# lgalke/aae-recommender

Measured on AMD Instinct MI355X. Metric: train docs/sec at |items|=100k h=200, higher is better.
Workload: dtype f32; 1 GPU; C3 PubMed-scale synthetic Bags: |items|=100000, hidden=200, code=50, fp32, batch=100 docs/GPU/step, full partial_fit (ae+disc+gen, 4 Adam) inside the AdversarialAutoEncoder.fit epoch loop (permutation batches of a corpus resident in HBM); n_items=100000, n_hidden=200, n_code=50, batch_per_gpu=100, global_batch=100, cond_inc=0, rng=device, parallelism=dp1

## Files before the change

### aae-recommender_amd/aaerec/_hip.py

```python
import ctypes as C
import itertools
import weakref
import os

import numpy as np
import torch

_HERE = os.path.dirname(os.path.abspath(__file__))
LIB_PATH = os.environ.get("AAE_HIP_LIB") or os.path.join(_HERE, "libaaerec_hip.so")

ABI_VERSION = 4
ACTIVATIONS = {"ReLU": 0, "SELU": 1, "Tanh": 2, "Sigmoid": 3, "ELU": 4, "LeakyReLU": 5,
               "Softplus": 6, "Hardtanh": 7, "ReLU6": 8, "CELU": 9, "Softsign": 10, "Hardsigmoid": 11, "LogSigmoid": 12,
               "Softshrink": 13, "Hardshrink": 14, "Identity": 15, "GELU": 16, "SiLU": 17, "Mish": 18, "Hardswish": 19}
FINALS = {"linear": 0, "softmax": 1, "sigmoid": 2}
OPTIMIZERS = {"adam": 0, "sgd": 1}
PRIORS = {"gauss": 0, "categorical": 1, "bernoulli": 2}
RNG_INJECT, RNG_DEVICE = 0, 1
RANK_K_MAX = 1024
COOC_TILE = 16384
SPGEMM_HASH_PRODUCTS = 4096
SPGEMM_STAGE = 512
SPTRANS_LDS = 4096
LOWRANK_DIMS_MAX = 4096
METRIC_MAX = 32
METRIC_ROW_MAX = 4096
RANK_ABSENT = 2 ** 31 - 1
METRIC_NDCG_K_MAX = 1 << 20
METRIC_KINDS = {"mrr": 0, "map": 1, "p": 2, "ndcg": 3, "r-prec": 4, "clicks": 5}
GRAD_FUSED, GRAD_EXPORT = 0, 1


class _NullCtx:
    def __enter__(self):
        return None

    def __exit__(self, *a):
        return False


_NULL_CTX = _NullCtx()

T_ENC_W1T, T_ENC_B1, T_ENC_W2, T_ENC_W3, T_DEC_V1, T_DEC_V2, T_DEC_V3, T_DISC_D1, T_DISC_D2, T_DISC_D3 = range(10)
T_ADAM_ENC, T_ADAM_GEN, T_ADAM_DEC, T_ADAM_DISC, T_GRAD = 16, 32, 48, 64, 80
T_ACT_Z, T_ACT_LOSSES, T_ACT_A1, T_ACT_DZC, T_ACT_DH2, T_ACT_DA2 = 96, 97, 98, 99, 100, 101
T_ACT_GA1 = 102
CAT_SUM, CAT_MEAN = 0, 1
CAT_SPARSE_ADAM, CAT_ADAM = 0, 1
O_ENC, O_DEC, O_GEN, O_DISC = 0, 1, 2, 3
MODEL_AAE, MODEL_AE, MODEL_VAE = 0, 1, 3
DTYPE_F32, DTYPE_BF16 = 0, 1


class AaeConfig(C.Structure):
    _fields_ = [("abi_version", C.c_int32), ("n_items", C.c_int32), ("n_hidden", C.c_int32),
                ("n_code", C.c_int32), ("cond_inc", C.c_int32), ("max_batch", C.c_int32),
                ("max_nnz", C.c_int32), ("activation", C.c_int32), ("enc_final", C.c_int32),
                ("optimizer", C.c_int32), ("normalize_inputs", C.c_int32), ("rng_mode", C.c_int32),
                ("prior", C.c_int32), ("grad_mode", C.c_int32), ("dropout1", C.c_float),
                ("dropout2", C.c_float), ("gen_lr", C.c_float), ("reg_lr", C.c_float),
                ("prior_scale", C.c_float), ("has_prior_scale", C.c_int32), ("seed", C.c_uint64),
                ("unfused_decoder", C.c_int32), ("dp_world", C.c_int32), ("model_kind", C.c_int32),
                ("dtype", C.c_int32), ("blocked_output", C.c_int32), ("dense_noise", C.c_int32),
                ("reserved", C.c_int32 * 2)]


class AaeBatch(C.Structure):
    _fields_ = [("indptr_dev", C.c_void_p), ("indices_dev", C.c_void_p), ("values_dev", C.c_void_p),
                ("rows_dev", C.c_void_p), ("row_start", C.c_int32), ("n_rows", C.c_int32),
                ("nnz_bound", C.c_int32), ("max_row_nnz", C.c_int32), ("generation", C.c_int64)]


class AaeRngInject(C.Structure):
    _fields_ = [("masks_dev", C.c_void_p * 12), ("z_real_dev", C.c_void_p)]


_COLL_AG = C.CFUNCTYPE(C.c_int, C.c_void_p, C.c_void_p, C.c_void_p, C.c_int64, C.c_void_p)
_COLL_AR = C.CFUNCTYPE(C.c_int, C.c_void_p, C.c_void_p, C.c_int64, C.c_void_p)


class AaeCollectives(C.Structure):
    _fields_ = [("ctx", C.c_void_p), ("all_gather", _COLL_AG), ("reduce_scatter", _COLL_AG), ("all_reduce", _COLL_AR),
                ("world", C.c_int32), ("rank", C.c_int32)]


class AaeTensor(C.Structure):
    _fields_ = [("byte_offset", C.c_size_t), ("rows", C.c_int64), ("cols", C.c_int64), ("ld", C.c_int64)]


class AaeCooc(C.Structure):
    _fields_ = [("indptr_dev", C.c_void_p), ("indices_dev", C.c_void_p), ("values_dev", C.c_void_p), ("n_rows", C.c_int32)]


class AaePopular(C.Structure):
    _fields_ = [("counts_dev", C.c_void_p), ("order_dev", C.c_void_p), ("pos_dev", C.c_void_p), ("n_items", C.c_int32)]


class AaeMetricSpec(C.Structure):
    _fields_ = [("kind", C.c_int32), ("k", C.c_int32)]


class AaeRankRows(C.Structure):
    _fields_ = [("indptr_dev", C.c_void_p), ("ranks_dev", C.c_void_p), ("n_rows", C.c_int32)]


class AaeLowRank(C.Structure):
    _fields_ = [("vt_dev", C.c_void_p), ("ld", C.c_int64), ("n_features", C.c_int32), ("dims", C.c_int32)]


_PROTOS = {
    "aae_abi_version": (C.c_int, []),
    "aae_set_option": (C.c_int, [C.c_char_p, C.c_char_p]),
    "aae_last_error": (C.c_char_p, []),
    "aae_arena_bytes": (C.c_int, [C.POINTER(AaeConfig), C.POINTER(C.c_size_t)]),
    "aae_create": (C.c_int, [C.POINTER(AaeConfig), C.c_void_p, C.c_size_t, C.c_void_p, C.POINTER(C.c_void_p)]),
    "aae_destroy": (C.c_int, [C.c_void_p]),
    "aae_tensor_info": (C.c_int, [C.c_void_p, C.c_int, C.POINTER(AaeTensor)]),
    "aae_set_lr": (C.c_int, [C.c_void_p, C.c_double, C.c_double]),
    "aae_params_changed": (C.c_int, [C.c_void_p]),
    "aae_set_rng_rows": (C.c_int, [C.c_void_p, C.c_int64, C.c_int64]),
    "aae_sync": (C.c_int, [C.c_void_p, C.c_void_p]),
    "aae_load_linear": (C.c_int, [C.c_void_p, C.c_int, C.c_int, C.c_void_p, C.c_void_p]),
    "aae_store_linear": (C.c_int, [C.c_void_p, C.c_int, C.c_int, C.c_void_p, C.c_void_p]),
    "aae_load_adam": (C.c_int, [C.c_void_p, C.c_int, C.c_int, C.c_void_p, C.c_void_p, C.c_void_p, C.c_void_p, C.c_int64]),
    "aae_store_adam": (C.c_int, [C.c_void_p, C.c_int, C.c_int, C.c_void_p, C.c_void_p, C.c_void_p, C.c_void_p, C.POINTER(C.c_int64)]),
    "aae_step": (C.c_int, [C.c_void_p, C.POINTER(AaeBatch), C.c_void_p, C.POINTER(AaeRngInject), C.c_void_p]),
    "aae_ae_encode": (C.c_int, [C.c_void_p, C.POINTER(AaeBatch), C.POINTER(AaeRngInject), C.c_void_p, C.c_void_p]),
    "aae_ae_decode_backward": (C.c_int, [C.c_void_p, C.c_void_p, C.c_int64, C.POINTER(AaeRngInject), C.c_void_p, C.c_void_p]),
    "aae_vae_step": (C.c_int, [C.c_void_p, C.POINTER(AaeBatch), C.c_void_p, C.c_void_p, C.c_void_p]),
# ... 39 lines not shown
    "aae_w1_import": (C.c_int, [C.c_void_p, C.c_void_p, C.c_void_p, C.c_int32, C.c_int32, C.c_int64, C.c_int, C.c_void_p]),
    "aae_set_grad_scale": (C.c_int, [C.c_void_p, C.c_float]),
    "aae_ae_forward": (C.c_int, [C.c_void_p, C.POINTER(AaeBatch), C.c_void_p, C.POINTER(AaeRngInject), C.c_void_p]),
    "aae_output_layer_step": (C.c_int, [C.c_void_p, C.POINTER(AaeBatch), C.c_void_p]),
    "aae_ae_backward": (C.c_int, [C.c_void_p, C.c_void_p, C.c_int64, C.c_void_p]),
    "aae_set_doc_l1": (C.c_int, [C.c_void_p, C.c_void_p]),
    "aae_set_first_layer_external": (C.c_int, [C.c_void_p, C.c_int]),
    "aae_first_layer_forward": (C.c_int, [C.c_void_p, C.POINTER(AaeBatch), C.c_void_p, C.c_void_p]),
    "aae_first_layer_update": (C.c_int, [C.c_void_p, C.c_void_p, C.c_int64, C.c_int32, C.c_int64, C.c_int, C.c_void_p]),
    "aae_apply_gathered": (C.c_int, [C.c_void_p, C.c_int, C.c_int, C.c_void_p, C.c_int64, C.c_int32, C.c_int64, C.c_void_p]),
    "aae_cat_encode": (C.c_int, [C.c_void_p, C.c_int32, C.c_int32, C.c_void_p, C.c_int32, C.c_int32, C.c_int32, C.c_void_p,
                                 C.c_int64, C.c_void_p]),
    "aae_cat_update": (C.c_int, [C.c_void_p, C.c_void_p, C.c_void_p, C.c_void_p, C.c_int32, C.c_int32, C.c_void_p, C.c_int32,
                                 C.c_int32, C.c_int32, C.c_void_p, C.c_int64, C.c_int32, C.c_double, C.c_int64, C.c_void_p]),
    "aae_csr_embed": (C.c_int, [C.c_void_p, C.c_void_p, C.c_void_p, C.c_int32, C.c_void_p, C.c_int32, C.c_int32, C.c_int64,
                                C.c_void_p, C.c_int64, C.c_void_p]),
    "aae_cooc_scores": (C.c_int, [C.POINTER(AaeCooc), C.c_int32, C.POINTER(AaeBatch), C.c_void_p, C.c_int64, C.c_void_p]),
    "aae_cooc_topk": (C.c_int, [C.POINTER(AaeCooc), C.c_int32, C.POINTER(AaeBatch), C.c_int32, C.c_int32, C.c_void_p, C.c_int64,
                                C.c_void_p, C.c_void_p, C.c_void_p]),
    "aae_cooc_ranks": (C.c_int, [C.POINTER(AaeCooc), C.c_int32, C.POINTER(AaeBatch), C.POINTER(AaeBatch), C.c_int32, C.c_void_p,
                                 C.c_int64, C.c_void_p, C.c_void_p]),
    "aae_cooc_scores_i32": (C.c_int, [C.POINTER(AaeCooc), C.c_int32, C.POINTER(AaeBatch), C.c_void_p, C.c_int64, C.c_void_p]),
    "aae_cooc_topk_i32": (C.c_int, [C.POINTER(AaeCooc), C.c_int32, C.POINTER(AaeBatch), C.c_int32, C.c_int32, C.c_void_p, C.c_int64,
                                    C.c_void_p, C.c_void_p, C.c_void_p]),
    "aae_cooc_ranks_i32": (C.c_int, [C.POINTER(AaeCooc), C.c_int32, C.POINTER(AaeBatch), C.POINTER(AaeBatch), C.c_int32, C.c_void_p,
                                     C.c_int64, C.c_void_p, C.c_void_p]),
    "aae_spgemm_i32_bound": (C.c_int, [C.POINTER(AaeCooc), C.POINTER(AaeCooc), C.c_int32, C.c_void_p, C.c_void_p]),
    "aae_spgemm_i32_count": (C.c_int, [C.POINTER(AaeCooc), C.POINTER(AaeCooc), C.c_int32, C.c_void_p, C.c_void_p, C.c_void_p]),
    "aae_spgemm_i32_fill": (C.c_int, [C.POINTER(AaeCooc), C.POINTER(AaeCooc), C.c_int32, C.c_void_p, C.c_void_p, C.c_void_p, C.c_void_p,
                                      C.c_void_p]),
    "aae_csr_transpose_count": (C.c_int, [C.c_void_p, C.c_void_p, C.c_int32, C.c_int32, C.c_void_p, C.c_void_p]),
    "aae_csr_transpose_fill": (C.c_int, [C.c_void_p, C.c_void_p, C.c_void_p, C.c_int32, C.c_int32, C.c_void_p, C.c_void_p, C.c_void_p,
                                         C.c_void_p, C.c_void_p, C.c_int64, C.c_int64, C.c_void_p]),
    "aae_mi_i32_marginals": (C.c_int, [C.POINTER(AaeCooc), C.POINTER(AaeCooc), C.c_int32, C.c_int32, C.c_void_p, C.c_void_p, C.c_void_p,
                                       C.c_void_p]),
    "aae_mi_i32_rows": (C.c_int, [C.POINTER(AaeCooc), C.POINTER(AaeCooc), C.c_int32, C.c_void_p, C.c_void_p, C.c_void_p, C.c_void_p,
                                  C.c_void_p]),
    "aae_mi_i32_finish": (C.c_int, [C.c_int32, C.c_void_p, C.c_void_p, C.c_void_p, C.c_void_p]),
    "aae_pop_counts": (C.c_int, [C.POINTER(AaeCooc), C.c_int32, C.c_void_p, C.c_void_p]),
    "aae_pop_topk": (C.c_int, [C.POINTER(AaePopular), C.POINTER(AaeBatch), C.c_int32, C.c_int32, C.c_void_p, C.c_void_p, C.c_void_p]),
    "aae_pop_ranks": (C.c_int, [C.POINTER(AaePopular), C.POINTER(AaeBatch), C.POINTER(AaeBatch), C.c_int32, C.c_void_p, C.c_void_p]),
    "aae_rand_scores": (C.c_int, [C.c_uint64, C.c_int64, C.c_int64, C.c_int32, C.c_int32, C.c_int32, C.c_void_p, C.c_int64, C.c_void_p]),
    "aae_rand_topk": (C.c_int, [C.c_uint64, C.c_int64, C.c_int64, C.c_int32, C.c_int32, C.POINTER(AaeBatch), C.c_int32, C.c_int32, C.c_void_p,
                                C.c_void_p, C.c_void_p]),
    "aae_rand_ranks": (C.c_int, [C.c_uint64, C.c_int64, C.c_int64, C.c_int32, C.c_int32, C.POINTER(AaeBatch), C.POINTER(AaeBatch), C.c_int32,
                                 C.c_void_p, C.c_void_p]),
    "aae_metric_rows": (C.c_int, [C.POINTER(AaeRankRows), C.POINTER(AaeMetricSpec), C.c_int32, C.c_void_p, C.c_int32, C.c_void_p,
                                  C.c_int64, C.c_void_p]),
    "aae_metric_finish": (C.c_int, [C.c_void_p, C.c_int64, C.c_int32, C.c_int32, C.c_void_p, C.c_void_p]),
    "aae_ranks_from_lists": (C.c_int, [C.c_void_p, C.c_int64, C.c_int32, C.POINTER(AaeBatch), C.c_void_p, C.c_void_p]),
    "aae_spmm_f32": (C.c_int, [C.POINTER(AaeBatch), C.c_void_p, C.c_int64, C.c_int32, C.c_int32, C.c_void_p, C.c_int64, C.c_void_p]),
    "aae_lowrank_scores": (C.c_int, [C.POINTER(AaeLowRank), C.c_int32, C.POINTER(AaeBatch), C.c_void_p, C.c_int64, C.c_void_p, C.c_int64,
                                     C.c_void_p]),
    "aae_lowrank_topk": (C.c_int, [C.POINTER(AaeLowRank), C.c_int32, C.POINTER(AaeBatch), C.POINTER(AaeBatch), C.c_int32, C.c_int32,
                                   C.c_void_p, C.c_int64, C.c_void_p, C.c_int64, C.c_void_p, C.c_void_p, C.c_void_p]),
    "aae_lowrank_ranks": (C.c_int, [C.POINTER(AaeLowRank), C.c_int32, C.POINTER(AaeBatch), C.POINTER(AaeBatch), C.POINTER(AaeBatch),
                                    C.c_int32, C.c_void_p, C.c_int64, C.c_void_p, C.c_int64, C.c_void_p, C.c_void_p]),
    "aae_dense_to_csr": (C.c_int, [C.c_void_p, C.c_int32, C.c_int64, C.c_int32, C.c_int32, C.c_void_p, C.c_void_p, C.c_void_p,
                                   C.c_int64, C.c_void_p, C.POINTER(C.c_int32 * 4), C.c_void_p]),
    "aae_profile_enable": (C.c_int, [C.c_void_p, C.c_int]),
    "aae_profile_read": (C.c_int, [C.c_void_p, C.c_int, C.POINTER(C.c_double), C.POINTER(C.c_int64)]),
    "aae_join": (C.c_int, [C.c_void_p, C.c_void_p]),
    "aae_join_output_layer": (C.c_int, [C.c_void_p, C.c_void_p]),
    "aae_rccl_unique_id": (C.c_int, [C.c_char_p]),
    "aae_rccl_init": (C.c_int, [C.c_char_p, C.c_int32, C.c_int32, C.POINTER(AaeCollectives)]),
    "aae_rccl_destroy": (C.c_int, [C.POINTER(AaeCollectives)]),
    "aae_dp_step": (C.c_int, [C.c_void_p, C.c_void_p, C.POINTER(AaeCollectives), C.POINTER(AaeBatch), C.POINTER(AaeBatch),
                              C.POINTER(AaeBatch), C.c_void_p, C.POINTER(AaeRngInject), C.c_void_p]),
    "aae_dp_reserve": (C.c_int, [C.c_void_p, C.c_int32, C.c_int32]),
    "aae_shard_step": (C.c_int, [C.c_void_p, C.POINTER(AaeCollectives), C.POINTER(AaeBatch), C.POINTER(AaeBatch), C.c_void_p,
                                 C.POINTER(AaeRngInject), C.c_float, C.c_void_p]),
    "aae_memcpy_sync": (C.c_int, [C.c_void_p, C.c_void_p, C.c_size_t, C.c_void_p]),
    "aae_echo_collectives": (C.c_int, [C.c_int32, C.POINTER(AaeCollectives)]),
    "aae_ipc_create": (C.c_int, [C.c_int64, C.c_char_p, C.POINTER(C.c_void_p)]),
    "aae_ipc_init": (C.c_int, [C.c_void_p, C.c_char_p, C.c_int32, C.c_int32, C.c_int64, C.POINTER(AaeCollectives)]),
    "aae_ipc_destroy": (C.c_int, [C.POINTER(AaeCollectives), C.c_void_p]),
    "aae_set_input_noise": (C.c_int, [C.c_void_p, C.c_void_p, C.c_int64]),
    "aae_set_input_noise_gen": (C.c_int, [C.c_void_p, C.c_float]),
    "aae_dae_thin": (C.c_int, [C.c_void_p, C.c_void_p, C.c_void_p, C.c_void_p, C.c_int64, C.c_float, C.c_void_p, C.c_void_p]),
    "aae_prefetch_batch": (C.c_int, [C.c_void_p, C.POINTER(AaeBatch)]),
    "aae_set_split": (C.c_int, [C.c_void_p, C.c_int32]),
}
K_ENC_GATHER, K_DEC_BCE_FWD, K_DEC_DA2, K_DEC_DV3_ADAM, K_ENC_W1_ADAM, K_DEC_FUSED, K_CHAIN, K_DEC_CRIT, K_DEC_OPT, K_RANK, K_COLLECTIVE = range(11)

_lib = None


class AaeHipError(RuntimeError):
    pass


def _destroy_handle(lib, handle, arena, pid):
    if os.getpid() == pid:
        try:
            lib.aae_destroy(handle)
        except Exception:
            pass
    del arena


def load_library():
    global _lib
    if _lib is not None:
        return _lib
    if not os.path.exists(LIB_PATH):
        raise ImportError(
            f"{LIB_PATH} is missing: build it with `python -c 'import __graft_entry__ as g; g.build()'` "
            "(hipcc --offload-arch=gfx950).  There is no CPU fallback for the AAE step.")
    lib = C.CDLL(LIB_PATH)
    for name, (res, args) in _PROTOS.items():
        fn = getattr(lib, name)
        fn.restype, fn.argtypes = res, args
    if lib.aae_abi_version() != ABI_VERSION:
        raise ImportError("libaaerec_hip.so ABI version mismatch")
    _lib = lib
    return lib


def set_option(name, value):
    _check(load_library().aae_set_option(str(name).encode(), None if value is None else str(value).encode()))


def _check(rc):
    if rc != 0:
        raise AaeHipError(f"libaaerec_hip error {rc}: {load_library().aae_last_error().decode()}")


def _ptr(t):
    return None if t is None else C.c_void_p(t.data_ptr())


def _arg(a):
    if a is None or torch.is_tensor(a):
        return _ptr(a)
    return C.byref(a) if isinstance(a, C.Structure) else a


_UPLOAD_STREAMS = {}


def upload(x, device, dtype=None):
    t = x if torch.is_tensor(x) else torch.as_tensor(np.asarray(x))
    dev = torch.device(device)
    if t.is_cuda or dev.type != "cuda":
        return t.to(dev, dtype) if dtype is not None else t.to(dev)
    if dtype is not None:
        t = t.to(dtype)
    side = _UPLOAD_STREAMS.get(dev)
    if side is None:
        side = _UPLOAD_STREAMS[dev] = torch.cuda.Stream(dev)
    with torch.cuda.stream(side):
        out = t.to(dev)
    out.record_stream(torch.cuda.current_stream(dev))
    return out


class HostRows:
    PIN_LIMIT = 32 << 30

    def __init__(self, n_rows, n_cols, device):
        self.device = torch.device(device)
        self.pinned = n_rows * n_cols * 4 <= self.PIN_LIMIT
        if self.pinned:
            try:
                self.host = torch.empty(n_rows, n_cols, dtype=torch.float32, pin_memory=True)
            except RuntimeError:
# ... 1304 lines not shown
```

### aae-recommender_amd/csrc/aae_abi.hip

```cpp
#include <hip/hip_runtime.h>
#include <hip/hip_ext.h>
#include <math.h>
#include <stdio.h>
#include <stdlib.h>
#include <string.h>

#include <algorithm>
#include <string>
#include <vector>

#include "../../include/aaerec_hip.h"
#include "gemm_f32.h"
#include "kernels.h"
#include "dec_fused.h"
#include "dec_fused_bf16.h"
#include "dec_crit_x3.h"
#include "rank_x3.h"
#include "rank_long.h"
#include "rank_full.h"
#include "cooc.h"
#include "spgemm.h"
#include "sptrans.h"
#include "mutinfo.h"
#include "popular.h"
#include "randrank.h"
#include "rank_metrics.h"
#include "lowrank.h"
#include "chain.h"
#include "chain4.h"
#include "chain16x3.h"
#include "cond_embed.h"
#include "w1_update.h"
#include "dae_corrupt.h"

using namespace aae;

#include "kernel_pick.h"

#include <map>
static std::map<std::string, std::string> g_options;
const char* option_value(const char* name) {
    auto it = g_options.find(name);
    if (it != g_options.end()) return it->second.c_str();
    return getenv((std::string("AAE_") + name).c_str());
}

#include "abi_model.h"
#include "abi_layers.h"
#include "abi_chains.h"
#include "abi_rank.h"

extern "C" {

int aae_abi_version(void) { return AAE_ABI_VERSION; }

int aae_set_option(const char* name, const char* value) {
    if (!name || !*name) return fail(AAE_EINVAL, "option name is empty");
    static const char* known[] = {"NO_CHAIN", "CHAIN16", "SPLIT_ANY", "BLOCKED_ANY", "EARLY_ANY", "NO_LATE_JOIN", "NO_ITEM_COUNT", "NO_ITEM_LISTS", "W1_SERIAL",
                                  "NO_RANK_FUSED", "CHAIN_KSLICES", "X16_ROWS", "DW_KSPLIT_ROWS", "DEC_TS", "CHAIN_TS", "DW_TS", "DEC_SKIP", "CHAIN_SKIP", "RANK_SKIP",
                                  "RANK_COLLECT_CAP"};
    bool ok = false;
    for (const char* k : known) ok = ok || strcmp(k, name) == 0;
    if (!ok) return fail(AAE_EINVAL, "unknown option (aae_options, csrc/abi_model.h, lists them)");
    if (value && strcmp(name, "RANK_COLLECT_CAP") == 0) {
        char* end = nullptr;
        const long v = strtol(value, &end, 10);
        if (end == value || *end || v < 1 || v > kLongCap) return fail(AAE_EINVAL, "RANK_COLLECT_CAP must be a whole number in [1, 4096]");
    }
    if (value) g_options[name] = value; else g_options.erase(name);
    return AAE_OK;
}
const char* aae_last_error(void) { return g_err.c_str(); }

int aae_arena_bytes(const aae_config* cfg, size_t* bytes_out) {
    TRY(validate(cfg));
    if (!bytes_out) return fail(AAE_EINVAL, "bytes_out is NULL");
    aae_model tmp; memset((void*)&tmp, 0, sizeof(tmp)); tmp.cfg = *cfg;
    read_options(tmp.opt);
    *bytes_out = layout(&tmp, nullptr, true);
    return AAE_OK;
}

int aae_create(const aae_config* cfg, void* arena_dev, size_t arena_bytes, void* stream, aae_handle* out) {
    TRY(validate(cfg));
    if (!arena_dev || !out) return fail(AAE_EINVAL, "arena/out is NULL");
    if (reinterpret_cast<uintptr_t>(arena_dev) & 255) return fail(AAE_EINVAL, "arena must be 256-byte aligned");
    aae_model* m = new aae_model();
    memset((void*)m, 0, sizeof(*m));
    m->cfg = *cfg;
    read_options(m->opt);
    size_t need = layout(m, static_cast<char*>(arena_dev), false);
    if (need > arena_bytes) { delete m; return fail(AAE_ENOMEM, "arena smaller than aae_arena_bytes()"); }
    m->base = static_cast<char*>(arena_dev); m->bytes = need;
    m->alpha_mode = cfg->activation == AAE_ACT_SELU;
    m->vae = cfg->model_kind == 3; m->vae_cut = false;
    m->bf16 = cfg->dtype == 1;
    m->blocked_ok = cfg->blocked_output == 1;
    m->blocked_any = m->opt.blocked_any;
    m->split_any = m->opt.split_any;
    m->x3_gemm = !m->bf16;
    m->noise_next = nullptr; m->noise_ld = 0; m->dense_step = false; m->noise_gen_next = false; m->noise_gen_scale = 0.f;
    m->ae_only = cfg->model_kind == 1 || m->vae;
    m->lazy = true;
    auto limit = [](bool& ok, size_t bytes) { return [&ok, bytes](auto kernel) { ok = ok && raise_lds_limit(kernel, bytes); }; };
    const int maxlds = 160 * 1024;
    {
        int dev = 0, cus = 0;
        if (hipGetDevice(&dev) != hipSuccess ||
            hipDeviceGetAttribute(&cus, hipDeviceAttributeMultiprocessorCount, dev) != hipSuccess || cus < 1) {
            delete m; return fail(AAE_EHIP, "no HIP device");
        }
        m->n_cu = std::min(cus, 304);
        const int nb = (m->h + 1 + 15) / 16;
        m->fused_nb = nb <= 4 ? 4 : nb <= 7 ? 7 : nb <= 13 ? 13 : 0;
        m->fused_ok = m->fused_nb != 0 && fused_width_ok(m->h, m->ldh);
        m->use_chain = (m->h + 1 <= 208) && (m->c + 1 <= 208) && (m->cp + 1 <= (m->vae ? kVaeDecInMax : 2 * 208)) &&
                       !m->opt.no_chain;
        const size_t chain_lds = kCSlots * kCR * kCL * sizeof(float);
        if (m->use_chain) each_chain(false, limit(m->use_chain, chain_lds));
        m->act_nm = cfg->activation > AAE_ACT_LEAKYRELU;
        if (m->use_chain && m->act_nm) each_chain(true, limit(m->use_chain, chain_lds));
        m->use_chain4 = m->use_chain && !m->act_nm && !m->opt.chain16;
        if (m->use_chain4) each_chain4(limit(m->use_chain4, chain_lds));
        if (m->use_chain && m->cp + 1 > 208 && !m->use_chain4 && !m->vae) m->use_chain = false;
        m->x16_rows = m->opt.x16_rows;
        m->dw_ksplit_rows = 256;
        if (m->opt.dw_ksplit_rows >= 0) m->dw_ksplit_rows = m->opt.dw_ksplit_rows;
        if (!m->opt.no_item_count) {
            void* hp = nullptr; void* dp = nullptr;
            if (hipHostMalloc(&hp, 64, hipHostMallocMapped) == hipSuccess && hipHostGetDevicePointer(&dp, hp, 0) == hipSuccess) {
                m->cnt_host = static_cast<int*>(hp); m->cnt_host_dev = static_cast<int*>(dp); *m->cnt_host = 0;
            } else { if (hp) (void)hipHostFree(hp); (void)hipGetLastError(); }
        }
        m->x16_ok = m->use_chain4 && m->FXi[P_W2] != nullptr;
        if (m->x16_ok) each_chain16x3(limit(m->x16_ok, kX16Lds));
        m->force_unfused = cfg->unfused_decoder == 1;
        if (m->fused_ok) {
            each_dec_fused(kDecFused, limit(m->fused_ok, maxlds));
            if (m->bf16) each_dec_fused_bf16(kDecFused, limit(m->fused_ok, maxlds));
            if (!raise_lds_limit(tile_bucket_kernel, maxlds - 2048)) m->fused_ok = false;
            m->bucket_wide_ok = raise_lds_limit(tile_bucket_wide_kernel, maxlds - 16384);
            {
                hipFuncAttributes fa;
                static bool told = false;
                if (m->bucket_wide_ok && !told && hipFuncGetAttributes(&fa, reinterpret_cast<const void*>(tile_bucket_wide_kernel)) == hipSuccess && fa.numRegs < 121) {
                    told = true;
                    fprintf(stderr, "aaerec: tile_bucket_wide_kernel allocates %d vector registers, not the 128 it claims to keep its CU to itself (buckets.h)\n", fa.numRegs);
                }
                (void)hipGetLastError();
            }
        }
    }
    m->late_enabled = !m->opt.no_late_join;
    m->early_enabled = true;
    m->early_any = m->opt.early_any;
    m->rank_ok = m->fused_ok && m->use_chain4 && !m->vae && !m->opt.no_rank_fused;
    m->vae_rank_ok = m->vae && m->fused_ok && m->use_chain4 && !m->opt.no_rank_fused;
    if (m->vae_rank_ok) each_chain4_vae(limit(m->vae_rank_ok, kCSlots * kCR * kCL * sizeof(float)));
    bool& rank_ok = m->vae ? m->vae_rank_ok : m->rank_ok;
    if (rank_ok) each_rank([&](const RankPick& r) { rank_ok = rank_ok && raise_lds_limit(r.kernel, r.lds); });
    m->w1_big_lds = raise_lds_limit(w1_item_update_kernel, sizeof(int) * w1_items_lds_words(16384));
    (void)hipGetLastError();
    m->grad_scale = 1.f;
    m->rng_row0 = 0; m->rng_global = 0;
    m->Gt = m->G.p;
    m->split_ok = false; m->opt_pending = false; m->side = nullptr; m->ev_crit = m->ev_opt = nullptr;
    m->split_wgs = std::max(1, (m->n_cu * 5) / 8);
    m->pf_armed = m->pf_built = m->pf_pending = false; m->pf_step = -1; m->hstep = 0; m->flushed_hstep = -1; m->ev_head = m->ev_pf = nullptr;
    bool side_ok = false;
    if (cfg->grad_mode == AAE_GRAD_FUSED) {
        int lo = 0, hi = 0;
        const unsigned evflags = hipEventDisableTiming | hipEventDisableSystemFence;
        side_ok = hipDeviceGetStreamPriorityRange(&lo, &hi) == hipSuccess &&
                  hipStreamCreateWithPriority(&m->side, hipStreamNonBlocking, lo) == hipSuccess &&
                  hipEventCreateWithFlags(&m->ev_crit, evflags) == hipSuccess &&
                  hipEventCreateWithFlags(&m->ev_opt, evflags) == hipSuccess &&
                  hipEventCreateWithFlags(&m->ev_head, evflags) == hipSuccess &&
                  hipEventCreateWithFlags(&m->ev_pf, evflags) == hipSuccess &&
                  hipEventCreateWithFlags(&m->ev_bk, evflags) == hipSuccess &&
                  hipEventCreateWithFlags(&m->ev_end, evflags) == hipSuccess;
        if (!side_ok) {
            if (m->side) (void)hipStreamDestroy(m->side);
            m->side = nullptr;
        }
        (void)hipGetLastError();
    }
    if (side_ok && m->fused_ok && m->bf16 && m->split_wgs > 0 &&
        (size_t)((m->N + kBU - 1) / kBU) * kBU * bf_stride(4) <= (size_t)m->R * m->ldn) {
        m->split_ok = true;
        for (int mode : {kDecCrit, kDecOpt}) each_dec_fused_bf16(mode, limit(m->split_ok, maxlds));
        (void)hipGetLastError();
    }
    if (side_ok && m->fused_ok && m->split_wgs > 0 && 
        (size_t)((m->N + kTI - 1) / kTI) * kTI * (size_t)std::min(m->R, 16 * kMB) * sizeof(float) < (size_t)0x7FFFFFF0u) {
        bool ok = true;
        for (int mode : {kDecCrit, kDecOpt, kDecOptAcc}) each_dec_fused(mode, limit(ok, maxlds));
        each_dec_opt_blocks(limit(ok, maxlds));
        if (!m->bf16) m->split_ok = ok;
        m->x3_ok = ok;
        each_dec_crit_x3(false, limit(m->x3_ok, maxlds));
        each_dec_opt_blocks_x3(limit(m->x3_ok, maxlds));
        each_dec_opt_x3(false, limit(m->x3_ok, maxlds));
        (void)hipGetLastError();
        if (m->bf16) {
            m->bf16_x3 = m->x3_ok && ok;
            if (!m->bf16_x3) m->x3_ok = false;
            else m->split_ok = true;
            m->bf16_one = m->bf16_x3;
            each_dec_crit_x3(true, limit(m->bf16_one, maxlds));
            each_dec_opt_x3(true, limit(m->bf16_one, maxlds));
            (void)hipGetLastError();
        }
        if (m->x3_ok) {
            const int ntiles = (m->N + 31) / 32;
            const double t_tile = (2.2 + 0.0096 * m->h) * (m->bf16_one ? 0.98 : 1.0);
            int w = (int)(ntiles * t_tile / (m->bf16_one ? 127.0 : 57.0) / 8.0 + 0.5) * 8;
            w = std::max(w, std::min(ntiles, m->bf16_one ? 40 : 64));
            const int cap = m->late_enabled ? m->n_cu * 7 / 16 : m->n_cu * 9 / 16;
            m->split_wgs = std::max(1, std::min(w, cap));
        }
    }
    hipStream_t s = S(stream);
    hipError_t e = hipMemsetAsync(arena_dev, 0, need, s);
    if (e != hipSuccess) { delete m; return fail(AAE_EHIP, std::string("hipMemsetAsync: ") + hipGetErrorString(e)); }
    struct { Ten* t; int col; } ones[] = {{&m->eh1, m->h}, {&m->eh2, m->h}, {&m->zc, m->cp}, {&m->dh1, m->h},
                                           {&m->dh2, m->h}, {&m->zin, m->c}, {&m->xh1, m->h}, {&m->xh2, m->h}};
    for (auto& o : ones)
        hipLaunchKernelGGL(fill_col_kernel, dim3(((int)o.t->rows + 255) / 256), dim3(256), 0, s, o.t->p, (int)o.t->ld,
                           (int)o.t->rows, o.col, 1.0f);
    OptScalars hs[4]; memset(hs, 0, sizeof(hs));
    for (int i = 0; i < 4; ++i) {
        hs[i].t = 0; hs[i].is_sgd = cfg->optimizer == AAE_OPT_SGD;
        hs[i].lr = (i == O_ENC || i == O_DEC) ? (double)cfg->gen_lr : (double)cfg->reg_lr;
        hs[i].neg_step_size = 0.f; hs[i].bc2_sqrt = 1.f; hs[i].inv_bc2_sqrt = 1.f;
    }
    e = hipMemcpyAsync(m->sc, hs, sizeof(hs), hipMemcpyHostToDevice, s);
    if (e == hipSuccess) e = hipStreamSynchronize(s);
    if (e != hipSuccess) { delete m; return fail(AAE_EHIP, std::string("init: ") + hipGetErrorString(e)); }
    *out = m;
    return AAE_OK;
}

#ifdef W1_TS
int aae_debug_w1_ts(unsigned long long* out, int n) {
    return (int)hipMemcpyFromSymbol(out, HIP_SYMBOL(aae::w1_ts), sizeof(unsigned long long) * (size_t)n);
}
#endif
int aae_destroy(aae_handle h) {
    if (!h) return AAE_OK;
    if (h->side) {
        (void)hipStreamSynchronize(h->side);
        (void)hipStreamDestroy(h->side);
    }
    if (h->dp_scratch) (void)hipFree(h->dp_scratch);
    if (h->cnt_host) (void)hipHostFree(h->cnt_host);
    for (hipEvent_t e : {h->ev_crit, h->ev_opt, h->ev_head, h->ev_pf, h->ev_bk, h->ev_end}) if (e) (void)hipEventDestroy(e);
    if (h->prof_ev) {
        for (int k = 0; k < AAE_K_N; ++k)
            for (auto& pr : h->prof_ev[k]) { (void)hipEventDestroy(pr.first); (void)hipEventDestroy(pr.second); }
        delete[] h->prof_ev;
    }
    delete h;
    return AAE_OK;
}


int aae_profile_enable(aae_handle h, int on) {
    if (!h) return fail(AAE_EINVAL, "handle is NULL");
    if (on && !h->prof_ev) h->prof_ev = new std::vector<std::pair<hipEvent_t, hipEvent_t>>[AAE_K_N];
    h->prof_on = on != 0;
    h->prof_mask = on == 1 ? ~0u : ((unsigned)on >> 1);
    return AAE_OK;
}

int aae_profile_read(aae_handle h, int kernel_id, double* total_ms, int64_t* launches) {
    if (!h || !total_ms || !launches) return fail(AAE_EINVAL, "NULL argument");
    if (kernel_id < 0 || kernel_id >= AAE_K_N) return fail(AAE_EINVAL, "bad kernel id");
    *total_ms = 0.0; *launches = 0;
    if (!h->prof_ev) return AAE_OK;
    auto& v = h->prof_ev[kernel_id];
    for (size_t i = 0; i < h->prof_used[kernel_id]; ++i) {
        HIPCHK(hipEventSynchronize(v[i].second));
        float ms = 0.f;
        HIPCHK(hipEventElapsedTime(&ms, v[i].first, v[i].second));
        *total_ms += ms; *launches += 1;
    }
    h->prof_used[kernel_id] = 0;
    return AAE_OK;
}

int aae_prefetch_batch(aae_handle h, const aae_batch* next) {
    if (!h || !next) return fail(AAE_EINVAL, "NULL argument");
    if (!next->indptr_dev || !next->indices_dev || !next->values_dev) return fail(AAE_EINVAL, "batch pointers are NULL");
    if (next->n_rows < 1 || next->n_rows > h->R) return fail(AAE_EINVAL, "batch n_rows outside [1, max_batch]");
    if (next->nnz_bound > h->cfg.max_nnz) return fail(AAE_EINVAL, "batch nnz_bound > max_nnz");
    if (next->generation == 0) { h->pf_armed = false; return AAE_OK; }
    h->pf_batch = *next;
    h->pf_armed = true;
    return AAE_OK;
}

// ... 3 lines not shown
    if (noise_dev && noise_ld < h->N) return fail(AAE_EINVAL, "noise_ld < n_items");
    h->noise_next = noise_dev; h->noise_ld = noise_ld;
    h->noise_gen_next = false;
    return AAE_OK;
}

int aae_join_output_layer(aae_handle h, void* stream) {
    if (!h) return fail(AAE_EINVAL, "handle is NULL");
    if (h->opt_pending) {
        HIPCHK(hipStreamWaitEvent(S(stream), h->ev_opt, 0));
        h->opt_pending = false;
        if (!h->pf_after_opt) h->pf_pending = false;
    }
    return AAE_OK;
}

int aae_join(aae_handle h, void* stream) {
    if (!h) return fail(AAE_EINVAL, "handle is NULL");
    return join_deferred(h, S(stream));
}

int aae_set_split(aae_handle h, int32_t workgroups) {
    if (!h) return fail(AAE_EINVAL, "handle is NULL");
    if (workgroups < 0) return fail(AAE_EINVAL, "workgroups must be >= 0");
    if (h->opt_pending) return fail(AAE_ESTATE, "aae_set_split with a deferred launch pending: call aae_join / aae_sync first");
    h->split_wgs = workgroups;
    return AAE_OK;
}

int aae_set_grad_scale(aae_handle h, float scale) {
    if (!h) return fail(AAE_EINVAL, "handle is NULL");
    h->grad_scale = scale; return AAE_OK;
}

int aae_set_rng_rows(aae_handle h, int64_t row_offset, int64_t global_rows) {
    if (!h) return fail(AAE_EINVAL, "handle is NULL");
    if (row_offset < 0 || global_rows < 0 || row_offset > (1 << 30) || global_rows > (1 << 30))
        return fail(AAE_EINVAL, "aae_set_rng_rows: bad offset / global_rows");
    h->rng_row0 = (int)row_offset; h->rng_global = (int)global_rows;
    return AAE_OK;
}

int aae_params_changed(aae_handle h) {
    if (!h) return fail(AAE_EINVAL, "handle is NULL");
    for (int i = 0; i < NP; ++i) h->pt_ok[i] = false;
    return AAE_OK;
}

int aae_set_lr(aae_handle h, double gen_lr, double reg_lr) {
    if (!h) return fail(AAE_EINVAL, "handle is NULL");
    TRY(join_host(h));
    OptScalars hs[4];
    HIPCHK(hipMemcpy(hs, h->sc, sizeof(hs), hipMemcpyDeviceToHost));
    hs[O_ENC].lr = gen_lr; hs[O_DEC].lr = gen_lr; hs[O_GEN].lr = reg_lr; hs[O_DISC].lr = reg_lr;
    HIPCHK(hipMemcpy(h->sc, hs, sizeof(hs), hipMemcpyHostToDevice));
    h->spec_tab_ok = false;
    return AAE_OK;
}

int aae_tensor_info(aae_handle h, int id, aae_tensor* out) {
    if (!h || !out) return fail(AAE_EINVAL, "handle/out is NULL");
    const Ten* t = nullptr;
    Ten tmp;
    auto adam = [&](int base, int lo, int hi, int set) -> const Ten* {
        int k = id - base, pid = lo + k / 2;
        if (k < 0 || pid > hi) return nullptr;
        return (k & 1) ? &h->V[set][pid] : &h->M[set][pid];
    };
    if (id >= 0 && id < AAE_T_N_PARAMS) t = &h->P[id];
    else if (id >= AAE_T_ADAM_ENC && id < AAE_T_ADAM_ENC + 8) t = adam(AAE_T_ADAM_ENC, P_W1T, P_W3, 0);
    else if (id >= AAE_T_ADAM_GEN && id < AAE_T_ADAM_GEN + 8) t = adam(AAE_T_ADAM_GEN, P_W1T, P_W3, 1);
    else if (id >= AAE_T_ADAM_DEC && id < AAE_T_ADAM_DEC + 6) t = adam(AAE_T_ADAM_DEC, P_V1, P_V3, 0);
    else if (id >= AAE_T_ADAM_DISC && id < AAE_T_ADAM_DISC + 6) t = adam(AAE_T_ADAM_DISC, P_D1, P_D3, 0);
    else if (id >= AAE_T_GRAD && id < AAE_T_GRAD + NP) { t = &h->Gr[id - AAE_T_GRAD]; if (!t->rows) t = nullptr; }
    else if (id == AAE_T_ACT_Z) t = &h->zsave;
    else if (id == AAE_T_ACT_A1) t = &h->a1;
    else if (id == AAE_T_ACT_DH2) t = &h->dh2;
    else if (id == AAE_T_ACT_DA2) t = &h->da2;
    else if (id == AAE_T_ACT_GA1) t = (h->ext_first && h->ga1x.p) ? &h->ga1x : h->use_chain ? &h->gb3 : &h->gb1;
    else if (id == AAE_T_ACT_DZC) { tmp = h->gzc; tmp.cols = h->cp; t = &tmp; }
    else if (id == AAE_T_ACT_LOSSES) {
        tmp.rows = 1; tmp.cols = 4; tmp.ld = 4; tmp.off = (size_t)((char*)h->losses - h->base); t = &tmp;
    }
    if (!t) return fail(AAE_EINVAL, "unknown tensor id");
    out->byte_offset = t->off; out->rows = t->rows; out->cols = t->cols; out->ld = t->ld;
    return AAE_OK;
}

int aae_sync(aae_handle h, void* stream) {
    if (!h) return fail(AAE_EINVAL, "handle is NULL");
    TRY(join_deferred(h, S(stream)));
    return lazy_flush(h, S(stream));
}


}

#include "abi_condition.h"
#include "abi_state_dict.h"
#include "abi_dae.h"
#include "abi_step_open.h"
#include "abi_output_layer.h"
#include "abi_step_phases.h"
#include "abi_predict.h"
#include "abi_cooc.h"
#include "abi_spgemm.h"
#include "abi_sptrans.h"
#include "abi_mutinfo.h"
#include "abi_popular.h"
#include "abi_random.h"
#include "abi_metrics.h"
#include "abi_lowrank.h"
#include "abi_data_parallel.h"

#include "dp_step.h"
#include "ipc_collectives.h"
```

### aae-recommender_amd/csrc/abi_chains.h

```cpp
#pragma once

namespace {

ChainOp cop(int kind, int src, int dst, int N) {
    ChainOp o; memset(&o, 0, sizeof(o));
    o.kind = kind; o.src = src; o.dst = dst; o.N = N; o.one_col = -1; o.scale = 1.f; o.yslot = 0; o.fake_slot = -1;
    return o;
}
ChainOp cop_load(const float* g, int ld, int dst, int N, int row0 = 0) {
    ChainOp o = cop(COP_LOAD, 0, dst, N); o.W = g; o.ldw = ld; o.out_row0 = row0; return o;
}
ChainOp cop_linear(int kind, int src, int dst, const Ten& W, int K, int N, int epi) {
    ChainOp o = cop(kind, src, dst, N); o.W = W.p; o.ldw = (int)W.ld; o.K = K; o.epi = epi;
    if (kind == COP_LINEAR_DX) { o.Wkn = W.p; o.ldkn = (int)W.ld; }
    return o;
}
void cop_out(ChainOp& o, float* out, int ld, int row0 = 0) { o.out = out; o.ldo = ld; o.out_row0 = row0; }

W4Copies w4_of(const aae_model* m, int pid) {
    return W4Copies{m->PT[pid].p, m->D4[pid].p, (int)m->P[pid].rows, (int)m->P[pid].cols, m->FXi[pid], m->DXi[pid], m->FXBi[pid], kCWide};
}
float* ga1_ptr(const aae_model* m) {
    return (m->ext_first && m->ga1x.p) ? m->ga1x.p + (size_t)(m->R - m->rows) * m->ldh : m->gb3.p;
}
// ... 173 lines not shown
        if (u.src >= 0) o.src = phys[u.src];
        if (u.y >= 0) o.yslot = phys[u.y];
        if (u.fake >= 0) o.fake_slot = phys[u.fake];
        o.dst = phys[u.dst];
        if (o.kind == COP_FINAL_FWD) o.src = o.dst;
    }
    return true;
}

static bool x16_program_ok(const ChainProgram& P) {
    for (int i = 0; i < P.nops; ++i) {
        const ChainOp& o = P.ops[i];
        switch (o.kind) {
            case COP_LINEAR: case COP_LINEAR_DX:
                if (!o.WX || o.N > kCWide || o.K > kX16Kp) return false;
                break;
            case COP_LOAD: if (o.dst_col0 + o.N > kX16Kp) return false; break;
            case COP_DROPACT: case COP_SLABSUM: case COP_STORE: case COP_FINAL_FWD: case COP_FINAL_BWD: case COP_PRIOR: case COP_DISC_HEAD:
                if (o.N > kCWide) return false;
                break;
            default: return false;
        }
        if (o.one_col >= kX16Kp) return false;
    }
    return true;
}

int print_chain_timeline(const ChainProgram& P, const unsigned long long* ts_dev, bool x16, bool four, hipStream_t s) {
    static const char* names[] = {"LOAD", "LINEAR", "LINEAR_DX", "FINAL_FWD", "FINAL_BWD", "ADV", "DROPACT", "SLABSUM", "ACTBWD", "STORE", "REPARAM", "REPARAM_BWD", "DISC_HEAD", "PRIOR"};
    unsigned long long h[128];
    HIPCHK(hipStreamSynchronize(s));
    HIPCHK(hipMemcpy(h, ts_dev, sizeof(h), hipMemcpyDeviceToHost));
    if (x16) {
        fprintf(stderr, "[chain16x3 rows=%d nops=%d total=%.2fus; per op: whole (products | epilogue | barrier)]", P.rows, P.nops, (h[3 * P.nops] - h[0]) * 0.01);
        for (int i = 0; i < P.nops; ++i) {
            const bool lin = P.ops[i].kind == COP_LINEAR || P.ops[i].kind == COP_LINEAR_DX;
            fprintf(stderr, " %s(K%d,N%d)=%.2f", names[P.ops[i].kind], P.ops[i].K, P.ops[i].N, (h[3 * i + 3] - h[3 * i]) * 0.01);
            if (lin) fprintf(stderr, "(%.2f|%.2f|%.2f)", (h[3 * i + 1] - h[3 * i]) * 0.01, (h[3 * i + 2] - h[3 * i + 1]) * 0.01, (h[3 * i + 3] - h[3 * i + 2]) * 0.01);
        }
        fprintf(stderr, "\n");
        return AAE_OK;
    }
    fprintf(stderr, "[chain rows=%d nops=%d total=%.2fus]", P.rows, P.nops, (h[P.nops] - h[0]) * 0.01);
    for (int i = 0; i < P.nops; ++i)
        fprintf(stderr, " %s(K%d,N%d%s%s)=%.2f", names[P.ops[i].kind], P.ops[i].K, P.ops[i].N,
                P.ops[i].out ? ",st" : "", P.ops[i].out2 ? ",st2" : "", (h[i + 1] - h[i]) * 0.01);
    fprintf(stderr, "\n");
    if (P.nops <= 2) return AAE_OK;
    fprintf(stderr, "   [op 2, wave 0 of workgroup 0] loads+mfma+partials=%.2f wait-barrier=%.2f epi-ctx=%.2f epilogue=%.2f barrier=%.2f (us)\n",
            (h[21] - h[20]) * 0.01, (h[22] - h[21]) * 0.01, (h[23] - h[22]) * 0.01, (h[24] - h[23]) * 0.01, (h[25] - h[24]) * 0.01);
    if (!four) return AAE_OK;
    fprintf(stderr, "   [op 2: matrix phase %.2f us = %.0f shader clocks -> %.2f GHz]\n", (h[64 + 50] - h[64 + 48]) * 0.01,
            (double)(h[64 + 51] - h[64 + 49]), (double)(h[64 + 51] - h[64 + 49]) / ((h[64 + 50] - h[64 + 48]) * 10.0));
    for (int k = 0; k < 3; ++k) {
        fprintf(stderr, "   [op 2, every wave, us after the op's start: %s]", k == 0 ? "loads issued" : k == 1 ? "first chunk multiplied" : "partial sums stored");
        for (int w = 0; w < 16; ++w) fprintf(stderr, " %.2f", ((double)h[64 + 16 * k + w] - (double)h[64 + 48]) * 0.01);
        fprintf(stderr, "\n");
    }
    return AAE_OK;
}

int launch_chain(aae_model* m, ChainBuilder& cb, hipStream_t s) {
    if (cb.P.nops > kCMaxOps) return fail(AAE_ESTATE, "chain program too long");
    const bool want_ts = m->opt.chain_ts && !cb.vae4;
    static unsigned long long* ts_dev = nullptr;
    if (want_ts) {
        if (!ts_dev && hipMalloc(&ts_dev, 128 * sizeof(unsigned long long)) != hipSuccess) return fail(AAE_EHIP, "ts alloc");
        cb.P.ts = ts_dev;
    }
    const bool ts_kernel = want_ts && !m->bf16;
    ProfScope ps(m, AAE_K_CHAIN, s);
    bool four = m->use_chain4;
    for (int i = 0; i < cb.P.nops && four; ++i)
        if ((cb.P.ops[i].kind == COP_LINEAR || cb.P.ops[i].kind == COP_LINEAR_DX) && !cb.P.ops[i].Wkn && !cb.P.ops[i].W4) four = false;
    for (int i = 0; i < cb.P.nops && four; ++i)
        if (cb.P.ops[i].kind == COP_ADV || (cb.P.ops[i].kind == COP_REPARAM && !cb.vae4) || cb.P.ops[i].kind == COP_REPARAM_BWD) four = false;
    if (cb.vae4 && !four) return fail(AAE_ESTATE, "a VAE rank program needs the 4-row chain kernel");
    for (int i = 0; i < cb.P.nops; ++i)
        if ((cb.P.ops[i].row_lo > 0 || cb.P.ops[i].y_glb) && !four)
            return fail(AAE_ESTATE, "a program prefix for the upper rows / an epilogue's y from global memory needs the 4-row chain kernel");
    if (four && m->x16_ok && cb.P.rows >= (cb.x16_rows > 0 ? cb.x16_rows : m->x16_rows) && !cb.P.bk.enabled && !cb.P.il.enabled && x16_program_ok(cb.P)) {
        ChainProgram X = cb.P;
        if (x16_remap_slots(X)) {
            X.x16_row_lo = 1 << 30;
            for (int i = 0; i < X.nops; ++i) if (X.ops[i].row_lo > 0) X.x16_row_lo = X.ops[i].row_lo;
            for (int cls = 0; cls < 2; ++cls) {
                int nxt = -1;
                for (int i = X.nops - 1; i >= 0; --i) {
                    X.ops[i].x16_next_lin[cls] = nxt;
                    const bool runs = cls == 1 || X.ops[i].row_lo == 0;
                    if (runs && (X.ops[i].kind == COP_LINEAR || X.ops[i].kind == COP_LINEAR_DX)) nxt = i;
                }
                X.x16_first_lin[cls] = nxt;
            }
            const ChainKernel kernel = pick_chain16x3(m->bf16, ts_kernel);
            if (!kernel) return fail(AAE_ESTATE, "no chain16x3 kernel is compiled for this mode");
            hipLaunchKernelGGL(kernel, dim3((X.rows + kX16R - 1) / kX16R), dim3(kX16T), kX16Lds, s, X);
            LAUNCHCHK("chain16x3_kernel");
            return ts_kernel ? print_chain_timeline(X, ts_dev, true, four, s) : AAE_OK;
        }
    }
    const ChainKernel kernel = four ? pick_chain4(m->bf16, ts_kernel, m->bf16 && !cb.P.kslices, cb.vae4) : pick_chain(m->bf16, m->act_nm);
    if (!kernel) return fail(AAE_ESTATE, "no chain kernel is compiled for this mode");
    int grid = (cb.P.rows + (four ? kR4 : kCR) - 1) / (four ? kR4 : kCR) + (cb.P.bk.enabled ? 1 : 0);
    if (cb.P.il.enabled && !four) cb.P.il.enabled = 0;
    if (cb.P.il.enabled) { grid += cb.P.il.nblocks; m->il_set ^= 1; m->item_lists_valid = true; }
    hipLaunchKernelGGL(kernel, dim3(grid), dim3(four ? kC4T : kCT), kCSlots * kCR * kCL * sizeof(float), s, cb.P);
    LAUNCHCHK("chain_kernel");
    return want_ts ? print_chain_timeline(cb.P, ts_dev, false, four, s) : AAE_OK;
}

int launch_w1_hot(aae_model* m, hipStream_t s);
static ItemLists item_lists_of(const aae_model* m, int set) {
    ItemLists L;
    L.rec = m->il_rec[set]; L.ovf = m->il_ovf[set]; L.hot_count = m->il_hot_count + set; L.cap = m->il_cap; L.hot_cap = m->il_hot_cap;
    return L;
}
struct DwBuilder {
    aae_model* mh = nullptr;
    DwGroup g; int tiles;
    int ksplit_rows = 0;
    int dw_ts = -1;
    DwBuilder() { memset(&g, 0, sizeof(g)); tiles = 0; }
    void add(aae_model* m, const float* G, int ldg, const float* X, int ldx, int rows, int pid, int which) {
        DwJob& J = g.jobs[g.njobs++];
        ksplit_rows = m->dw_ksplit_rows; dw_ts = m->opt.dw_ts;
        const Ten& W = m->P[pid];
        const int set = (which == O_GEN) ? 1 : 0;
        J.G = G; J.ldg = ldg; J.X = X; J.ldx = ldx; J.rows = rows; J.M = (int)W.rows; J.N = (int)W.cols;
        J.p = W.p; J.m = m->M[set][pid].p; J.v = m->V[set][pid].p; J.ld = (int)W.ld; J.sc = m->sc + which;
        J.grad = m->cfg.grad_mode == AAE_GRAD_EXPORT ? m->Gr[pid].p : nullptr;
        J.w4 = w4_of(m, pid);
        J.tile0 = tiles; J.tiles_n = (J.N + 31) / 32;
        tiles += ((J.M + 31) / 32) * J.tiles_n;
    }
    int add_first_layer(aae_model* m, const float* ga1, int which, hipStream_t s) {
        const int set = (which == O_GEN) ? 1 : 0;
        W1Job& w = g.w1;
        w.enabled = 1; w.ga1 = ga1; w.ld = m->ldh; w.h = m->h; w.rows = m->rows;
        w.bp = m->P[P_B1].p; w.bm = m->M[set][P_B1].p; w.bv1 = m->V[set][P_B1].p;
        w.bgrad = m->cfg.grad_mode == AAE_GRAD_EXPORT ? m->Gr[P_B1].p : nullptr; w.sc = m->sc + which;
        w.ncol = (m->h + 63) / 64;
        constexpr bool no_merge = false;
        w.nitem = 0;
        m->w1_items_merged = false;
        w.wave_form = 0;
        if (!no_merge && !m->dense_step && (!m->ext_first || m->own_first) && sizeof(int) * w1_items_lds_words(m->rows) <= kDwSmemBytes) {
            TRY(ensure_buckets(m, s));
            w.items = w1_items_args(m, ga1, 0, 0, which);
            w.nitem = std::max(1, std::min(std::min(m->cfg.max_nnz, std::max(256, m->rows * 32)), m->N));
            m->w1_items_merged = true;
            constexpr bool no_wave = false;
            constexpr bool no_hybrid = false, hyb_any = false;
            if (!no_hybrid && m->rows <= 16 * kMB && sizeof(int) * w1_hybrid_lds_words(m->rows) <= kDwSmemBytes &&
                (int64_t)m->cfg.max_nnz <= 512ll * w.nitem && ((int64_t)m->N >= 40ll * m->rows || hyb_any)) {
                w.wave_form = 2;
                w.nitem = (w.nitem + 3) / 4;
                if (m->item_lists_valid && !w.items.gout) {
                    w.lists_on = 1; w.lists = item_lists_of(m, m->il_set);
                    w.nhot = std::min(m->il_hot_cap, 64);
                }
            } else
            if (!no_wave && m->rows > 16 * kMB && m->hot_list && (int64_t)m->N >= 40ll * m->rows) {
                w.wave_form = 1;
                w.nitem = (w.nitem + 3) / 4;
                const int set = m->hot_flip; m->hot_flip ^= 1;
                w.hot = m->hot_list + (size_t)set * m->hot_cap; w.hot_count = m->hot_count + set; w.hot_zero = m->hot_count + (set ^ 1);
                m->w1_hot_pending = true; m->w1_hot_set = set; m->w1_hot_which = which; m->w1_hot_ga1 = ga1;
                mh = m;
            }
            w.cnt_out = nullptr;
            constexpr bool hyb_count = true;
            if ((w.wave_form != 2 || hyb_count) && m->cnt_host) {
                w.cnt_out = m->cnt_host_dev;
                const int seen = *reinterpret_cast<volatile int*>(m->cnt_host);
                if (seen > 0) {
                    const int per = w.wave_form ? 4 : 1;
                    int want = ((seen + seen / 4 + per - 1) / per + 63) & ~63;
                    if (w.wave_form == 2) want = std::max(want, (int)((std::min<int64_t>(m->cfg.max_nnz, m->N) + 2047) / 2048));
                    w.nitem = std::min(w.nitem, std::max(256, want));
                }
            }
            if (w.lists_on) w.nitem += w.nhot;
        }
        return AAE_OK;
    }
    void add_loss(aae_model* m, int n, int slot) { g.loss.enabled = 1; g.loss.terms = m->adv_terms; g.loss.n = n; g.loss.out = m->losses + slot; }
    int launch(hipStream_t s, hipEvent_t done = nullptr, bool* marked = nullptr) {
        int blocks = tiles;
// ... 120 lines not shown
        const int gy = std::max(1, std::min(16, m->chunks / 16 + 1));
        hipLaunchKernelGGL(zero_int_kernel, dim3(std::min(64, ntiles / 256 + 1)), dim3(256), 0, s, m->tcount, ntiles + 1);
        hipLaunchKernelGGL(tile_hist_kernel, dim3(B, gy), dim3(256), 0, s, m->bv, m->tcount);
        hipLaunchKernelGGL(tile_scan_kernel, dim3(1), dim3(1024), 0, s, m->tcount, m->tstart, ntiles);
        hipLaunchKernelGGL(tile_fill_kernel, dim3(B, gy), dim3(256), 0, s, m->bv, m->tstart, m->tcount, m->teb, m->ten, m->tev);
    }
    LAUNCHCHK("tile buckets");
    m->buckets_valid = true;
    return AAE_OK;
}
int build_tile_buckets_aside(aae_model* m) {
    TRY(build_tile_buckets(m, m->side));
    HIPCHK(hipEventRecord(m->ev_bk, m->side));
    m->bk_pending = true;
    return AAE_OK;
}
int ensure_buckets(aae_model* m, hipStream_t s) {
    if (m->bk_pending) {
        HIPCHK(hipStreamWaitEvent(s, m->ev_bk, 0));
        m->bk_pending = false;
    }
    if (!m->buckets_valid) TRY(build_tile_buckets(m, s));
    return AAE_OK;
}

W1Items w1_items_args(aae_model* m, const float* ga1, int rpb, size_t bstride, int which) {
    const int set = (which == O_GEN) ? 1 : 0;
    W1Items a;
    a.ulist = m->ulist; a.ucount = m->ucount;
    a.tstart = m->tstart; a.eb = m->teb; a.en = m->ten; a.ev = m->tev;
    a.ga1 = ga1; a.ld = m->ldh; a.rpb = rpb; a.bstride = bstride;
    a.rscale = m->rscale; a.rows = m->rows; a.h = m->h;
    a.W = m->P[P_W1T].p; a.M = m->M[set][P_W1T].p; a.V = m->V[set][P_W1T].p; a.ldw = m->ldw1;
    a.gout = m->cfg.grad_mode == AAE_GRAD_EXPORT ? m->Gr[P_W1T].p : nullptr;
    a.sc = m->sc + which; a.tsync = m->tsync; a.step_ctr = m->step_ctr;
    a.mark_synced = (which == O_GEN || m->ae_only) ? 1 : 0;
    return a;
}
int launch_w1_items(aae_model* m, const float* ga1, int rpb, size_t bstride, int which, hipStream_t s) {
    TRY(ensure_buckets(m, s));
    const W1Items a = w1_items_args(m, ga1, rpb, bstride, which);
    const size_t lds = sizeof(int) * w1_items_lds_words(m->rows);
    if (lds > 64 * 1024 && !m->w1_big_lds) return fail(AAE_ESTATE, "first-layer update: batch too large for the LDS row lists");
    ProfScope ps(m, AAE_K_ENC_W1_ADAM, s);
    const int items = std::max(1, std::min(std::min(m->cfg.max_nnz, std::max(256, m->rows * 32)), m->N));
    hipLaunchKernelGGL(w1_item_update_kernel, dim3(items), dim3(256), lds, s, a);
    LAUNCHCHK("w1_item_update");
    return AAE_OK;
}

static void piggyback_buckets(aae_model* m, ChainBuilder& cb) {
    const int ntiles = (m->N + kTI - 1) / kTI;
    const size_t need = sizeof(int) * ((size_t)ntiles + 1 + kBucketMaxDocs + 1 + 1024);
    if (m->x16_ok && m->rows >= m->x16_rows) return;
    if (m->buckets_valid || !fused_decoder_applies(m) || ntiles > kBucketMaxTiles || m->rows > kBucketMaxDocs ||
        need > (size_t)kCSlots * kCR * kCL * sizeof(float))
        return;
    flip_bucket_set(m);
    BucketJob& b = cb.P.bk;
    b.bv = m->bv; b.ntiles = ntiles; b.tstart = m->tstart; b.eb = m->teb; b.en = m->ten; b.ev = m->tev; b.enabled = 1;
    m->buckets_valid = true;
}

static void piggyback_item_lists(aae_model* m, ChainBuilder& cb) {
    if (m->opt.no_item_lists || !m->il_cap || m->item_lists_valid || !m->buckets_valid || m->bk_pending) return;
    if (m->cfg.grad_mode != AAE_GRAD_FUSED || m->dense_step || m->ext_first) return;
    if (m->x16_ok && m->rows >= m->x16_rows) return;
    const int bound = std::max(1, std::min(std::min(m->cfg.max_nnz, std::max(256, m->rows * 32)), m->N));
    if (!(m->rows <= 16 * kMB && sizeof(int) * w1_items_lds_words(m->rows) <= kDwSmemBytes &&
          sizeof(int) * w1_hybrid_lds_words(m->rows) <= kDwSmemBytes && (int64_t)m->cfg.max_nnz <= 512ll * bound &&
          (int64_t)m->N >= 40ll * m->rows))
        return;
    static_assert(sizeof(int) * (kC4T / 64 * 2 * kW1HybRows + kW1BuildDeferWords + 2 * 4 + 2 * kW1OvfRows + 4) <= kCSlots * kCR * kCL * sizeof(float),
                  "the builder's LDS fits a chain workgroup's");
    const int set = m->il_set ^ 1;
    ItemListJob& j = cb.P.il;
    j.ulist = m->ulist; j.ucount = m->ucount; j.tstart = m->tstart; j.eb = m->teb; j.en = m->ten; j.ev = m->tev;
    j.rscale = m->rscale; j.rows = m->rows;
    j.out = item_lists_of(m, set); j.hot_zero = m->il_hot_count + (set ^ 1);
    j.nblocks = std::max(1, std::min(64, (bound + 2 * (kC4T / 64) - 1) / (2 * (kC4T / 64))));
    j.enabled = 1;
}

int chain_ae_forward(aae_model* m, bool with_dec, const float* cond_dev, float* z_out, hipStream_t s) {
    const int B = m->rows, h = m->h, c = m->c, cp = m->cp;
    const aae_rng_inject& I = m->inj;
    ChainBuilder cb(m, B);
    piggyback_buckets(m, cb);
    chain_encoder_tail(m, cb, true, I.masks_dev[1], 1, B, m->eh2.p, s, I.masks_dev[0], 0);
    ChainOp& f = m->cfg.enc_final == AAE_FINAL_LINEAR ? cb.P.ops[cb.P.nops - 1] : cb.add(cop(COP_FINAL_FWD, 2, 2, c));
    f.aux = m->cfg.enc_final;
    cop_out(f, m->zc.p, m->ldc); f.out2 = m->zsave.p; f.ldo2 = m->ldz;
    if (z_out) { ChainOp& st = cb.add(cop(COP_STORE, 2, 2, c)); cop_out(st, z_out, c); }
    if (with_dec) {
        if (wide_dec_in(m)) {
            const int nA = kCWide - c, ci = m->cfg.cond_inc;
            ChainOp& ca = cb.add(cop_load(cond_dev, ci, 2, nA)); ca.dst_col0 = c;
            ChainOp& cl = cb.add(cop_load(cond_dev + nA, ci, 5, ci - nA)); cl.one_col = cp - kCWide;
        } else if (m->cfg.cond_inc > 0) {
            ChainOp& cl = cb.add(cop_load(cond_dev, m->cfg.cond_inc, 2, m->cfg.cond_inc)); cl.dst_col0 = c; cl.one_col = cp;
        } else {
            f.one_col = cp;
        }
        ChainOp& v1 = add_dec_in_fwd(cb, m, 2, 5, 3, s);
        v1.d = make_drop(m, 0, true, I.masks_dev[2], nullptr, B, h, 2); v1.one_col = h; cop_out(v1, m->dh1.p, m->ldh);
        ChainOp& v2 = cb.add(cop_fwd(m, P_V2, 3, 4, h + 1, h, CEPI_DROPACT, s));
        v2.d = make_drop(m, 1, true, I.masks_dev[3], nullptr, B, h, 3); v2.one_col = h; cop_out(v2, m->dh2.p, m->ldh);
    }
    m->dec_hidden_done = with_dec;
    return launch_chain(m, cb, s);
}

int chain_dec_hidden(aae_model* m, bool train, int rows, hipStream_t s) {
    const int h = m->h, cp = m->cp;
    const aae_rng_inject& I = m->inj;
    ChainBuilder cb(m, rows);
    if (wide_dec_in(m)) {
        cb.add(cop_load(m->zc.p, m->ldc, 0, kCWide));
        ChainOp& lb = cb.add(cop_load(m->zc.p + kCWide, m->ldc, 3, cp - kCWide)); lb.one_col = cp - kCWide;
    } else {
        ChainOp& l = cb.add(cop_load(m->zc.p, m->ldc, 0, cp)); l.one_col = cp;
    }
    ChainOp& v1 = add_dec_in_fwd(cb, m, 0, 3, 1, s);
    v1.d = make_drop(m, 0, train, I.masks_dev[2], nullptr, rows, h, 2); v1.one_col = h; cop_out(v1, m->dh1.p, m->ldh);
    ChainOp& v2 = cb.add(cop_fwd(m, P_V2, 1, 2, h + 1, h, CEPI_DROPACT, s));
    v2.d = make_drop(m, 1, train, I.masks_dev[3], nullptr, rows, h, 3); v2.one_col = h; cop_out(v2, m->dh2.p, m->ldh);
    return launch_chain(m, cb, s);
}

int chain_ae_backward(aae_model* m, bool dec_part, bool enc_part, const float* part_slabs, size_t slab_stride,
                      const float* gz_ext, int ld_gz, float* dzc_out, int which, hipStream_t s, int nslab = 16, bool item_lists = false) {
    const int B = m->rows, h = m->h, c = m->c, cp = m->cp;
    const aae_rng_inject& I = m->inj;
    ChainBuilder cb(m, B);
    if (dec_part) {
        if (part_slabs) {
            ChainOp& ss = cb.add(cop(COP_SLABSUM, 0, 2, h)); ss.W = part_slabs; ss.ldw = m->ldh; ss.aux = nslab; ss.stride = slab_stride;
            ss.epi = CEPI_ACTBWD; ss.aux_ptr = m->dh2.p; ss.aux_ld = m->ldh;
            ss.d = make_drop(m, 1, true, I.masks_dev[3], nullptr, B, h, 3); cop_out(ss, m->gb0.p, m->ldh);
        } else {
            cb.add(cop_load(m->gb0.p, m->ldh, 2, h));
        }
        if (y_needs_load(m)) cb.add(cop_load(m->dh1.p, m->ldh, 3, h));
        ChainOp& x2 = cb.add(cop_dx(m, P_V2, 2, 4, h, h, CEPI_ACTBWD, s)); set_y(cb, m, x2, m->dh1.p, m->ldh, 3);
        x2.d = make_drop(m, 0, true, I.masks_dev[2], nullptr, B, h, 2); cop_out(x2, m->gb1.p, m->ldh);
        add_dec_in_dx(cb, m, 4, 5, 3, dzc_out, s);
    }
    if (enc_part) {
        if (!dec_part || gz_ext) cb.add(cop_load(gz_ext ? gz_ext : m->gzc.p, gz_ext ? ld_gz : m->ldc, 5, c));
        int sg = 7;
        ChainOp* prod = (dec_part && !gz_ext && cb.P.nops) ? &cb.P.ops[cb.P.nops - 1] : nullptr;
        if (m->cfg.enc_final == AAE_FINAL_LINEAR && prod && cp == c && !prod->out2) {
            prod->out2 = m->ga3.p; prod->ldo2 = m->ldz; sg = 5;
        } else {
            if (m->cfg.enc_final != AAE_FINAL_LINEAR) cb.add(cop_load(m->zsave.p, m->ldz, 6, c));
            ChainOp& fb = cb.add(cop(COP_FINAL_BWD, 5, 7, c)); fb.yslot = 6; fb.aux = m->cfg.enc_final;
            cop_out(fb, m->ga3.p, m->ldz);
        }
        if (y_needs_load(m)) cb.add(cop_load(m->eh2.p, m->ldh, 8, h));
        ChainOp& x3 = cb.add(cop_dx(m, P_W3, sg, 9, c, h, CEPI_ACTBWD, s)); set_y(cb, m, x3, m->eh2.p, m->ldh, 8);
        x3.d = make_drop(m, 1, true, I.masks_dev[which == O_GEN ? 9 : 1], nullptr, B, h, which == O_GEN ? 9 : 1);
        cop_out(x3, m->gb2.p, m->ldh);
        if (y_needs_load(m)) cb.add(cop_load(m->eh1.p, m->ldh, 0, h));
        ChainOp& x2 = cb.add(cop_dx(m, P_W2, 9, 1, h, h, CEPI_ACTBWD, s)); set_y(cb, m, x2, m->eh1.p, m->ldh, 0);
        x2.d = make_drop(m, 0, true, I.masks_dev[which == O_GEN ? 8 : 0], nullptr, B, h, which == O_GEN ? 8 : 0);
        cop_out(x2, ga1_ptr(m), m->ldh);
    }
    if (item_lists) piggyback_item_lists(m, cb);
    return launch_chain(m, cb, s);
}

int encoder_first_layer_update(aae_model* m, const float* ga1, int which, hipStream_t s, bool merged = false) {
    const int B = m->rows, h = m->h;
    const int set = (which == O_GEN) ? 1 : 0;
    const bool exportg = m->cfg.grad_mode == AAE_GRAD_EXPORT;
    if (m->dense_step) {
        if (!merged) {
            hipLaunchKernelGGL(colsum_adam_kernel, dim3((h + 63) / 64), dim3(1024), 0, s, ga1, B, h, m->ldh, m->P[P_B1].p,
                               m->M[set][P_B1].p, m->V[set][P_B1].p, (float*)nullptr, m->sc + which);
            LAUNCHCHK("colsum_adam");
        }
        TRY(linear_dw(m, m->Xn.p, m->ldn, B, ga1, m->ldh, P_W1T, which, s));
        hipLaunchKernelGGL(fill_tsync_kernel, dim3(grid1d((size_t)m->N)), dim3(256), 0, s, m->tsync, m->N, m->step_ctr);
        LAUNCHCHK("fill_tsync");
        return AAE_OK;
    }
    if (!merged) {
        hipLaunchKernelGGL(colsum_adam_kernel, dim3((h + 63) / 64), dim3(1024), 0, s, ga1, B, h, m->ldh, m->P[P_B1].p,
                           m->M[set][P_B1].p, m->V[set][P_B1].p, exportg ? m->Gr[P_B1].p : (float*)nullptr, m->sc + which);
        LAUNCHCHK("colsum_adam");
    }
    if (merged && m->w1_items_merged) { m->w1_items_merged = false; return AAE_OK; }
    return launch_w1_items(m, ga1, 0, 0, which, s);
}

int launch_gather(aae_model* m, const float* bias, float* act_out, const DropSpec& d, bool head, bool open_step, const char* what,
                  hipStream_t s) {
    ProfScope ps(m, AAE_K_ENC_GATHER, s);
    const size_t shm = (size_t)16 * r4(m->h) * sizeof(float);
    constexpr int g4_rows = 512;
    const bool four = m->rows >= g4_rows;
    const AdvanceJob adv{m->sc, m->step_ctr, m->lazy ? m->tab : nullptr, m->losses, open_step ? 1 : 0,
                         head ? m->stamp2 : nullptr, head ? m->ucount2 : nullptr};
    hipExtLaunchKernelGGL(four ? enc_gather_kernel_t<4> : enc_gather_kernel_t<16>, dim3(m->rows), dim3(four ? 256 : 1024),
                          (uint32_t)(four ? shm / 4 : shm), s, nullptr, head ? m->ev_head : nullptr, 0, m->bv,
                          (const float*)m->P[P_W1T].p, m->ldw1, bias, m->h, (int)m->cfg.normalize_inputs,
                          m->a1.p, act_out, m->ldh, (int)m->cfg.activation, d, (uint64_t)m->cfg.seed,
                          (const long long*)m->step_ctr, m->rscale, m->doc_l1, adv, (long long)(open_step ? m->hstep : -1));
    LAUNCHCHK(what);
    return AAE_OK;
}

int gather_first_layer(aae_model* m, bool train, const uint8_t* mk1, uint32_t sid1, hipStream_t s, bool head = false,
                       bool open_step = false) {
    const DropSpec d1 = make_drop(m, 0, train, mk1, nullptr, m->rows, m->h, sid1);
    TRY(launch_gather(m, m->P[P_B1].p, m->eh1.p, d1, head, open_step, "enc_gather", s));
    m->pf_bumped = head;
    return AAE_OK;
}

static bool same_batch(const aae_batch& a, const aae_batch& b) {
    return a.indptr_dev == b.indptr_dev && a.indices_dev == b.indices_dev && a.values_dev == b.values_dev &&
           a.rows_dev == b.rows_dev && a.row_start == b.row_start && a.n_rows == b.n_rows &&
           a.generation != 0 && a.generation == b.generation;
}

int launch_prefetch(aae_model* m, bool wait_head = true, bool early = false) {
    const aae_batch& b = m->pf_batch;
    m->pf_armed = false;
    m->pf_this_step = true;
    m->pf_after_opt = !wait_head;
    if (!m->side || !m->mark2 || !m->lazy) return AAE_OK;
    BatchView bv; bv.indptr = b.indptr_dev; bv.indices = b.indices_dev; bv.values = b.values_dev;
    bv.rows = b.rows_dev; bv.row_start = b.row_start; bv.n_rows = b.n_rows;
    const int mr = b.max_row_nnz > 0 ? b.max_row_nnz : 1024;
    const int chunks = std::max(1, std::min(64, (mr + 15) / 16));
    const int gy = std::max(1, std::min(16, chunks / 16 + 1));
    hipStream_t q = m->side;
    if (early) HIPCHK(hipStreamWaitEvent(q, m->ev_end, 0));
    else if (wait_head) HIPCHK(hipStreamWaitEvent(q, m->ev_head, 0));
    if (early || !(wait_head && m->pf_bumped)) hipLaunchKernelGGL(bump_stamp_kernel, dim3(1), dim3(1), 0, q, m->stamp2, m->ucount2);
    m->pf_bumped = false;
    hipLaunchKernelGGL(uniq_items_kernel, dim3(b.n_rows, gy), dim3(256), 0, q, bv, m->mark2, m->stamp2, m->ulist2, m->ucount2);
    if (m->cfg.optimizer == AAE_OPT_ADAM) {
        const int grid = std::min(m->cfg.max_nnz, std::max(256, b.n_rows * 32));
        hipLaunchKernelGGL(w1_catchup_kernel, dim3(grid), dim3(256), 0, q, m->ulist2, m->ucount2, m->N, m->tsync,
                           m->P[P_W1T].p, m->M[0][P_W1T].p, m->V[0][P_W1T].p, m->M[1][P_W1T].p, m->V[1][P_W1T].p,
                           m->ldw1, m->h, m->tab, m->step_ctr, 0, m->mark, m->stamp, early ? m->hstep : -1ll);
    }
    LAUNCHCHK("prefetch (unique items + catch-up of the next batch)");
    TRY(side_done(m, m->ev_pf));
    m->pf_pending = true;
    m->pf_built = true; m->pf_step = m->hstep + 1; m->pf_built_batch = b;
    return AAE_OK;
}

int chain_vae_forward(aae_model* m, const float* cond_dev, const float* eps_dev, int rows, hipStream_t s) {
    const int h = m->h, c = m->c, cp = m->cp;
    ChainBuilder cb(m, rows);
    ChainOp& l = cb.add(cop_load(m->eh1.p, m->ldh, 0, h)); l.one_col = h;
    ChainOp& ml = cb.add(cop_fwd(m, P_W3, 0, 1, h + 1, 2 * c, CEPI_NONE, s));
    cop_out(ml, m->mulv.p, (int)m->mulv.ld);
    ChainOp& rp = cb.add(cop(COP_REPARAM, 1, 2, c));
    rp.W = eps_dev; rp.ldw = c; rp.aux = 12; rp.aux_ptr = m->veps.p; rp.aux_ld = (int)m->veps.ld;
    if (wide_dec_in(m)) {
        ChainOp& ca = cb.add(cop_load(cond_dev, m->cfg.cond_inc, 2, kCWide - c)); ca.dst_col0 = c;
        ChainOp& st = cb.add(cop(COP_STORE, 2, 2, kCWide)); cop_out(st, m->zc.p, m->ldc);
    } else {
        if (m->cfg.cond_inc > 0) {
            ChainOp& cl = cb.add(cop_load(cond_dev, m->cfg.cond_inc, 2, m->cfg.cond_inc)); cl.dst_col0 = c; cl.one_col = cp;
        } else {
            rp.one_col = cp;
        }
        ChainOp& st = cb.add(cop(COP_STORE, 2, 2, cp)); cop_out(st, m->zc.p, m->ldc);
    }
    ChainOp& v1 = add_vae_dec_in_fwd(cb, m, cond_dev, m->cfg.cond_inc, c, true, 2, 4, 3, nullptr);
    v1.one_col = h; cop_out(v1, m->dh2.p, m->ldh);
    return launch_chain(m, cb, s);
}

int chain_vae_encode(aae_model* m, const float* eps_dev, float* z_out, int rows, hipStream_t s) {
    const int h = m->h, c = m->c;
    ChainBuilder cb(m, rows);
    ChainOp& l = cb.add(cop_load(m->eh1.p, m->ldh, 0, h)); l.one_col = h;
    ChainOp& ml = cb.add(cop_fwd(m, P_W3, 0, 1, h + 1, 2 * c, CEPI_NONE, s));
    cop_out(ml, m->mulv.p, (int)m->mulv.ld);
    ChainOp& rp = cb.add(cop(COP_REPARAM, 1, 2, c));
    rp.W = eps_dev; rp.ldw = c; rp.aux = 12; rp.aux_ptr = m->veps.p; rp.aux_ld = (int)m->veps.ld;
    ChainOp& st = cb.add(cop(COP_STORE, 2, 2, c)); cop_out(st, m->zc.p, m->ldc);
    if (z_out) { st.out2 = z_out; st.ldo2 = c; }
    return launch_chain(m, cb, s);
}
int chain_vae_dec_hidden(aae_model* m, int rows, hipStream_t s) {
    const int h = m->h, cp = m->cp;
    ChainBuilder cb(m, rows);
    ChainOp& l = cb.add(cop_load(m->zc.p, m->ldc, 2, std::min(cp, kCWide)));
    if (!wide_dec_in(m)) l.one_col = cp;
    ChainOp& v1 = add_vae_dec_in_fwd(cb, m, m->zc.p, m->ldc, 0, false, 2, 4, 3, nullptr);
    v1.one_col = h; cop_out(v1, m->dh2.p, m->ldh);
    return launch_chain(m, cb, s);
}
int chain_vae_backward_dec(aae_model* m, const float* part_slabs, size_t slab_stride, float* dzc_out, hipStream_t s) {
    const int B = m->rows, h = m->h, cp = m->cp;
    ChainBuilder cb(m, B);
    if (part_slabs) {
        ChainOp& ss = cb.add(cop(COP_SLABSUM, 0, 0, h)); ss.W = part_slabs; ss.ldw = m->ldh; ss.aux = 16; ss.stride = slab_stride;
        cb.add(cop_load(m->dh2.p, m->ldh, 1, h));
        ChainOp& ab = cb.add(cop(COP_ACTBWD, 0, 2, h)); ab.yslot = 1; cop_out(ab, m->gb0.p, m->ldh);
    } else {
        cb.add(cop_load(m->gb0.p, m->ldh, 2, h));
    }
    add_vae_dec_in_dx(cb, m, 2, 3, 8, true, dzc_out);
    return launch_chain(m, cb, s);
}
int chain_vae_backward_enc(aae_model* m, const float* dz_dev, int ld_dz, hipStream_t s) {
    const int B = m->rows, h = m->h, c = m->c;
    ChainBuilder cb(m, B);
    cb.P.loss_slot = 1;
    cb.add(cop_load(dz_dev, ld_dz, 3, c));
    cb.add(cop_load(m->mulv.p, (int)m->mulv.ld, 4, 2 * c));
    ChainOp& rb = cb.add(cop(COP_REPARAM_BWD, 3, 5, 2 * c)); rb.yslot = 4; rb.scale = m->grad_scale;
    rb.aux_ptr = m->veps.p; rb.aux_ld = (int)m->veps.ld; cop_out(rb, m->gmulv.p, (int)m->gmulv.ld);
    cb.add(cop_load(m->eh1.p, m->ldh, 6, h));
    ChainOp& x1 = cb.add(cop_linear(COP_LINEAR_DX, 5, 7, m->P[P_W3], 2 * c, h, CEPI_ACTBWD)); x1.yslot = 6;
    cop_out(x1, m->gb3.p, m->ldh);
    return launch_chain(m, cb, s);
}

int chain_vae_backward(aae_model* m, const float* part_slabs, size_t slab_stride, hipStream_t s) {
    const int B = m->rows, h = m->h, c = m->c, cp = m->cp;
    ChainBuilder cb(m, B);
    cb.P.loss_slot = 1;
    if (part_slabs) {
        ChainOp& ss = cb.add(cop(COP_SLABSUM, 0, 0, h)); ss.W = part_slabs; ss.ldw = m->ldh; ss.aux = 16; ss.stride = slab_stride;
        cb.add(cop_load(m->dh2.p, m->ldh, 1, h));
        ChainOp& ab = cb.add(cop(COP_ACTBWD, 0, 2, h)); ab.yslot = 1; cop_out(ab, m->gb0.p, m->ldh);
    } else {
        cb.add(cop_load(m->gb0.p, m->ldh, 2, h));
    }
    add_vae_dec_in_dx(cb, m, 2, 3, 8, cp > c, nullptr);
    cb.add(cop_load(m->mulv.p, (int)m->mulv.ld, 4, 2 * c));
    ChainOp& rb = cb.add(cop(COP_REPARAM_BWD, 3, 5, 2 * c)); rb.yslot = 4; rb.scale = m->grad_scale;
    rb.aux_ptr = m->veps.p; rb.aux_ld = (int)m->veps.ld; cop_out(rb, m->gmulv.p, (int)m->gmulv.ld);
    cb.add(cop_load(m->eh1.p, m->ldh, 6, h));
    ChainOp& x1 = cb.add(cop_linear(COP_LINEAR_DX, 5, 7, m->P[P_W3], 2 * c, h, CEPI_ACTBWD)); x1.yslot = 6;
    cop_out(x1, m->gb3.p, m->ldh);
    return launch_chain(m, cb, s);
}

int chain_disc_step(aae_model* m, hipStream_t s) {
    const int B = m->rows, h = m->h, c = m->c;
    const aae_rng_inject& I = m->inj;
    if (!m->ext_first) TRY(gather_first_layer(m, false, nullptr, 0, s));
    constexpr bool merge_ok = true;
    bool merged = merge_ok && m->use_chain4 && B % kR4 == 0 && !m->vae;
    for (int pid : {P_W2, P_W3, P_D1, P_D2}) merged = merged && m->PT[pid].p != nullptr;
    if (!merged) {
        ChainBuilder cb(m, B);
        chain_encoder_tail(m, cb, false, nullptr, 0, B, nullptr, s);
        ChainOp& f = m->cfg.enc_final == AAE_FINAL_LINEAR ? cb.P.ops[cb.P.nops - 1] : cb.add(cop(COP_FINAL_FWD, 2, 2, c));
        f.aux = m->cfg.enc_final; cop_out(f, m->zin.p, m->ldz, B);
        TRY(launch_chain(m, cb, s));
    }
    {
        ChainBuilder cb(m, 2 * B);
        cb.beside_deferred(m);
        cb.P.loss_slot = 1; cb.P.loss_terms = m->adv_terms;
        if (merged) {
            chain_encoder_tail(m, cb, false, nullptr, 0, B, nullptr, s);
            if (m->cfg.enc_final != AAE_FINAL_LINEAR) { ChainOp& f = cb.add(cop(COP_FINAL_FWD, 2, 2, c)); f.aux = m->cfg.enc_final; }
            for (int i = 0; i < cb.P.nops; ++i) {
                ChainOp& o = cb.P.ops[i];
                o.row_lo = B;
                if (o.kind == COP_LOAD || o.out) o.out_row0 = -B;
            }
        }
        ChainOp& l = cb.add(cop(COP_PRIOR, 0, 0, c)); l.one_col = c;
        l.W = m->zin.p; l.ldw = m->ldz; l.row_split = B; l.aux = m->cfg.prior;
        l.scale = m->cfg.has_prior_scale ? m->cfg.prior_scale : 1.0f;
        l.grow0 = m->rng_row0;
        l.aux_ptr = m->cfg.rng_mode == AAE_RNG_DEVICE ? nullptr : const_cast<float*>(I.z_real_dev); l.aux_ld = c;
        cop_out(l, m->zin.p, m->ldz);
        if (merged) l.fake_slot = 2;
        ChainOp& d1 = cb.add(cop_fwd(m, P_D1, 0, 1, c + 1, h, CEPI_DROPACT, s));
        d1.d = make_drop(m, 0, true, I.masks_dev[4], I.masks_dev[6], B, h, 4); d1.one_col = h; cop_out(d1, m->xh1.p, m->ldh);
        ChainOp& d2 = cb.add(cop_fwd(m, P_D2, 1, 2, h + 1, h, CEPI_DROPACT, s));
        d2.d = make_drop(m, 1, true, I.masks_dev[5], I.masks_dev[7], B, h, 5); d2.one_col = h; cop_out(d2, m->xh2.p, m->ldh);
        ChainOp& x3 = cb.add(cop_linear(COP_DISC_HEAD, 2, 5, m->P[P_D3], h + 1, h, CEPI_ACTBWD)); x3.yslot = 2; x3.d = d2.d;
        x3.aux = 0; x3.row_split = B; x3.scale = m->grad_scale; x3.aux_ptr = m->ga3.p; x3.aux_ld = 4;
        cop_out(x3, m->gb0.p, m->ldh);
        ChainOp& x2 = cb.add(cop_dx(m, P_D2, 5, 6, h, h, CEPI_ACTBWD, s)); x2.yslot = 1; x2.d = d1.d;
        cop_out(x2, m->gb1.p, m->ldh);
        TRY(launch_chain(m, cb, s));
    }
    DwBuilder dw;
    dw.add(m, m->ga3.p, 4, m->xh2.p, m->ldh, 2 * B, P_D3, O_DISC);
    dw.add(m, m->gb0.p, m->ldh, m->xh1.p, m->ldh, 2 * B, P_D2, O_DISC);
    dw.add(m, m->gb1.p, m->ldh, m->zin.p, m->ldz, 2 * B, P_D1, O_DISC);
    dw.add_loss(m, 2 * B, 1);
    return dw.launch(s);
}

int chain_gen_step(aae_model* m, hipStream_t s) {
    const int B = m->rows, h = m->h, c = m->c;
    const aae_rng_inject& I = m->inj;
    ChainBuilder cb(m, B);
    cb.beside_deferred(m);
    cb.P.loss_slot = 2; cb.P.loss_terms = m->adv_terms;
    cb.add(cop_load(m->a1.p, m->ldh, 0, h));
    ChainOp& e1 = cb.add(cop(COP_DROPACT, 0, 1, h));
    e1.d = make_drop(m, 0, true, I.masks_dev[8], nullptr, B, h, 8); e1.one_col = h; cop_out(e1, m->eh1.p, m->ldh);
    ChainOp& e2 = cb.add(cop_fwd(m, P_W2, 1, 2, h + 1, h, CEPI_DROPACT, s));
    e2.d = make_drop(m, 1, true, I.masks_dev[9], nullptr, B, h, 9); e2.one_col = h; cop_out(e2, m->eh2.p, m->ldh);
    ChainOp& l3 = cb.add(cop_fwd(m, P_W3, 2, 3, h + 1, c, CEPI_NONE, s));
    ChainOp& f = m->cfg.enc_final == AAE_FINAL_LINEAR ? l3 : cb.add(cop(COP_FINAL_FWD, 3, 3, c));
    f.aux = m->cfg.enc_final; f.one_col = c;
    ChainOp& d1 = cb.add(cop_fwd(m, P_D1, 3, 4, c + 1, h, CEPI_DROPACT, s));
    d1.d = make_drop(m, 0, true, I.masks_dev[10], nullptr, B, h, 10); d1.one_col = h;
    ChainOp& d2 = cb.add(cop_fwd(m, P_D2, 4, 5, h + 1, h, CEPI_DROPACT, s));
    d2.d = make_drop(m, 1, true, I.masks_dev[11], nullptr, B, h, 11); d2.one_col = h;
    ChainOp& x3 = cb.add(cop_linear(COP_DISC_HEAD, 5, 8, m->P[P_D3], h + 1, h, CEPI_ACTBWD)); x3.yslot = 5; x3.d = d2.d;
    x3.aux = 1; x3.row_split = B; x3.scale = m->grad_scale;
    ChainOp& x2 = cb.add(cop_dx(m, P_D2, 8, 9, h, h, CEPI_ACTBWD, s)); x2.yslot = 4; x2.d = d1.d;
    ChainOp& dz = cb.add(cop_dx(m, P_D1, 9, 0, h, c, CEPI_NONE, s));
    int sg = 6;
    if (m->cfg.enc_final == AAE_FINAL_LINEAR) {
        cop_out(dz, m->ga3.p, m->ldz); sg = 0;
    } else {
        ChainOp& fb = cb.add(cop(COP_FINAL_BWD, 0, 6, c)); fb.yslot = 3; fb.aux = m->cfg.enc_final;
        cop_out(fb, m->ga3.p, m->ldz);
    }
    ChainOp& w3 = cb.add(cop_dx(m, P_W3, sg, 7, c, h, CEPI_ACTBWD, s)); w3.yslot = 2; w3.d = e2.d;
    cop_out(w3, m->gb2.p, m->ldh);
    ChainOp& w2 = cb.add(cop_dx(m, P_W2, 7, 8, h, h, CEPI_ACTBWD, s)); w2.yslot = 1; w2.d = e1.d;
    cop_out(w2, ga1_ptr(m), m->ldh);
    TRY(launch_chain(m, cb, s));
    DwBuilder dw;
    dw.add(m, m->ga3.p, m->ldz, m->eh2.p, m->ldh, B, P_W3, O_GEN);
    dw.add(m, m->gb2.p, m->ldh, m->eh1.p, m->ldh, B, P_W2, O_GEN);
    TRY(dw.add_first_layer(m, ga1_ptr(m), O_GEN, s));
    dw.add_loss(m, B, 2);
    const bool mark_end = m->early_enabled && m->pf_this_step && m->w1_items_merged && !m->ext_first && m->side && m->ev_end &&
                          (m->rows > 16 * kMB || m->early_any);
    bool marked = false;
    TRY(dw.launch(s, mark_end ? m->ev_end : nullptr, &marked));
    m->end_marked = marked;
    if (m->ext_first && !m->own_first) return AAE_OK;
    return encoder_first_layer_update(m, m->gb3.p, O_GEN, s, true);
}

}
```

### aae-recommender_amd/csrc/abi_layers.h

```cpp
#pragma once

namespace {

static inline int gmode(const aae_model* m) { return m->bf16 ? kGemmBf16 : m->x3_gemm ? kGemmX3 : kGemmF32; }
template <class Epi>
int linear_fwd(const float* X, int ldx, int rows, const Ten& Wa, const Epi& epi, hipStream_t s, int bf = 0) {
    GemmShape g{X, Wa.p, rows, (int)Wa.rows, (int)Wa.cols, ldx, (int)Wa.ld, r4((int)Wa.cols) + 16};
    g.k_per_split = ((int)Wa.cols + 63) / 64 * 64;
    if (Wa.rows > 4096) (void)launch_gemm_mode<0, 1, true>(bf, g, epi, 1, s);
    else (void)launch_gemm_mode<0, 1, false>(bf, g, epi, 1, s);
    LAUNCHCHK("linear_fwd");
    return AAE_OK;
}
template <class Epi>
int linear_dx(const float* Gd, int ldg, int rows, const Ten& Wa, int n_in, const Epi& epi, hipStream_t s, int bf = 0) {
    GemmShape g{Gd, Wa.p, rows, n_in, (int)Wa.rows, ldg, (int)Wa.ld, 0};
    g.k_per_split = ((int)Wa.rows + 63) / 64 * 64;
    (void)launch_gemm_mode<0, 0, false>(bf, g, epi, 1, s);
    LAUNCHCHK("linear_dx");
    return AAE_OK;
}
int linear_dw(aae_model* m, const float* Gd, int ldg, int rows, const float* X, int ldx, int pid, int which,
              hipStream_t s) {
    const Ten& W = m->P[pid];
    GemmShape g{Gd, X, (int)W.rows, (int)W.cols, rows, ldg, ldx, 0};
    g.k_per_split = (rows + 63) / 64 * 64;
    const bool big = W.rows > 4096;
    const int bf = pid == P_V3 ? gmode(m) : kGemmF32;
    if (m->cfg.grad_mode == AAE_GRAD_EXPORT) {
        EpiStore e; e.out = m->Gr[pid].p; e.ld = (int)W.ld;
        if (big) (void)launch_gemm_mode<1, 0, true>(bf, g, e, 1, s); else (void)launch_gemm_mode<1, 0, false>(bf, g, e, 1, s);
    } else {
        const int set = (which == O_GEN) ? 1 : 0;
        EpiAdam e; e.p = W.p; e.m = m->M[set][pid].p; e.v = m->V[set][pid].p; e.ld = (int)W.ld; e.sc = m->sc + which;
        m->pt_ok[pid] = false;
        if (big) (void)launch_gemm_mode<1, 0, true>(bf, g, e, 1, s); else (void)launch_gemm_mode<1, 0, false>(bf, g, e, 1, s);
    }
    LAUNCHCHK("linear_dw");
    return AAE_OK;
}

int set_batch(aae_model* m, const aae_batch* b) {
    if (!b || !b->indptr_dev || !b->indices_dev || !b->values_dev) return fail(AAE_EINVAL, "batch pointers are NULL");
    if (b->n_rows < 1 || b->n_rows > m->R) return fail(AAE_EINVAL, "batch n_rows outside [1, max_batch]");
    if (b->nnz_bound > m->cfg.max_nnz) return fail(AAE_EINVAL, "batch nnz_bound > max_nnz");
    m->bv.indptr = b->indptr_dev; m->bv.indices = b->indices_dev; m->bv.values = b->values_dev;
    m->bv.rows = b->rows_dev; m->bv.row_start = b->row_start; m->bv.n_rows = b->n_rows;
    m->rows = b->n_rows; m->have_batch = true; m->buckets_valid = false; m->item_lists_valid = false; m->w1_merged = false;
    {
        int mr = b->max_row_nnz > 0 ? b->max_row_nnz : 1024;
        m->chunks = std::max(1, std::min(64, (mr + 15) / 16));
    }
    return AAE_OK;
}

int lazy_prepare(aae_model* m, int upto_off, bool bump, hipStream_t s) {
    if (bump) hipLaunchKernelGGL(bump_stamp_kernel, dim3(1), dim3(1), 0, s, m->stamp, m->ucount);
    int gy = std::max(1, std::min(16, m->chunks / 16 + 1));
    hipLaunchKernelGGL(uniq_items_kernel, dim3(m->rows, gy), dim3(256), 0, s, m->bv, m->mark, m->stamp, m->ulist,
                       m->ucount);
    LAUNCHCHK("uniq_items");
    if (m->cfg.optimizer == AAE_OPT_ADAM) {
        int grid = std::min(m->cfg.max_nnz, std::max(256, m->rows * 32));
        hipLaunchKernelGGL(w1_catchup_kernel, dim3(grid), dim3(256), 0, s, m->ulist, m->ucount, m->N, m->tsync,
                           m->P[P_W1T].p, m->M[0][P_W1T].p, m->V[0][P_W1T].p, m->M[1][P_W1T].p, m->V[1][P_W1T].p,
                           m->ldw1, m->h, m->tab, m->step_ctr, upto_off);
        LAUNCHCHK("w1_catchup");
    }
    return AAE_OK;
}

int lazy_flush(aae_model* m, hipStream_t s) {
    if (!m->lazy || m->cfg.optimizer != AAE_OPT_ADAM) return AAE_OK;
    hipLaunchKernelGGL(w1_catchup_kernel, dim3(std::min(m->N, 8192)), dim3(256), 0, s, (const int*)nullptr,
                       (const int*)nullptr, m->N, m->tsync, m->P[P_W1T].p, m->M[0][P_W1T].p, m->V[0][P_W1T].p,
                       m->M[1][P_W1T].p, m->V[1][P_W1T].p, m->ldw1, m->h, m->tab, m->step_ctr, 0);
    LAUNCHCHK("w1_catchup all");
    return AAE_OK;
}

int encoder_forward(aae_model* m, bool train, const uint8_t* mk1, const uint8_t* mk2, uint32_t sid1, uint32_t sid2,
                    bool reuse_a1, float* z_dst, int ldz_dst, hipStream_t s) {
    const int B = m->rows, h = m->h;
    DropSpec d1 = make_drop(m, 0, train, mk1, nullptr, B, h, sid1);
    DropSpec d2 = make_drop(m, 1, train, mk2, nullptr, B, h, sid2);
    if (!reuse_a1) {
        ProfScope ps(m, AAE_K_ENC_GATHER, s);
        size_t shm = (size_t)16 * r4(h) * sizeof(float);
        hipLaunchKernelGGL(enc_gather_kernel, dim3(B), dim3(1024), shm, s, m->bv, m->P[P_W1T].p, m->ldw1,
                           m->P[P_B1].p, h, m->cfg.normalize_inputs, m->a1.p, m->eh1.p, m->ldh, m->cfg.activation,
                           d1, m->cfg.seed, m->step_ctr, m->rscale, m->doc_l1, AdvanceJob{nullptr, nullptr, nullptr, nullptr, 0},
                           (long long)-1);
        LAUNCHCHK("enc_gather");
    } else {
        hipLaunchKernelGGL(drop_act_kernel, dim3(grid1d((size_t)B * h)), dim3(256), 0, s, m->a1.p, m->eh1.p, B, h,
                           m->ldh, m->cfg.activation, d1, m->cfg.seed, m->step_ctr);
        LAUNCHCHK("drop_act");
    }
    EpiDropAct e2; e2.out = m->eh2.p; e2.ld = m->ldh; e2.act = m->cfg.activation; e2.d = d2; e2.seed = m->cfg.seed;
    e2.step_ctr = m->step_ctr;
    TRY(linear_fwd(m->eh1.p, m->ldh, B, m->P[P_W2], e2, s, gmode(m)));
    EpiStore e3; e3.out = z_dst; e3.ld = ldz_dst;
    TRY(linear_fwd(m->eh2.p, m->ldh, B, m->P[P_W3], e3, s, gmode(m)));
    if (m->cfg.enc_final != AAE_FINAL_LINEAR) {
        hipLaunchKernelGGL(final_act_fwd_kernel, dim3((B + 3) / 4), dim3(256), 0, s, z_dst, B, m->c, ldz_dst,
                           m->cfg.enc_final, (float*)nullptr, 0);
        LAUNCHCHK("final_act_fwd");
    }
    return AAE_OK;
}

int launch_w1_items(aae_model* m, const float* ga1, int rpb, size_t bstride, int which, hipStream_t s);
W1Items w1_items_args(aae_model* m, const float* ga1, int rpb, size_t bstride, int which);
int ensure_buckets(aae_model* m, hipStream_t s);

int encoder_backward(aae_model* m, const float* gz, int ldgz, const float* z, int ldzz, const uint8_t* mk1,
                     const uint8_t* mk2, uint32_t sid1, uint32_t sid2, int which, hipStream_t s) {
    const int B = m->rows, h = m->h, cc = m->c;
    DropSpec d1 = make_drop(m, 0, true, mk1, nullptr, B, h, sid1);
    DropSpec d2 = make_drop(m, 1, true, mk2, nullptr, B, h, sid2);
    const float* ga3 = gz; int ldga3 = ldgz;
    if (m->cfg.enc_final != AAE_FINAL_LINEAR) {
        hipLaunchKernelGGL(final_act_bwd_kernel, dim3((B + 3) / 4), dim3(256), 0, s, z, ldzz, gz, ldgz, m->ga3.p,
                           m->ldz, B, cc, m->cfg.enc_final);
        LAUNCHCHK("final_act_bwd");
        ga3 = m->ga3.p; ldga3 = m->ldz;
    }
    EpiActBwd b2; b2.out = m->gb0.p; b2.ld = m->ldh; b2.y = m->eh2.p; b2.ldy = m->ldh; b2.act = m->cfg.activation;
    b2.d = d2; b2.seed = m->cfg.seed; b2.step_ctr = m->step_ctr;
    TRY(linear_dx(ga3, ldga3, B, m->P[P_W3], h, b2, s, gmode(m)));
    TRY(linear_dw(m, ga3, ldga3, B, m->eh2.p, m->ldh, P_W3, which, s));
    EpiActBwd b1; b1.out = m->gb1.p; b1.ld = m->ldh; b1.y = m->eh1.p; b1.ldy = m->ldh; b1.act = m->cfg.activation;
    b1.d = d1; b1.seed = m->cfg.seed; b1.step_ctr = m->step_ctr;
    TRY(linear_dx(m->gb0.p, m->ldh, B, m->P[P_W2], h, b1, s, gmode(m)));
    TRY(linear_dw(m, m->gb0.p, m->ldh, B, m->eh1.p, m->ldh, P_W2, which, s));
    const int set = (which == O_GEN) ? 1 : 0;
    const bool exportg = m->cfg.grad_mode == AAE_GRAD_EXPORT;
    hipLaunchKernelGGL(colsum_adam_kernel, dim3((h + 63) / 64), dim3(1024), 0, s, m->gb1.p, B, h, m->ldh,
                       m->P[P_B1].p, m->M[set][P_B1].p, m->V[set][P_B1].p, exportg ? m->Gr[P_B1].p : (float*)nullptr,
                       m->sc + which);
    LAUNCHCHK("colsum_adam");
    return launch_w1_items(m, m->gb1.p, 0, 0, which, s);
}

int disc_forward(aae_model* m, int rows, const uint8_t* m1a, const uint8_t* m1b, const uint8_t* m2a,
                 const uint8_t* m2b, int split, uint32_t sid1, uint32_t sid2, hipStream_t s) {
    const int h = m->h;
    DropSpec d1 = make_drop(m, 0, true, m1a, m1b, split, h, sid1);
    DropSpec d2 = make_drop(m, 1, true, m2a, m2b, split, h, sid2);
    EpiDropAct e1; e1.out = m->xh1.p; e1.ld = m->ldh; e1.act = m->cfg.activation; e1.d = d1; e1.seed = m->cfg.seed;
    e1.step_ctr = m->step_ctr;
    TRY(linear_fwd(m->zin.p, m->ldz, rows, m->P[P_D1], e1, s, gmode(m)));
    EpiDropAct e2 = e1; e2.out = m->xh2.p; e2.d = d2;
    TRY(linear_fwd(m->xh1.p, m->ldh, rows, m->P[P_D2], e2, s, gmode(m)));
    EpiSigmoid e3; e3.out = m->dout.p; e3.ld = 4;
    TRY(linear_fwd(m->xh2.p, m->ldh, rows, m->P[P_D3], e3, s));
// ... 37 lines not shown
```

### aae-recommender_amd/csrc/abi_model.h

```cpp
#pragma once

static thread_local std::string g_err;
static int fail(int code, const std::string& msg) { g_err = msg; return code; }

#define HIPCHK(expr)                                                                        \
    do {                                                                                    \
        hipError_t e_ = (expr);                                                             \
        if (e_ != hipSuccess)                                                               \
            return fail(AAE_EHIP, std::string(#expr) + ": " + hipGetErrorString(e_));       \
    } while (0)
#define LAUNCHCHK(what)                                                                     \
    do {                                                                                    \
        hipError_t e_ = hipGetLastError();                                                  \
        if (e_ != hipSuccess) return fail(AAE_EHIP, std::string(what) + ": " + hipGetErrorString(e_)); \
    } while (0)
#define TRY(expr) do { int rc_ = (expr); if (rc_ != AAE_OK) return rc_; } while (0)

namespace {

inline int r4(int x) { return (x + 3) & ~3; }

struct Ten {
    float* p = nullptr; size_t off = 0; int64_t rows = 0, cols = 0, ld = 0;
    size_t floats() const { return (size_t)rows * ld; }
};

enum { P_W1T = 0, P_B1, P_W2, P_W3, P_V1, P_V2, P_V3, P_D1, P_D2, P_D3, NP };
enum { O_ENC = 0, O_DEC = 1, O_GEN = 2, O_DISC = 3 };

}

struct aae_options {
    bool no_chain;
    bool chain16;
    bool split_any;
    bool blocked_any;
    bool early_any;
    bool no_late_join;
    bool no_item_lists;
    bool no_item_count;
    bool w1_serial;
    bool no_rank_fused;
    bool chain_kslices;
    int x16_rows;
    int rank_collect_cap;
    int dw_ksplit_rows;
    char dec_ts[8];
    bool chain_ts;
    int dw_ts;
    int dec_skip, chain_skip, rank_skip;
};
const char* option_value(const char* name);
inline void read_options(aae_options& o) {
    auto on = [](const char* n) { return option_value(n) != nullptr; };
    auto num = [](const char* n, int dflt) { const char* e = option_value(n); return e ? atoi(e) : dflt; };
    o.no_chain = on("NO_CHAIN"); o.chain16 = on("CHAIN16"); o.split_any = on("SPLIT_ANY"); o.blocked_any = on("BLOCKED_ANY");
    o.early_any = on("EARLY_ANY"); o.no_late_join = on("NO_LATE_JOIN"); o.no_item_count = on("NO_ITEM_COUNT");
    o.no_item_lists = on("NO_ITEM_LISTS");
    o.w1_serial = on("W1_SERIAL"); o.no_rank_fused = on("NO_RANK_FUSED"); o.chain_kslices = on("CHAIN_KSLICES");
    o.x16_rows = num("X16_ROWS", 1024); o.dw_ksplit_rows = num("DW_KSPLIT_ROWS", -1);
    o.rank_collect_cap = std::max(0, std::min(num("RANK_COLLECT_CAP", 0), 4096));
    const char* ts = option_value("DEC_TS");
    snprintf(o.dec_ts, sizeof(o.dec_ts), "%s", ts ? ts : "");
    o.chain_ts = on("CHAIN_TS"); o.dw_ts = num("DW_TS", -1);
    o.dec_skip = num("DEC_SKIP", 0); o.chain_skip = num("CHAIN_SKIP", 0); o.rank_skip = num("RANK_SKIP", 0);
}

struct aae_model {
    aae_config cfg;
    aae_options opt;
    char* base; size_t bytes;
    int N, h, c, cp, R, R2;
    int ldh, ldw1, ldc, ldz, ldn;
    bool alpha_mode;
    float grad_scale;
    int rng_row0, rng_global;
    Ten P[NP], M[2][NP], V[2][NP], Gr[NP];
    unsigned short* FXi[NP]; unsigned short* DXi[NP]; unsigned short* FXBi[NP];
    bool x16_ok; int x16_rows;
    Ten PT[NP]; Ten D4[NP]; bool pt_ok[NP];
    Ten a1, eh1, eh2, zc, dh1, dh2, G, slabs, gb0, gb1, gb2, gb3, gzc, ga3, zin, xh1, xh2, dout, zsave, da2;
    Ten ga1x;
    const float* doc_l1;
    bool ext_first;
    bool own_first;
    bool ae_only;
    bool vae;
    bool bf16;
    bool vae_cut;
    Ten mulv, gmulv, veps;
    bool use_chain;
    bool use_chain4;
    bool act_nm;
    bool dec_hidden_done;
    bool enc_bwd_done;
    int max_slabs;
    float* bce_partials; int bce_partials_cap;
    float* fix_partials;
    float* rscale;
    bool w1_merged;
    bool w1_items_merged;
    bool buckets_valid;
    unsigned* il_rec[2]; unsigned* il_ovf[2]; int* il_hot_count; int il_cap, il_hot_cap, il_set;
    bool item_lists_valid;
    bool lazy;
    int n_cu; bool fused_ok; int fused_nb; bool force_unfused;
    int* tcount; int* tstart; int* teb; int* ten; float* tev;
    int* tstart2; int* teb2; int* ten2; float* tev2;
    int* tsync; int* mark; int* ulist; int* ucount; int* stamp; LazyTab* tab;
    int* hot_list = nullptr; int* hot_count = nullptr; int hot_cap = 0, hot_flip = 0;
    bool w1_hot_pending = false; int w1_hot_set = 0, w1_hot_which = 0; const float* w1_hot_ga1 = nullptr;
    int* pslot; int* ptag;
    int chunks;
    float* losses;
    float* adv_terms;
    OptScalars* sc;
    long long* step_ctr;
    BatchView bv; bool have_batch; int rows; int phase;
    aae_rng_inject inj;
    bool prof_on; unsigned prof_mask;
    std::vector<std::pair<hipEvent_t, hipEvent_t>>* prof_ev;
    size_t prof_used[AAE_K_N];
    bool split_ok; int split_wgs; bool opt_pending;
    hipStream_t side; hipEvent_t ev_crit, ev_opt;
    bool bf16_one = false;
    bool bf16_x3 = false;
    float* Gt;
    Ten Xn; const float* noise_next; int64_t noise_ld; bool dense_step;
    bool noise_gen_next; float noise_gen_scale;
    float* noise_l1;
    bool bucket_wide_ok = false;
    bool split_any = false;
    float* dp_scratch = nullptr; size_t dp_scratch_floats = 0;
    bool x3_gemm = false;
    bool x3_ok = false;
    bool w1_big_lds = false;
    bool blocked_any = false;
    Ten dh2f;
    bool blocked_ok; Ten Gacc;
    int* mark2; int* ulist2; int* ucount2; int* stamp2;
    int* cnt_host; int* cnt_host_dev;
    int dw_ksplit_rows;
    aae_batch pf_batch, pf_built_batch; bool pf_armed; bool pf_built; long long pf_step; long long hstep;
    bool pf_pending; hipEvent_t ev_head, ev_pf;
    bool pf_bumped = false;
    bool pf_after_opt = false;
    hipEvent_t ev_bk = nullptr; bool bk_pending = false;
    bool last_out_split = false;
    Ten dh2s; OptScalars* sc_snap = nullptr;
    bool late_enabled = false, late_ok = false;
    hipEvent_t ev_end = nullptr; bool end_marked = false, spec_tab_ok = false, pf_this_step = false, early_enabled = false, early_any = false;
    long long flushed_hstep = -1;
    int64_t long_stats[5] = {0, 0, 0, 0, 0};
    bool rank_ok = false;
    bool vae_rank_ok = false;
    bool side_ordered = false;
};

namespace {

struct Arena {
    char* base; size_t off = 0; bool dry;
    float* take(size_t nfloats, size_t* off_out) {
        off = (off + 255) & ~(size_t)255;
        size_t o = off; off += nfloats * sizeof(float);
        if (off_out) *off_out = o;
        return dry ? nullptr : reinterpret_cast<float*>(base + o);
    }
    Ten mat(int64_t rows, int64_t cols, int64_t ld, int64_t pad_rows = 0) {
        Ten t; t.rows = rows; t.cols = cols; t.ld = ld;
        t.p = take((size_t)(rows + pad_rows) * ld, &t.off);
        return t;
    }
};

constexpr int kRowBlock = 104, kMaxRowBlocks = 16;

inline bool fused_width_ok(int h, int ldh) {
    return (h + 1 + 15) / 16 <= 13 && ldh <= 256 && (ldh % 4) == 0 && ldh <= kSD - 2;
}

constexpr int kVaeInParts = 5, kVaeDecInMax = kVaeInParts * kCWide;
static_assert(kVaeDecInMax == 1040, "validate()'s message, include/aaerec_hip.h, README.md and aaerec/vae.py name this bound");
int validate(const aae_config* c) {
    if (!c) return fail(AAE_EINVAL, "cfg is NULL");
    if (c->abi_version != AAE_ABI_VERSION) return fail(AAE_EINVAL, "abi_version mismatch");
    if (c->n_items < 1 || c->n_hidden < 1 || c->n_code < 1 || c->cond_inc < 0)
        return fail(AAE_EINVAL, "n_items/n_hidden/n_code must be positive");
    if (c->n_hidden > 4096) return fail(AAE_EINVAL, "n_hidden > 4096 not supported");
    if (c->max_batch < 1 || c->max_nnz < 1) return fail(AAE_EINVAL, "max_batch/max_nnz must be positive");
    if (c->max_batch > 16384) return fail(AAE_EINVAL, "max_batch > 16384 not supported");
    if (c->activation < 0 || c->activation >= AAE_ACT_COUNT) return fail(AAE_EINVAL, "unknown activation");
    if (c->enc_final < 0 || c->enc_final > AAE_FINAL_SIGMOID) return fail(AAE_EINVAL, "unknown enc_final");
    if (c->optimizer != AAE_OPT_ADAM && c->optimizer != AAE_OPT_SGD) return fail(AAE_EINVAL, "unknown optimizer");
    if (c->rng_mode != AAE_RNG_INJECT && c->rng_mode != AAE_RNG_DEVICE) return fail(AAE_EINVAL, "unknown rng_mode");
    if (c->grad_mode != AAE_GRAD_FUSED && c->grad_mode != AAE_GRAD_EXPORT) return fail(AAE_EINVAL, "unknown grad_mode");
    if (!(c->dropout1 >= 0.f && c->dropout1 < 1.f && c->dropout2 >= 0.f && c->dropout2 < 1.f))
        return fail(AAE_EINVAL, "dropout must be in [0,1)");
    if (c->reserved[0] || c->reserved[1]) return fail(AAE_EINVAL, "reserved fields must be zero");
    if (c->dense_noise != 0 && c->dense_noise != 1) return fail(AAE_EINVAL, "dense_noise must be 0 or 1 (dense noisy encoder input)");
    if (c->dense_noise == 1 && (c->model_kind != 1 || c->grad_mode != AAE_GRAD_FUSED || c->dtype != 0))
        return fail(AAE_EINVAL, "dense_noise = 1 (dense noisy encoder input) needs the plain autoencoder (model_kind = 1), fp32, fused optimiser");
    if (c->blocked_output != 0 && c->blocked_output != 1) return fail(AAE_EINVAL, "blocked_output must be 0 or 1 (row-blocked fused output layer)");
    if (c->dtype != 0 && c->dtype != 1) return fail(AAE_EINVAL, "dtype must be 0 (fp32) or 1 (bf16 matrix-core inputs)");
    if (c->dtype == 1 && c->model_kind == 3) return fail(AAE_EINVAL, "bf16 arithmetic is not available in VAE mode");
    if (c->model_kind < 0 || c->model_kind > 3 || c->model_kind == 2)
        return fail(AAE_EINVAL, "model_kind must be 0 (AAE), 1 (plain autoencoder) or 3 (VAE)");
    if (c->model_kind == 3 && (c->n_hidden + 1 > 208 || c->n_code + c->cond_inc + 1 > kVaeDecInMax || 2 * c->n_code > 208))
        return fail(AAE_EINVAL, "VAE mode needs n_hidden <= 207, n_code + cond_inc + 1 <= 1040 (the decoder input in up to five parts of 208 columns), 2 * n_code <= 208");
    if (c->dp_world < 0 || c->dp_world > 64) return fail(AAE_EINVAL, "dp_world (data-parallel world size) out of range");
    if (c->unfused_decoder != 0 && c->unfused_decoder != 1) return fail(AAE_EINVAL, "unfused_decoder must be 0 or 1");
    return AAE_OK;
}


size_t layout(aae_model* m, char* base, bool dry) {
    const aae_config& c = m->cfg;
    m->N = c.n_items; m->h = c.n_hidden; m->c = c.n_code; m->cp = c.n_code + c.cond_inc;
    m->R = c.max_batch; m->R2 = 2 * c.max_batch;
    m->ldh = r4(m->h + 1); m->ldw1 = r4(m->h); m->ldc = r4(m->cp + 1); m->ldz = r4(m->c + 1); m->ldn = r4(m->N);
    Arena a{base, 0, dry};
    const int N = m->N, h = m->h, cc = m->c, cp = m->cp;
    m->P[P_W1T] = a.mat(N, h, m->ldw1);
    m->P[P_B1] = a.mat(1, h, m->ldw1);
    m->P[P_W2] = a.mat(h, h + 1, m->ldh, 16);
    m->P[P_W3] = a.mat(c.model_kind == 3 ? 2 * cc : cc, h + 1, m->ldh, 16);
    m->P[P_V1] = a.mat(h, cp + 1, m->ldc, 16);
    m->P[P_V2] = a.mat(h, h + 1, m->ldh, 16);
// ... 238 lines not shown
```

### aae-recommender_amd/csrc/abi_step_open.h

```cpp
#pragma once

namespace {

void remember_inject(aae_model* m, const aae_rng_inject* inj, bool reset) {
    if (inj) m->inj = *inj;
    else if (reset) memset(&m->inj, 0, sizeof(m->inj));
}

int launch_advance(aae_model* m, hipStream_t s, bool ahead = false) {
    hipLaunchKernelGGL(advance_step_kernel, dim3(1), dim3(64), 0, s, m->sc, m->step_ctr, m->lazy ? m->tab : nullptr,
                       ahead ? (int*)nullptr : m->stamp, ahead ? (int*)nullptr : m->ucount, m->losses);
    LAUNCHCHK("advance_step");
    return AAE_OK;
}

int open_step_plain(aae_model* m, const aae_batch* batch, const aae_rng_inject* inj, hipStream_t s) {
    TRY(set_batch(m, batch));
    remember_inject(m, inj, true);
    TRY(join_deferred(m, s));
    m->hstep++; m->pf_armed = false;
    TRY(launch_advance(m, s));
    m->enc_bwd_done = false;
    return AAE_OK;
}
// ... 2 lines not shown
    const bool ahead = m->pf_built && m->pf_step == m->hstep && same_batch(m->pf_built_batch, *batch) && m->lazy;
    m->pf_built = false;
    if (ahead) { std::swap(m->mark, m->mark2); std::swap(m->ulist, m->ulist2); std::swap(m->ucount, m->ucount2); std::swap(m->stamp, m->stamp2); }
    return ahead;
}

int stage_cond(aae_model* m, const float* cond_dev, hipStream_t s) {
    if (m->cfg.cond_inc <= 0) return AAE_OK;
    hipLaunchKernelGGL(copy2d_kernel, dim3(grid1d((size_t)m->rows * m->cfg.cond_inc)), dim3(256), 0, s, cond_dev,
                       m->cfg.cond_inc, m->zc.p + m->c, m->ldc, m->rows, m->cfg.cond_inc, 1.0f);
    LAUNCHCHK("copy cond");
    return AAE_OK;
}

}

extern "C" {

static int ae_encode_impl(aae_handle m, const aae_batch* batch, const aae_rng_inject* inj, float* z_out, bool with_dec,
                          const float* cond_dev, void* stream) {
    if (!m) return fail(AAE_EINVAL, "handle is NULL");
    TRY(set_batch(m, batch));
    remember_inject(m, inj, true);
    hipStream_t s = S(stream);
    TRY(join_step_open(m, s));
    m->hstep++;
    const bool ahead = take_lists_built_ahead(m, batch);
    const bool end_marked = m->end_marked, spec_ok = m->spec_tab_ok;
    m->end_marked = false; m->pf_this_step = false; m->spec_tab_ok = m->lazy;
    const bool noise_gen = m->noise_gen_next; const float noise_gen_scale = m->noise_gen_scale; m->noise_gen_next = false;
    const bool fold_advance = ahead && m->use_chain && !m->ext_first && m->noise_next == nullptr && !noise_gen;
    if (!fold_advance) TRY(launch_advance(m, s, ahead));
    m->dense_step = m->noise_next != nullptr || noise_gen;
    const float* noise = m->noise_next; m->noise_next = nullptr;
    if (m->dense_step) {
        if (!m->use_chain) return fail(AAE_ESTATE, "the dense noisy input needs the layer-chain kernels");
        if (m->lazy && m->cfg.optimizer == AAE_OPT_ADAM) {
            hipLaunchKernelGGL(w1_catchup_kernel, dim3(std::min(m->N, 8192)), dim3(256), 0, s, (const int*)nullptr,
                               (const int*)nullptr, m->N, m->tsync, m->P[P_W1T].p, m->M[0][P_W1T].p, m->V[0][P_W1T].p,
                               m->M[1][P_W1T].p, m->V[1][P_W1T].p, m->ldw1, m->h, m->tab, m->step_ctr, -1);
            LAUNCHCHK("w1_catchup all");
        }
        hipLaunchKernelGGL(uniq_items_kernel, dim3(m->rows, std::max(1, std::min(16, m->chunks / 16 + 1))), dim3(256), 0, s, m->bv,
                           m->mark, m->stamp, m->ulist, m->ucount);
        if (noise_gen) TRY(launch_dense_noise_gen(m, noise_gen_scale, s));
        else {
        hipLaunchKernelGGL(dense_input_kernel, dim3(m->rows), dim3(1024), 0, s, m->bv, noise, m->noise_ld, m->N,
                           (int)m->cfg.normalize_inputs, m->Xn.p, m->ldn);
        LAUNCHCHK("dense_input");
        }
        const int B = m->rows, h = m->h, N = m->N;
        int splits;
        const int kps = split_k_items(m, B, &splits);
        GemmShape g{m->Xn.p, m->P[P_W1T].p, B, h, N, m->ldn, m->ldw1, kps};
        EpiSlab e; e.out = m->slabs.p; e.ld = m->ldh; e.slab_stride = (size_t)m->R * m->ldh;
        (void)launch_gemm_mode<0, 0, true>(gmode(m), g, e, splits, s);
        LAUNCHCHK("dense first layer");
        DropSpec d1 = make_drop(m, 0, true, m->inj.masks_dev[0], nullptr, B, h, 0);
        hipLaunchKernelGGL(slab_reduce_fwd_kernel, dim3(grid1d((size_t)B * h)), dim3(256), 0, s, m->slabs.p, splits,
                           e.slab_stride, B, h, m->ldh, m->P[P_B1].p, m->a1.p, m->eh1.p, (int)m->cfg.activation, d1,
                           (uint64_t)m->cfg.seed, m->step_ctr);
        LAUNCHCHK("slab_reduce_fwd");
        m->dec_hidden_done = false; m->enc_bwd_done = false;
        TRY(chain_ae_forward(m, with_dec, cond_dev, z_out, s));
        m->phase = 1;
        m->pf_armed = false;
        return AAE_OK;
    }
    if (m->ext_first) {
        if (!m->use_chain || m->vae) return fail(AAE_ESTATE, "an external first layer needs the layer-chain kernels (and no VAE mode)");
        m->dec_hidden_done = false; m->enc_bwd_done = false; m->pf_armed = false;
        TRY(chain_ae_forward(m, with_dec, cond_dev, z_out, s));
        m->phase = 1;
        return AAE_OK;
    }
    if (m->lazy && !ahead) TRY(lazy_prepare(m, -1, false, s));
    m->dec_hidden_done = false; m->enc_bwd_done = false;
    if (m->side && m->ev_bk && m->last_out_split && m->rows > 16 * kMB && !m->buckets_valid && fused_decoder_applies(m))
        TRY(build_tile_buckets_aside(m));
    const bool pf = m->pf_armed && m->side && m->mark2 && m->lazy && m->use_chain;
    if (m->pf_armed && !pf) m->pf_armed = false;
    if (m->use_chain) {
        const bool early = pf && ahead && end_marked && spec_ok && m->early_enabled && (m->rows > 16 * kMB || m->early_any);
        if (early) TRY(launch_prefetch(m, true, true));
        TRY(gather_first_layer(m, true, m->inj.masks_dev[0], 0, s, pf && !early, fold_advance));
        if (pf && !early) TRY(launch_prefetch(m));
        TRY(chain_ae_forward(m, with_dec, cond_dev, z_out, s));
        m->phase = 1;
        return AAE_OK;
    }
    TRY(encoder_forward(m, true, m->inj.masks_dev[0], m->inj.masks_dev[1], 0, 1, false, m->zc.p, m->ldc, s));
    hipLaunchKernelGGL(copy2d_kernel, dim3(grid1d((size_t)m->rows * m->c)), dim3(256), 0, s, m->zc.p, m->ldc,
                       m->zsave.p, m->ldz, m->rows, m->c, 1.0f);
    if (z_out)
        hipLaunchKernelGGL(copy2d_kernel, dim3(grid1d((size_t)m->rows * m->c)), dim3(256), 0, s, m->zc.p, m->ldc,
                           z_out, m->c, m->rows, m->c, 1.0f);
    LAUNCHCHK("ae_encode copies");
    m->phase = 1;
    return AAE_OK;
}

int aae_ae_encode(aae_handle m, const aae_batch* batch, const aae_rng_inject* inj, float* z_out, void* stream) {
    return ae_encode_impl(m, batch, inj, z_out, false, nullptr, stream);
}


}
```

### aae-recommender_amd/csrc/abi_step_phases.h

```cpp
#pragma once

extern "C" {

int aae_decoder_step(aae_handle m, const aae_batch* batch, const float* zin_dev, int64_t zin_ld,
                     const aae_rng_inject* inj, float* dzin_out, void* stream) {
    if (!m) return fail(AAE_EINVAL, "handle is NULL");
    if (!zin_dev) return fail(AAE_EINVAL, "zin_dev is NULL");
    if (zin_ld < m->cp) return fail(AAE_EINVAL, "zin_ld < n_code + cond_inc");
    hipStream_t s = S(stream);
    TRY(open_step_plain(m, batch, inj, s));
    m->dec_hidden_done = false;
    m->phase = 1;
    TRY(decode_backward(m, zin_dev, zin_ld, nullptr, dzin_out, DecodeMode{}, s));
    m->phase = 0;
    return AAE_OK;
}

int aae_vae_step(aae_handle m, const aae_batch* batch, const float* cond_dev, const float* eps_dev, void* stream) {
    if (!m) return fail(AAE_EINVAL, "handle is NULL");
    if (!m->vae) return fail(AAE_ESTATE, "model was not created in VAE mode (cfg.model_kind = 3)");
    if (!m->use_chain) return fail(AAE_ESTATE, "VAE mode needs the layer-chain kernels");
    if (m->cfg.cond_inc > 0 && !cond_dev) return fail(AAE_EINVAL, "cond_inc > 0 needs cond_dev");
    if (m->cfg.rng_mode == AAE_RNG_INJECT && !eps_dev) return fail(AAE_EINVAL, "rng_mode inject needs eps_dev");
    hipStream_t s = S(stream);
// ... 206 lines not shown
    const float pscale = m->cfg.has_prior_scale ? m->cfg.prior_scale : 1.0f;
    if (m->cfg.rng_mode != AAE_RNG_DEVICE && !I.z_real_dev) return fail(AAE_EINVAL, "rng_mode=inject needs z_real_dev");
    if (!m->use_chain) {
        if (m->cfg.rng_mode == AAE_RNG_DEVICE) {
            hipLaunchKernelGGL(prior_kernel, dim3(grid1d((size_t)B * cc)), dim3(256), 0, s, m->zin.p, m->ldz, B, cc,
                               m->cfg.prior, pscale, m->cfg.seed, m->step_ctr, m->rng_row0);
        } else {
            hipLaunchKernelGGL(copy2d_kernel, dim3(grid1d((size_t)B * cc)), dim3(256), 0, s, I.z_real_dev, cc, m->zin.p,
                               m->ldz, B, cc, pscale);
        }
        LAUNCHCHK("prior");
    }
    if (m->use_chain) {
        TRY(chain_disc_step(m, s));
        m->phase = 4;
        return AAE_OK;
    }
    TRY(encoder_forward(m, false, nullptr, nullptr, 0, 0, false, m->zin.p + (size_t)B * m->ldz, m->ldz, s));
    TRY(disc_forward(m, 2 * B, I.masks_dev[4], I.masks_dev[6], I.masks_dev[5], I.masks_dev[7], B, 4, 5, s));
    hipLaunchKernelGGL(adv_loss_kernel, dim3(1), dim3(256), 0, s, m->dout.p, 4, B, 0, m->grad_scale, m->ga3.p, 4,
                       m->losses, 1);
    LAUNCHCHK("adv_loss disc");
    {
        DropSpec d1 = make_drop(m, 0, true, I.masks_dev[4], I.masks_dev[6], B, h, 4);
        DropSpec d2 = make_drop(m, 1, true, I.masks_dev[5], I.masks_dev[7], B, h, 5);
        EpiActBwd b2; b2.out = m->gb0.p; b2.ld = m->ldh; b2.y = m->xh2.p; b2.ldy = m->ldh; b2.act = m->cfg.activation;
        b2.d = d2; b2.seed = m->cfg.seed; b2.step_ctr = m->step_ctr;
        TRY(linear_dx(m->ga3.p, 4, 2 * B, m->P[P_D3], h, b2, s));
        TRY(linear_dw(m, m->ga3.p, 4, 2 * B, m->xh2.p, m->ldh, P_D3, O_DISC, s));
        EpiActBwd b1 = b2; b1.out = m->gb1.p; b1.y = m->xh1.p; b1.d = d1;
        TRY(linear_dx(m->gb0.p, m->ldh, 2 * B, m->P[P_D2], h, b1, s, gmode(m)));
        TRY(linear_dw(m, m->gb0.p, m->ldh, 2 * B, m->xh1.p, m->ldh, P_D2, O_DISC, s));
        TRY(linear_dw(m, m->gb1.p, m->ldh, 2 * B, m->zin.p, m->ldz, P_D1, O_DISC, s));
    }
    m->phase = 4;
    return AAE_OK;
}

int aae_gen_step(aae_handle m, const aae_rng_inject* inj, void* stream) {
    if (!m) return fail(AAE_EINVAL, "handle is NULL");
    if (m->phase != 4) return fail(AAE_ESTATE, "aae_gen_step before aae_disc_step");
    remember_inject(m, inj, false);
    hipStream_t s = S(stream);
    const int B = m->rows, h = m->h, cc = m->c;
    const aae_rng_inject& I = m->inj;
    if (m->use_chain) {
        TRY(chain_gen_step(m, s));
        m->phase = 0;
        return AAE_OK;
    }
    TRY(encoder_forward(m, true, I.masks_dev[8], I.masks_dev[9], 8, 9, true, m->zin.p, m->ldz, s));
    hipLaunchKernelGGL(copy2d_kernel, dim3(grid1d((size_t)B * cc)), dim3(256), 0, s, m->zin.p, m->ldz, m->zsave.p,
                       m->ldz, B, cc, 1.0f);
    TRY(disc_forward(m, B, I.masks_dev[10], nullptr, I.masks_dev[11], nullptr, B, 10, 11, s));
    hipLaunchKernelGGL(adv_loss_kernel, dim3(1), dim3(256), 0, s, m->dout.p, 4, B, 1, m->grad_scale, m->ga3.p, 4,
                       m->losses, 2);
    LAUNCHCHK("adv_loss gen");
    {
        DropSpec d1 = make_drop(m, 0, true, I.masks_dev[10], nullptr, B, h, 10);
        DropSpec d2 = make_drop(m, 1, true, I.masks_dev[11], nullptr, B, h, 11);
        EpiActBwd b2; b2.out = m->gb0.p; b2.ld = m->ldh; b2.y = m->xh2.p; b2.ldy = m->ldh; b2.act = m->cfg.activation;
        b2.d = d2; b2.seed = m->cfg.seed; b2.step_ctr = m->step_ctr;
        TRY(linear_dx(m->ga3.p, 4, B, m->P[P_D3], h, b2, s));
        EpiActBwd b1 = b2; b1.out = m->gb1.p; b1.y = m->xh1.p; b1.d = d1;
        TRY(linear_dx(m->gb0.p, m->ldh, B, m->P[P_D2], h, b1, s, gmode(m)));
        EpiStore ez; ez.out = m->gzc.p; ez.ld = m->ldc;
        TRY(linear_dx(m->gb1.p, m->ldh, B, m->P[P_D1], cc, ez, s, gmode(m)));
    }
    TRY(encoder_backward(m, m->gzc.p, m->ldc, m->zsave.p, m->ldz, I.masks_dev[8], I.masks_dev[9], 8, 9, O_GEN, s));
    m->phase = 0;
    return AAE_OK;
}

int aae_disc_gen(aae_handle m, const aae_rng_inject* inj, void* stream) {
    TRY(aae_disc_step(m, inj, stream));
    return aae_gen_step(m, nullptr, stream);
}

int aae_step(aae_handle m, const aae_batch* batch, const float* cond_dev, const aae_rng_inject* inj, void* stream) {
    if (!m) return fail(AAE_EINVAL, "handle is NULL");
    if (m->ext_first) return fail(AAE_ESTATE, "aae_step: the first layer is external (aae_set_first_layer_external): drive the phases");
    if (m->cfg.cond_inc > 0 && !cond_dev) return fail(AAE_EINVAL, "cond_inc > 0 needs cond_dev");
    hipStream_t s = S(stream);
    TRY(ae_encode_impl(m, batch, inj, nullptr, true, cond_dev, stream));
    TRY(stage_cond(m, cond_dev, s));
    DecodeMode mode; mode.enc_too = true;
    TRY(decode_backward(m, nullptr, 0, nullptr, nullptr, mode, s));
    TRY(aae_ae_encoder_backward(m, nullptr, 0, stream));
    if (!m->ae_only) TRY(aae_disc_gen(m, nullptr, stream));
    return AAE_OK;
}

int aae_read_losses(aae_handle m, float out[3], void* stream) {
    if (!m || !out) return fail(AAE_EINVAL, "handle/out is NULL");
    float tmp[4];
    HIPCHK(hipMemcpyAsync(tmp, m->losses, sizeof(tmp), hipMemcpyDeviceToHost, S(stream)));
    HIPCHK(hipStreamSynchronize(S(stream)));
    out[0] = tmp[0]; out[1] = tmp[1]; out[2] = tmp[2];
    return AAE_OK;
}


}
```

### aae-recommender_amd/csrc/chain.h

```cpp
#pragma once
#include "device_common.h"
#include "gemm_f32.h"
#include "kernels.h"
#include "buckets.h"
#include "w1_update.h"
#include "w1_lists.h"

namespace aae {

constexpr int kCR = 16;
constexpr int kCL = 212;
constexpr int kCSlots = 10;
constexpr int kCWide = 208;
constexpr int kCT = 1024;
constexpr int kCW = kCT / 64;
constexpr int kCQ = (13 + kCW - 1) / kCW;
constexpr int kTPR = kCT / 16;
constexpr int kRS = kCT == 1024 ? 6 : 5;
constexpr int kJ = 64 / kTPR;
constexpr int kCMaxOps = 16;

enum { COP_LOAD = 0,
       COP_LINEAR,
       COP_LINEAR_DX,
       COP_FINAL_FWD,
       COP_FINAL_BWD,
       COP_ADV,
       COP_DROPACT,
       COP_SLABSUM,
       COP_ACTBWD,
       COP_STORE,
       COP_REPARAM,
       COP_REPARAM_BWD,
       COP_DISC_HEAD,
       COP_PRIOR };

enum { CEPI_NONE = 0, CEPI_DROPACT = 1, CEPI_ACTBWD = 2, CEPI_SIGMOID = 3 };

struct ChainOp {
    int kind, src, dst, K, N;
    const float* W; int ldw;
    const float* Wkn; int ldkn;
    const float* W4; int ns4;
    const unsigned short* WX; int xpl;
    int x16_next_lin[2];
    int epi, yslot;
    DropSpec d;
    float* out; int ldo; int out_row0;
    float* out2; int ldo2;
    int one_col;
    int aux;
    size_t stride;
    float scale;
    int row_split;
    int dst_col0;
    float* aux_ptr; int aux_ld;
    int grow0;
    int row_lo;
    int fake_slot;
    const float* y_glb; int y_ld;
    int acc_in;
};

struct ChainProgram {
    int nops, rows, act;
    uint64_t seed; const long long* step_ctr;
    float* loss_out; int loss_slot;
    float* loss_terms;
    int dbg;
    unsigned long long* ts;
    BucketJob bk;
    int x16_first_lin[2], x16_row_lo;
    ChainOp ops[kCMaxOps];
    int kslices;
    ItemListJob il;
};

__device__ __forceinline__ void chain_barrier() { asm volatile("s_waitcnt lgkmcnt(0)\n\ts_barrier" ::: "memory"); }

template <class T> __device__ __forceinline__ T chain_pin(T v) { asm volatile("" : "+s"(v)); return v; }

struct EpiCtx {
    int epi, act, den, drng, split, width, goa, gob;
    uint32_t thr;
    uint64_t dkey;
    float mk, ak, ad;
    const uint8_t* ma; const uint8_t* mb;
    const float* y;
};

__device__ __forceinline__ EpiCtx chain_epi_ctx(int epi, const ChainOp& op, const ChainProgram& P, uint64_t key,
                                                const float* slots) {
    EpiCtx c;
    c.epi = epi; c.act = P.act;
    c.den = op.d.enabled; c.drng = op.d.device_rng;
    c.split = op.d.split_row; c.width = op.d.width;
    c.goa = op.d.goff_a; c.gob = op.d.goff_b;
    c.thr = op.d.keep_threshold;
    uint64_t sid = op.d.stream_id;
    c.mk = op.d.mul_keep; c.ak = op.d.add_keep; c.ad = op.d.add_drop;
    c.ma = op.d.mask_a; c.mb = op.d.mask_b;
    int ys = op.yslot;
    asm volatile("" : "+s"(c.epi), "+s"(c.act), "+s"(c.den), "+s"(c.drng), "+s"(c.split), "+s"(c.width), "+s"(c.goa), "+s"(c.gob), "+s"(c.thr));
    asm volatile("" : "+s"(sid), "+s"(c.mk), "+s"(c.ak), "+s"(c.ad), "+s"(c.ma), "+s"(c.mb), "+s"(ys));
    c.dkey = key ^ (sid * 0xA0761D6478BD642Full);
    c.y = slots + ys * kCR * kCL;
    return c;
}

__device__ __forceinline__ int chain_keep(const EpiCtx& c, int row, int col) {
    if (c.drng) return hash_cell(c.dkey, (uint32_t)(row + (row < c.split ? c.goa : c.gob)), (uint32_t)col) >= c.thr;
    typedef const __attribute__((address_space(1))) uint8_t* gmask_t;
    gmask_t m = (gmask_t)(row < c.split ? c.ma : c.mb);
    if (!m) return 1;
    const int r = row < c.split ? row : row - c.split;
    return m[(size_t)r * c.width + col] != 0;
}

template <bool NM = false>
__device__ __forceinline__ float chain_epi(const EpiCtx& c, int grow, int lrow, int col, float v) {
    if (c.epi == CEPI_DROPACT) {
        if (c.den) v = chain_keep(c, grow, col) ? v * c.mk + c.ak : c.ad;
        return act_fwd<NM>(c.act, v);
    }
    if (c.epi == CEPI_ACTBWD) {
        v *= act_grad_from_y<NM>(c.act, c.y[lrow * kCL + col]);
        if (c.den) v *= chain_keep(c, grow, col) ? c.mk : 0.f;
        return v;
    }
    if (c.epi == CEPI_SIGMOID) return sigmoidf_(v);
    return v;
}

__device__ __forceinline__ void chain_load_block(const float* __restrict__ g, int ld, int row0, int nrows, int N,
                                                 float* dst, int dst_col0, float scale) {
    const int tid = threadIdx.x, lrow = tid >> kRS;
    const bool vec = (ld & 3) == 0 && (dst_col0 & 3) == 0 && ((reinterpret_cast<uintptr_t>(g) & 15) == 0);
    const int rowc = min(lrow, max(nrows, 1) - 1);
    const int nf4 = (N + 3) >> 2;
    if (vec) {
        float4 v[2];
#pragma unroll
        for (int j = 0; j < kJ; ++j) {
            const int c4 = min((tid & (kTPR - 1)) + kTPR * j, nf4 - 1);
            v[j] = *reinterpret_cast<const float4*>(g + (size_t)(row0 + rowc) * ld + c4 * 4);
        }
#pragma unroll
        for (int j = 0; j < kJ; ++j) {
            const int c4 = (tid & (kTPR - 1)) + kTPR * j;
            if (c4 * 4 + dst_col0 < kCL) {
                const bool ok = lrow < nrows;
                float4 o;
                o.x = (ok && c4 * 4 + 0 < N) ? v[j].x * scale : 0.f;
                o.y = (ok && c4 * 4 + 1 < N) ? v[j].y * scale : 0.f;
                o.z = (ok && c4 * 4 + 2 < N) ? v[j].z * scale : 0.f;
                o.w = (ok && c4 * 4 + 3 < N) ? v[j].w * scale : 0.f;
                *reinterpret_cast<float4*>(dst + lrow * kCL + dst_col0 + c4 * 4) = o;
            }
// ... 659 lines not shown
```

### aae-recommender_amd/csrc/chain4.h

```cpp
#pragma once
#include "chain.h"

namespace aae {

constexpr int kR4 = 4;
#ifndef C4_WAVES
#define C4_WAVES 16
#endif
constexpr int kC4W = C4_WAVES;
constexpr int kC4WS = kC4W == 16 ? 4 : 3;
constexpr int kC4T = 64 * kC4W;
constexpr int kC4E = 1024 / kC4T;
constexpr int kC4ER = kC4T / 256;
constexpr int kC4Part = 4096;

__device__ __forceinline__ float chain4_rb(float x) {
    return __builtin_bit_cast(float, gemm_pack_bf16(x, 0.f) << 16);
}

struct Lin4 { int N, K, ldkn, ns4; const float* W4; const float* Wkn; };

template <int MK, bool BF, bool TS = false>
__device__ __forceinline__ void chain4_linear(const Lin4& op, const float* src, float* part, int wave, int lane,
                                              int cgs, int kper, unsigned long long* wts_ = nullptr) {
// ... 61 lines not shown
    }
    f32x4 acc0 = (f32x4){0.f, 0.f, 0.f, 0.f}, acc1 = acc0;
    const float* a = src + (lane & 3) * kCL;
    if (wts && lane == 0) wts[wave] = wall_clock64();
    const int klim = min(min(K, k0 + kper), kCL);
#ifdef C4_NO_A
    auto ldx = [&](int j) { return make_float4(1.f + j, 2.f, 3.f, 4.f + lane); };
#else
    auto ldx = [&](int j) { return *reinterpret_cast<const float4*>(a + min(k0 + 4 * j, kCL - 4)); };
#endif
    float4 xn = ldx(0);
#pragma unroll
    for (int j = 0; j < MK / 4; ++j) {
        if (wts && j == 1 && lane == 0) { asm volatile("s_nop 0" :: "v"(acc0[0])); wts[16 + wave] = wall_clock64(); }
        const int kk = k0 + 4 * j;
        float4 x = xn;
        if (j + 1 < MK / 4) xn = ldx(j + 1);
        if (kk >= klim) continue;
        if (kk + 4 > klim) {
            x.y = kk + 1 < klim ? x.y : 0.f;
            x.z = kk + 2 < klim ? x.z : 0.f;
            x.w = 0.f;
        }
        float w0 = w[4 * j], w1 = w[4 * j + 1], w2 = w[4 * j + 2], w3 = w[4 * j + 3];
        if (BF) {
            x.x = chain4_rb(x.x); x.y = chain4_rb(x.y); x.z = chain4_rb(x.z); x.w = chain4_rb(x.w);
            w0 = chain4_rb(w0); w1 = chain4_rb(w1); w2 = chain4_rb(w2); w3 = chain4_rb(w3);
        }
#ifdef C4_NO_MFMA
        acc0[0] += x.x * w0; acc1[0] += x.y * w1; acc0[1] += x.z * w2; acc1[1] += x.w * w3;
#else
        acc0 = __builtin_amdgcn_mfma_f32_4x4x1f32(x.x, w0, acc0, 0, 0, 0);
        acc1 = __builtin_amdgcn_mfma_f32_4x4x1f32(x.y, w1, acc1, 0, 0, 0);
        acc0 = __builtin_amdgcn_mfma_f32_4x4x1f32(x.z, w2, acc0, 0, 0, 0);
        acc1 = __builtin_amdgcn_mfma_f32_4x4x1f32(x.w, w3, acc1, 0, 0, 0);
#endif
    }
    acc0 += acc1;
    float* pp = part + (size_t)ks * (4 * 64 * cgp) + 64 * cg + lane;
#pragma unroll
#ifndef C4_NO_PART
    for (int r = 0; r < 4; ++r) pp[r * 64 * cgp] = acc0[r];
#else
    if (acc0[0] == 12345.f) pp[0] = acc0[1];
#endif
    if (wts && lane == 0) wts[32 + wave] = wall_clock64();
}

template <int NJ>
__device__ __forceinline__ f32x4 chain4_cols(const float* W4, int ns4, int N, int K, const float* src, int wave, int lane) {
    const int kq = lane >> 4, col = min(16 * wave + (lane & 15), N - 1);
    const unsigned st = (unsigned)ns4 * 16u;
    const __amdgpu_buffer_rsrc_t rw = __builtin_amdgcn_make_buffer_rsrc(const_cast<float*>(W4), 0, (unsigned)(((K + 3) >> 2) + kW4Pad) * st, 0x00020000);
    const unsigned vo = (unsigned)col * 16u + (unsigned)kq * st;
    unsigned so = 0;
    float4 wq[NJ];
#pragma unroll
    for (int j = 0; j < NJ; ++j) { wq[j] = __builtin_bit_cast(float4, __builtin_amdgcn_raw_buffer_load_b128(rw, vo, so, 0)); so += 4u * st; }
    __builtin_amdgcn_sched_barrier(0);
    const float4* a4 = reinterpret_cast<const float4*>(src + (lane & 3) * kCL + 4 * kq);
    f32x4 c0 = (f32x4){0.f, 0.f, 0.f, 0.f}, c1 = c0;
#pragma unroll
    for (int j = 0; j < NJ; ++j) {
        const float4 x = a4[4 * j];
        c0 = __builtin_amdgcn_mfma_f32_4x4x1f32(chain4_rb(x.x), chain4_rb(wq[j].x), c0, 0, 0, 0);
        c1 = __builtin_amdgcn_mfma_f32_4x4x1f32(chain4_rb(x.y), chain4_rb(wq[j].y), c1, 0, 0, 0);
        c0 = __builtin_amdgcn_mfma_f32_4x4x1f32(chain4_rb(x.z), chain4_rb(wq[j].z), c0, 0, 0, 0);
        c1 = __builtin_amdgcn_mfma_f32_4x4x1f32(chain4_rb(x.w), chain4_rb(wq[j].w), c1, 0, 0, 0);
    }
    c0 += c1;
#pragma unroll
    for (int r = 0; r < 4; ++r) {
        const auto a = __builtin_amdgcn_permlane16_swap(__float_as_uint(c0[r]), __float_as_uint(c0[r]), false, false);
        const float y = __uint_as_float(a[0]) + __uint_as_float(a[1]);
        const auto b = __builtin_amdgcn_permlane32_swap(__float_as_uint(y), __float_as_uint(y), false, false);
        c0[r] = __uint_as_float(b[0]) + __uint_as_float(b[1]);
    }
    return c0;
}

template <bool BF, bool TS = false, bool COLS = false, bool VAE = false>
__global__ __launch_bounds__(kC4T) void chain4_kernel(ChainProgram P) {
    extern __shared__ __attribute__((aligned(16))) float slots[];
    const int il_blocks = P.il.enabled ? P.il.nblocks : 0;
    if ((int)blockIdx.x >= (int)gridDim.x - il_blocks) {
        w1_lists_build_body<kC4T>(P.il, reinterpret_cast<unsigned*>(slots), (int)blockIdx.x - ((int)gridDim.x - il_blocks), il_blocks);
        return;
    }
    if (P.bk.enabled && (int)blockIdx.x == (int)gridDim.x - 1 - il_blocks) {
        tile_bucket_body<kBucketMaxDocs, kC4T>(P.bk.bv, P.bk.ntiles, P.bk.tstart, P.bk.eb, P.bk.en, P.bk.ev, reinterpret_cast<int*>(slots));
        return;
    }
    float* part = slots + kCSlots * kR4 * kCL;
    const int tid = threadIdx.x, lane = tid & 63;
    const int wave = __builtin_amdgcn_readfirstlane(tid >> 6);
    const int erow0 = tid >> 8, ecol = tid & 255;
    const int r0 = blockIdx.x * kR4;
    const int nrows = min(kR4, P.rows - r0);
    const uint64_t key = rng_key(P.seed, (uint64_t)*P.step_ctr, 0);

    unsigned long long* tsp = (TS && blockIdx.x == 0) ? P.ts : nullptr;
    int nops = P.nops, kslices = COLS ? P.kslices : 1;
    asm volatile("" : "+s"(tsp), "+s"(nops));
    if constexpr (COLS) asm volatile("" : "+s"(kslices));
    for (int oi = 0; oi < nops; ++oi) {
        const ChainOp& op = P.ops[oi];
        if (TS && tsp && tid == 0) tsp[oi] = wall_clock64();
        int kind = op.kind, src_i = op.src, dst_i = op.dst, row_lo = op.row_lo, one_col = op.one_col, opN = op.N, opK = op.K;
        int ldo = op.ldo, ldo2 = op.ldo2, out_row0 = op.out_row0;
        float* outp = op.out; float* out2p = op.out2;
        Lin4 lin; lin.N = opN; lin.K = opK; lin.ldkn = op.ldkn; lin.ns4 = op.ns4; lin.W4 = op.W4; lin.Wkn = op.Wkn;
        int epi_k = op.epi, yslot_k = op.yslot, acc_in = op.acc_in;
        asm volatile("" : "+s"(kind), "+s"(src_i), "+s"(dst_i), "+s"(row_lo), "+s"(one_col), "+s"(opN), "+s"(opK), "+s"(ldo), "+s"(ldo2),
                          "+s"(out_row0), "+s"(outp), "+s"(out2p), "+s"(epi_k), "+s"(yslot_k), "+s"(acc_in));
        const float* ygp = op.y_glb; int yld = op.y_ld;
        asm volatile("" : "+s"(lin.ldkn), "+s"(lin.ns4), "+s"(lin.W4), "+s"(lin.Wkn), "+s"(ygp), "+s"(yld));
        lin.N = opN; lin.K = opK;
        if (r0 < row_lo) continue;
        float* dst = slots + dst_i * kR4 * kCL;
        const float* src = slots + src_i * kR4 * kCL;

        const float* qW = nullptr; float* qaux_ptr = nullptr; size_t qstride = 0;
        int qldw = 0, qdst_col0 = 0, qaux = 0, qaux_ld = 0, qyslot = 0, qgrow0 = 0, qrow_split = 0, qfake_slot = -1;
        float qscale = 0.f;
        if (kind != COP_LINEAR && kind != COP_LINEAR_DX) {
            qW = op.W; qaux_ptr = op.aux_ptr; qstride = op.stride; qldw = op.ldw; qdst_col0 = op.dst_col0; qaux = op.aux;
            qaux_ld = op.aux_ld; qyslot = op.yslot; qgrow0 = op.grow0; qrow_split = op.row_split; qfake_slot = op.fake_slot; qscale = op.scale;
            asm volatile("" : "+s"(qW), "+s"(qaux_ptr), "+s"(qstride), "+s"(qldw), "+s"(qdst_col0), "+s"(qaux), "+s"(qaux_ld), "+s"(qyslot),
                              "+s"(qgrow0), "+s"(qrow_split), "+s"(qfake_slot), "+s"(qscale));
        }
        bool one_done = false;
        if (kind == COP_LINEAR || kind == COP_LINEAR_DX) {
            const int N = opN, K = opK;
            const int CG = (N + 63) >> 6;
            const int cgs = CG <= 1 ? 0 : CG <= 2 ? 1 : 2, cgp = 1 << cgs;
            const int KS = kC4W >> cgs;
            const int kper = (((K + KS - 1) >> (kC4WS - cgs)) + 3) & ~3;
            unsigned long long* wts = (TS && tsp && oi == 2) ? tsp + 64 : nullptr;
            if (wts && tid == 0) { wts[48] = wall_clock64(); wts[49] = clock64(); }
            bool cols_ok = false;
            if constexpr (BF && COLS && kC4W == 16) cols_ok = !kslices && lin.W4 && K <= kCWide && N <= 16 * kC4W && src_i != dst_i;
            if (cols_ok) {
                const int crow = lane >> 4, ccol = 16 * wave + (lane & 15);
                float yv1 = 0.f;
                if (ygp) {
                    typedef const __attribute__((address_space(1))) float* gf_t;
                    yv1 = (ccol < N && crow < nrows) ? ((gf_t)ygp)[(size_t)(r0 + crow) * yld + ccol] : 0.f;
                }
                f32x4 cs = (f32x4){0.f, 0.f, 0.f, 0.f};
                if (16 * wave < N) {
                    if (K <= 64) cs = chain4_cols<4>(lin.W4, lin.ns4, N, K, src, wave, lane);
                    else if (K <= 112) cs = chain4_cols<7>(lin.W4, lin.ns4, N, K, src, wave, lane);
                    else cs = chain4_cols<13>(lin.W4, lin.ns4, N, K, src, wave, lane);
                }
                if (wts && lane == 0) wts[32 + wave] = wall_clock64();
                one_done = true;
                if (16 * wave < kCL) {
                    const EpiCtx ec = chain_epi_ctx(epi_k, op, P, key, slots);
                    float v = 0.f;
                    if (ccol < N && crow < nrows) {
                        v = crow == 0 ? cs[0] : crow == 1 ? cs[1] : crow == 2 ? cs[2] : cs[3];
                        if (acc_in) v += dst[crow * kCL + ccol];
                        if (ec.epi == CEPI_ACTBWD) {
                            v *= act_grad_from_y<false>(ec.act, ygp ? yv1 : (slots + yslot_k * kR4 * kCL)[crow * kCL + ccol]);
                            if (ec.den) v *= chain_keep(ec, r0 + crow, ccol) ? ec.mk : 0.f;
                        } else {
                            v = chain_epi<false>(ec, r0 + crow, crow, ccol, v);
                        }
                    }
                    if (ccol < kCL) dst[crow * kCL + ccol] = ccol == one_col ? (crow < nrows ? 1.f : 0.f) : v;
                }
            } else {
// ... 248 lines not shown
```

### aae-recommender_amd/csrc/kernels.h

```cpp
#pragma once
#include "device_common.h"
#include "gemm_f32.h"

namespace aae {

struct BatchView {
    const int64_t* indptr; const int32_t* indices; const float* values;
    const int32_t* rows; int row_start; int n_rows;
    __device__ __forceinline__ int doc(int b) const { return rows ? rows[b] : row_start + b; }
};

constexpr int kLazyReplay = 128;
constexpr int kLazyTabCap = 65536;

struct LazyTab { float nss_gen, nss_reg, ibc2, pad; };

struct AdvanceJob { OptScalars* sc; long long* ctr; LazyTab* tab; float* losses; int enabled;
                    int* stamp2 = nullptr; int* ucount2 = nullptr; };
__device__ __forceinline__ void advance_step_body(OptScalars* sc, long long* ctr, LazyTab* tab, int* stamp, int* ucount,
                                                  float* losses, int i) {
    if (i == 0) { *ctr += 1; if (stamp) { *stamp += 1; *ucount = 0; } losses[1] = 0.f; losses[2] = 0.f; }
    if (i >= 4) return;
    OptScalars s = sc[i];
    s.t += 1;
// ... 444 lines not shown
        for (int j = lane; j < c; j += 64) mx = fmaxf(mx, zr[j]);
        for (int o = 32; o > 0; o >>= 1) mx = fmaxf(mx, __shfl_xor(mx, o, 64));
        float sum = 0.f;
        for (int j = lane; j < c; j += 64) sum += expf(zr[j] - mx);
        sum = wave_sum(sum);
        for (int j = lane; j < c; j += 64) zr[j] = expf(zr[j] - mx) / sum;
    } else if (kind == 2) {
        for (int j = lane; j < c; j += 64) zr[j] = sigmoidf_(zr[j]);
    }
    if (copy_out)
        for (int j = lane; j < c; j += 64) copy_out[(size_t)r * ld_copy + j] = zr[j];
}

__global__ void final_act_bwd_kernel(const float* __restrict__ z, int ldz, const float* __restrict__ gz, int ldg,
                                     float* __restrict__ ga, int lda, int rows, int c, int kind) {
    int r = blockIdx.x * (blockDim.x >> 6) + (threadIdx.x >> 6), lane = threadIdx.x & 63;
    if (r >= rows) return;
    const float* zr = z + (size_t)r * ldz;
    const float* gr = gz + (size_t)r * ldg;
    float* o = ga + (size_t)r * lda;
    if (kind == 1) {
        float dot = 0.f;
        for (int j = lane; j < c; j += 64) dot += gr[j] * zr[j];
        dot = wave_sum(dot);
        for (int j = lane; j < c; j += 64) o[j] = zr[j] * (gr[j] - dot);
    } else if (kind == 2) {
        for (int j = lane; j < c; j += 64) o[j] = gr[j] * zr[j] * (1.f - zr[j]);
    } else {
        for (int j = lane; j < c; j += 64) o[j] = gr[j];
    }
}

__global__ void copy2d_kernel(const float* __restrict__ src, int lds_, float* __restrict__ dst, int ldd, int rows,
                              int cols, float scale) {
    for (int i = blockIdx.x * blockDim.x + threadIdx.x; i < rows * cols; i += gridDim.x * blockDim.x) {
        int r = i / cols, c = i - r * cols;
        dst[(size_t)r * ldd + c] = src[(size_t)r * lds_ + c] * scale;
    }
}

__global__ void fill_col_kernel(float* dst, int ld, int rows, int col, float v) {
    int r = blockIdx.x * blockDim.x + threadIdx.x;
    if (r < rows) dst[(size_t)r * ld + col] = v;
}

__global__ void prior_kernel(float* __restrict__ z, int ld, int rows, int c, int prior, float scale, uint64_t seed,
                             const long long* step_ctr, int grow0) {
    const uint64_t k = rng_key(seed, (uint64_t)*step_ctr, 0) ^ (100ull * 0xA0761D6478BD642Full);
    for (int i = blockIdx.x * blockDim.x + threadIdx.x; i < rows * c; i += gridDim.x * blockDim.x) {
        int r = i / c, j = i - r * c;
        const uint32_t gr = (uint32_t)(r + grow0);
        float v = 0.f;
        if (prior == 0) v = draw_gauss(k, gr, j) * scale;
        else if (prior == 1) v = draw_class(k, gr, c) == j ? scale : 0.f;
        z[(size_t)r * ld + j] = v;
    }
}

__global__ __launch_bounds__(256) void adv_loss_kernel(const float* __restrict__ dout, int ldo, int B, int mode,
                                                       float gscale, float* __restrict__ ga, int lda,
                                                       float* losses, int slot) {
    __shared__ double red[256];
    double acc = 0.0;
    const float invB = 1.f / (float)B;
    const int rows = mode == 0 ? 2 * B : B;
    for (int r = threadIdx.x; r < rows; r += 256) {
        float dv = dout[(size_t)r * ldo];
        float g, l;
        if (mode == 0 && r >= B) { l = logf(1.f - dv + kTiny); g = invB / (1.f - dv + kTiny); }
        else { l = logf(dv + kTiny); g = -invB / (dv + kTiny); }
        ga[(size_t)r * lda] = g * dv * (1.f - dv) * gscale;
        acc += (double)l;
    }
    red[threadIdx.x] = acc;
    __syncthreads();
    for (int o = 128; o > 0; o >>= 1) {
        if (threadIdx.x < o) red[threadIdx.x] += red[threadIdx.x + o];
        __syncthreads();
    }
    if (threadIdx.x == 0) losses[slot] = (float)(-red[0] / (double)B);
}


__global__ __launch_bounds__(256) void uniq_items_kernel(BatchView bv, int* __restrict__ mark,
                                                         const int* __restrict__ stamp_p, int* __restrict__ ulist,
                                                         int* __restrict__ ucount) {
    const int b = blockIdx.x;
    const int dc = bv.doc(b);
    const int64_t lo = bv.indptr[dc], hi = bv.indptr[dc + 1];
    const int stamp = *stamp_p;
    for (int64_t e = lo + (int64_t)blockIdx.y * 256 + threadIdx.x; e < hi; e += (int64_t)gridDim.y * 256) {
        const int idx = bv.indices[e];
        if (atomicExch(&mark[idx], stamp) != stamp) ulist[atomicAdd(ucount, 1)] = idx;
    }
}

__device__ __forceinline__ void lazy_replay(float& p, float& m1, float& v1, float& m3, float& v3, int t0, int upto,
                                            const LazyTab* stab) {
    const int n = upto - t0;
    const int nl = n < kLazyReplay ? n : kLazyReplay;
    for (int j = 1; j <= nl; ++j) {
        const LazyTab T = stab[j - 1];
        m1 = m1 + 0.1f * (0.f - m1);
        v1 = v1 * 0.999f;
        p = p + (T.nss_gen * m1) * __builtin_amdgcn_rcpf(__builtin_amdgcn_sqrtf(v1) * T.ibc2 + 1e-8f);
        m3 = m3 + 0.1f * (0.f - m3);
        v3 = v3 * 0.999f;
        p = p + (T.nss_reg * m3) * __builtin_amdgcn_rcpf(__builtin_amdgcn_sqrtf(v3) * T.ibc2 + 1e-8f);
    }
    const int rest = n - nl;
    if (rest > 0) {
        const float dm = exp2f((float)rest * -0.15200309344504997f);
        const float dv = exp2f((float)rest * -0.0014434168696687186f);
        m1 *= dm; m3 *= dm; v1 *= dv; v3 *= dv;
    }
}

__global__ __launch_bounds__(256) void w1_catchup_kernel(const int* __restrict__ ulist, const int* __restrict__ ucount,
                                                         int n_rows_all, int* __restrict__ tsync,
                                                         float* __restrict__ W, float* __restrict__ M1,
                                                         float* __restrict__ V1, float* __restrict__ M3,
                                                         float* __restrict__ V3, int ld, int h,
                                                         const LazyTab* __restrict__ tab, const long long* step_ctr,
                                                         int upto_off, const int* __restrict__ skip_mark = nullptr,
                                                         const int* __restrict__ skip_stamp = nullptr, long long upto_abs = -1) {
    __shared__ LazyTab stab[kLazyReplay];
    const int upto = upto_abs >= 0 ? (int)upto_abs : (int)*step_ctr + upto_off;
    const int cnt = ulist ? *ucount : n_rows_all;
    const int skip = skip_mark ? *skip_stamp : 0;
    for (int r = blockIdx.x; r < cnt; r += gridDim.x) {
        const int row = ulist ? ulist[r] : r;
        const int t0 = (skip_mark && skip_mark[row] == skip) ? upto : tsync[row];
        if (t0 < upto) {
            const int nl = min(upto - t0, kLazyReplay);
            for (int j = threadIdx.x; j < nl; j += 256) stab[j] = tab[(t0 + 1 + j) & (kLazyTabCap - 1)];
            __syncthreads();
            for (int c = threadIdx.x; c < h; c += 256) {
                const size_t o = (size_t)row * ld + c;
                float p = W[o], m1 = M1[o], v1 = V1[o], m3 = M3[o], v3 = V3[o];
                lazy_replay(p, m1, v1, m3, v3, t0, upto, stab);
                W[o] = p; M1[o] = m1; V1[o] = v1; M3[o] = m3; V3[o] = v3;
            }
        }
        __syncthreads();
        if (threadIdx.x == 0 && t0 < upto) tsync[row] = upto;
    }
}

__global__ __launch_bounds__(256) void w1_sparse_adam_kernel(const int* __restrict__ ulist,
                                                             const int* __restrict__ ucount, float* __restrict__ W,
                                                             float* __restrict__ M, float* __restrict__ V,
                                                             float* __restrict__ G, int ld, int h, const OptScalars* sc,
                                                             int* __restrict__ tsync, const long long* step_ctr,
                                                             int mark_synced) {
    const OptScalars s = *sc;
    const int cnt = *ucount;
    for (int r = blockIdx.x; r < cnt; r += gridDim.x) {
        const int row = ulist[r];
        for (int c = threadIdx.x; c < h; c += 256) {
            const size_t o = (size_t)row * ld + c;
            float p = W[o], m = s.is_sgd ? 0.f : M[o], v = s.is_sgd ? 0.f : V[o];
            adam_update(p, m, v, G[o], s);
            W[o] = p; G[o] = 0.f;
            if (!s.is_sgd) { M[o] = m; V[o] = v; }
        }
        if (mark_synced && threadIdx.x == 0) tsync[row] = (int)*step_ctr;
    }
}

__global__ __launch_bounds__(256) void w1_pack_kernel(const int* __restrict__ ulist, const int* __restrict__ ucount,
                                                      float* __restrict__ gW1T, int ldw, int h, int cap,
                                                      int* __restrict__ hdr, float* __restrict__ vals) {
    const int cnt = min(*ucount, cap);
    if (blockIdx.x == 0 && threadIdx.x == 0) hdr[0] = (*ucount > cap) ? -1 : cnt;
    for (int r = blockIdx.x; r < cnt; r += gridDim.x) {
        const int row = ulist[r];
        if (threadIdx.x == 0) hdr[1 + r] = row;
        for (int c = threadIdx.x; c < h; c += 256) {
            vals[(size_t)r * h + c] = gW1T[(size_t)row * ldw + c];
            gW1T[(size_t)row * ldw + c] = 0.f;
        }
    }
}

__global__ __launch_bounds__(256) void w1_unpack_kernel(const int* __restrict__ hdr, const float* __restrict__ vals,
                                                        int h, float* __restrict__ gW1T, int ldw,
                                                        int* __restrict__ mark, const int* __restrict__ stamp_p,
                                                        int* __restrict__ ulist, int* __restrict__ ucount) {
    const int cnt = hdr[0];
    const int stamp = *stamp_p;
    for (int r = blockIdx.x; r < cnt; r += gridDim.x) {
        const int row = hdr[1 + r];
        for (int c = threadIdx.x; c < h; c += 256) gW1T[(size_t)row * ldw + c] += vals[(size_t)r * h + c];
        if (threadIdx.x == 0 && atomicExch(&mark[row], stamp) != stamp) ulist[atomicAdd(ucount, 1)] = row;
    }
}

template <int K>
__global__ __launch_bounds__(256) void topk_rows_kernel(float* __restrict__ scores, int ld, int n_items, BatchView bv,
                                                        int exclude_known, int k_out, int* __restrict__ idx_out,
                                                        float* __restrict__ val_out) {
    __shared__ float s_val[4]; __shared__ int s_idx[4]; __shared__ int s_who[4];
    __shared__ float s_min[4], s_max[4];
    const int row = blockIdx.x, tid = threadIdx.x, lane = tid & 63, wave = tid >> 6;
    float* sc = scores + (size_t)row * ld;
    float vmin = INFINITY, vmax = -INFINITY;
    if (exclude_known) {
        const int dc = bv.doc(row);
        const int64_t lo = bv.indptr[dc], hi = bv.indptr[dc + 1];
        for (int64_t e = lo + tid; e < hi; e += 256) {
            const int i = bv.indices[e];
            const float v = sc[i];
            vmin = fminf(vmin, v); vmax = fmaxf(vmax, v);
            sc[i] = -INFINITY;
        }
        __syncthreads();
    }
    float tv[K]; int ti[K];
#pragma unroll
    for (int j = 0; j < K; ++j) { tv[j] = -INFINITY; ti[j] = -1; }
    for (int i = tid; i < n_items; i += 256) {
        const float v = sc[i];
        if (v != -INFINITY) { vmin = fminf(vmin, v); vmax = fmaxf(vmax, v); }
        if (v > tv[K - 1]) {
            tv[K - 1] = v; ti[K - 1] = i;
#pragma unroll
            for (int j = K - 1; j > 0; --j) {
                if (tv[j] > tv[j - 1]) {
                    const float fv = tv[j]; tv[j] = tv[j - 1]; tv[j - 1] = fv;
                    const int iv = ti[j]; ti[j] = ti[j - 1]; ti[j - 1] = iv;
// ... 166 lines not shown
```

### include/aaerec_hip.h

```cpp
#ifndef AAEREC_HIP_H
#define AAEREC_HIP_H

#include <stddef.h>
#include <stdint.h>

#ifdef __cplusplus
extern "C" {
#endif

#define AAE_ABI_VERSION 4

#define AAE_OK 0
#define AAE_EINVAL (-1)
#define AAE_ENOMEM (-2)
#define AAE_EHIP (-3)
#define AAE_ESTATE (-4)

enum { AAE_ACT_RELU = 0, AAE_ACT_SELU = 1, AAE_ACT_TANH = 2, AAE_ACT_SIGMOID = 3,
       AAE_ACT_ELU = 4, AAE_ACT_LEAKYRELU = 5,
       AAE_ACT_SOFTPLUS = 6, AAE_ACT_HARDTANH = 7, AAE_ACT_RELU6 = 8, AAE_ACT_CELU = 9, AAE_ACT_SOFTSIGN = 10,
       AAE_ACT_HARDSIGMOID = 11, AAE_ACT_LOGSIGMOID = 12, AAE_ACT_SOFTSHRINK = 13, AAE_ACT_HARDSHRINK = 14,
       AAE_ACT_IDENTITY = 15,
       AAE_ACT_GELU = 16, AAE_ACT_SILU = 17, AAE_ACT_MISH = 18, AAE_ACT_HARDSWISH = 19, AAE_ACT_COUNT = 20 };
enum { AAE_FINAL_LINEAR = 0, AAE_FINAL_SOFTMAX = 1, AAE_FINAL_SIGMOID = 2 };
enum { AAE_OPT_ADAM = 0, AAE_OPT_SGD = 1 };
enum { AAE_RNG_INJECT = 0,
       AAE_RNG_DEVICE = 1 };
enum { AAE_PRIOR_GAUSS = 0, AAE_PRIOR_CATEGORICAL = 1, AAE_PRIOR_BERNOULLI = 2 };
enum { AAE_MODEL_AAE = 0,
       AAE_MODEL_AE = 1,
       AAE_MODEL_VAE = 3 };
enum { AAE_DTYPE_F32 = 0,
       AAE_DTYPE_BF16 = 1 };
enum { AAE_GRAD_FUSED = 0,
       AAE_GRAD_EXPORT = 1 };

typedef struct aae_config {
    int32_t abi_version;
    int32_t n_items;
    int32_t n_hidden;
    int32_t n_code;
    int32_t cond_inc;
    int32_t max_batch;
    int32_t max_nnz;
    int32_t activation;
    int32_t enc_final;
    int32_t optimizer;
    int32_t normalize_inputs;
    int32_t rng_mode;
    int32_t prior;
    int32_t grad_mode;
    float dropout1, dropout2;
    float gen_lr, reg_lr;
    float prior_scale;
    int32_t has_prior_scale;
    uint64_t seed;
    int32_t unfused_decoder;
    int32_t dp_world;
    int32_t model_kind;
    int32_t dtype;
    int32_t blocked_output;
    int32_t dense_noise;
    int32_t reserved[2];
} aae_config;

typedef struct aae_model* aae_handle;

typedef struct aae_batch {
    const int64_t* indptr_dev;
    const int32_t* indices_dev;
    const float* values_dev;
    const int32_t* rows_dev;
    int32_t row_start;
    int32_t n_rows;
    int32_t nnz_bound;
    int32_t max_row_nnz;
    int64_t generation;
} aae_batch;

typedef struct aae_rng_inject {
    const uint8_t* masks_dev[12];
    const float* z_real_dev;
} aae_rng_inject;

enum {
    AAE_T_ENC_W1T = 0, AAE_T_ENC_B1, AAE_T_ENC_W2, AAE_T_ENC_W3,
    AAE_T_DEC_V1, AAE_T_DEC_V2, AAE_T_DEC_V3,
    AAE_T_DISC_D1, AAE_T_DISC_D2, AAE_T_DISC_D3,
    AAE_T_N_PARAMS,
    AAE_T_ADAM_ENC = 16,
    AAE_T_ADAM_GEN = 32,
    AAE_T_ADAM_DEC = 48,
    AAE_T_ADAM_DISC = 64,
    AAE_T_GRAD = 80,
    AAE_T_ACT_Z = 96,
    AAE_T_ACT_LOSSES = 97,
    AAE_T_ACT_A1 = 98,
    AAE_T_ACT_DH2 = 100,
    AAE_T_ACT_DA2 = 101,
    AAE_T_ACT_GA1 = 102,
    AAE_T_ACT_DZC = 99
};

typedef struct aae_tensor {
    size_t byte_offset;
    int64_t rows, cols;
    int64_t ld;
} aae_tensor;

int aae_abi_version(void);
const char* aae_last_error(void);
int aae_set_option(const char* name, const char* value);

int aae_arena_bytes(const aae_config* cfg, size_t* bytes_out);
int aae_create(const aae_config* cfg, void* arena_dev, size_t arena_bytes, void* stream,
               aae_handle* out);
int aae_destroy(aae_handle h);
int aae_tensor_info(aae_handle h, int tensor_id, aae_tensor* out);
int aae_sync(aae_handle h, void* stream);
int aae_set_rng_rows(aae_handle h, int64_t row_offset, int64_t global_rows);
int aae_params_changed(aae_handle h);
int aae_set_lr(aae_handle h, double gen_lr, double reg_lr);

int aae_load_linear(aae_handle h, int net, int layer, const float* weight_host,
                    const float* bias_host);
int aae_store_linear(aae_handle h, int net, int layer, float* weight_host, float* bias_host);
int aae_load_adam(aae_handle h, int which, int layer, const float* m_w, const float* v_w,
                  const float* m_b, const float* v_b, int64_t step);
int aae_store_adam(aae_handle h, int which, int layer, float* m_w, float* v_w, float* m_b,
                   float* v_b, int64_t* step);

int aae_step(aae_handle h, const aae_batch* batch, const float* cond_dev,
             const aae_rng_inject* inject, void* stream);

int aae_ae_encode(aae_handle h, const aae_batch* batch, const aae_rng_inject* inject,
                  float* z_out_dev, void* stream);
int aae_ae_decode_backward(aae_handle h, const float* zc_dev, int64_t zc_ld,
                           const aae_rng_inject* inject, float* dzc_out_dev, void* stream);
int aae_ae_encoder_backward(aae_handle h, const float* dz_dev, int64_t dz_ld, void* stream);
int aae_disc_gen(aae_handle h, const aae_rng_inject* inject, void* stream);
int aae_decoder_step(aae_handle h, const aae_batch* batch, const float* zin_dev, int64_t zin_ld,
                     const aae_rng_inject* inject, float* dzin_out_dev, void* stream);
int aae_vae_step(aae_handle h, const aae_batch* batch, const float* cond_dev, const float* eps_dev, void* stream);
int aae_vae_predict(aae_handle h, const aae_batch* batch, const float* cond_dev, const float* eps_dev,
                    float* out_dev, int64_t out_ld, void* stream);
int aae_vae_encode(aae_handle h, const aae_batch* batch, const float* eps_dev, float* z_out_dev, int32_t train, void* stream);
int aae_vae_decode_backward(aae_handle h, const float* zc_dev, int64_t zc_ld, float* dzc_out_dev, void* stream);
int aae_vae_encoder_backward(aae_handle h, const float* dz_dev, int64_t dz_ld, void* stream);
int aae_ae_forward(aae_handle h, const aae_batch* batch, const float* cond_dev, const aae_rng_inject* inject, void* stream);
int aae_output_layer_step(aae_handle h, const aae_batch* batch, void* stream);
int aae_ae_backward(aae_handle h, const float* dA2_dev, int64_t dA2_ld, void* stream);
int aae_set_doc_l1(aae_handle h, const float* doc_l1_dev);
int aae_set_first_layer_external(aae_handle h, int on);
int aae_first_layer_forward(aae_handle h, const aae_batch* batch, const float* bias_dev, void* stream);
int aae_first_layer_update(aae_handle h, const float* ga1_dev, int64_t ld, int32_t rows_per_block, int64_t block_stride,
                           int which, void* stream);
int aae_apply_gathered(aae_handle h, int which_a, int which_b, const float* packets_dev, int64_t peer_stride,
                       int32_t n_peers, int64_t span_offset, void* stream);

enum { AAE_CAT_SUM = 0, AAE_CAT_MEAN = 1 };
enum { AAE_CAT_SPARSE_ADAM = 0, AAE_CAT_ADAM = 1 };
int aae_cat_encode(const float* table_dev, int32_t vocab, int32_t dim, const int32_t* idx_dev, int32_t rows,
                   int32_t width, int32_t reduce, float* out_dev, int64_t out_ld, void* stream);
int aae_cat_update(float* table_dev, float* exp_avg_dev, float* exp_avg_sq_dev, float* grad_scratch_dev, int32_t vocab,
                   int32_t dim, const int32_t* idx_dev, int32_t rows, int32_t width, int32_t reduce,
                   const float* dout_dev, int64_t dout_ld, int32_t optimizer, double lr, int64_t step, void* stream);
int aae_csr_embed(const int64_t* indptr_dev, const int32_t* indices_dev, const float* values_dev, int32_t n_rows,
                  const float* table_dev, int32_t n_table_rows, int32_t dim, int64_t table_ld, float* out_dev,
                  int64_t out_ld, void* stream);
int aae_dense_to_csr(const void* dense_dev, int32_t elem_bytes, int64_t ld, int32_t rows, int32_t n_cols,
                     int64_t* indptr_dev, int32_t* indices_dev, float* values_dev, int64_t capacity,
                     int32_t* scratch_dev, int32_t* stats_out_host, void* stream);
int aae_disc_step(aae_handle h, const aae_rng_inject* inject, void* stream);
int aae_gen_step(aae_handle h, const aae_rng_inject* inject, void* stream);

int aae_read_losses(aae_handle h, float out_host[3], void* stream);

int aae_predict(aae_handle h, const aae_batch* batch, const float* cond_dev, float* out_dev,
                int64_t out_ld, void* stream);
int aae_predict_topk(aae_handle h, const aae_batch* batch, const float* cond_dev, int32_t k,
                     int32_t exclude_known, int32_t* idx_out_dev, float* val_out_dev, void* stream);
int aae_rank_max_rows(aae_handle h, int32_t k, int32_t* rows_out);
int aae_rank_long_stats(aae_handle h, int64_t out[5]);
// ... 68 lines not shown
#define AAE_METRIC_MAX 32
#define AAE_METRIC_ROW_MAX 4096
#define AAE_RANK_ABSENT 2147483647
typedef enum aae_metric_kind {
    AAE_METRIC_MRR = 0, AAE_METRIC_MAP = 1, AAE_METRIC_P = 2, AAE_METRIC_NDCG = 3, AAE_METRIC_RPREC = 4, AAE_METRIC_CLICKS = 5
} aae_metric_kind;
typedef struct aae_metric_spec {
    int32_t kind;
    int32_t k;
} aae_metric_spec;
typedef struct aae_rank_rows {
    const int64_t* indptr_dev;
    const int32_t* ranks_dev;
    int32_t n_rows;
} aae_rank_rows;
int aae_metric_rows(const aae_rank_rows* rows, const aae_metric_spec* specs, int32_t n_metrics, const double* discounts_dev,
                    int32_t n_discounts, double* per_row_dev, int64_t ld, void* stream);
int aae_metric_finish(const double* per_row_dev, int64_t ld, int32_t n_rows, int32_t n_metrics, double* out_dev, void* stream);
int aae_ranks_from_lists(const int32_t* ids_dev, int64_t ld, int32_t k, const aae_batch* truth, int32_t* ranks_out_dev, void* stream);
typedef struct aae_lowrank {
    const float* vt_dev;
    int64_t ld;
    int32_t n_features;
    int32_t dims;
} aae_lowrank;
int aae_lowrank_scores(const aae_lowrank* lowrank, int32_t n_items, const aae_batch* features, float* hidden_dev, int64_t hidden_ld,
                       float* scores_dev, int64_t ld, void* stream);
int aae_lowrank_topk(const aae_lowrank* lowrank, int32_t n_items, const aae_batch* features, const aae_batch* items, int32_t k,
                     int32_t exclude_known, float* hidden_dev, int64_t hidden_ld, float* scratch_dev, int64_t scratch_ld,
                     int32_t* idx_out_dev, float* val_out_dev, void* stream);
int aae_lowrank_ranks(const aae_lowrank* lowrank, int32_t n_items, const aae_batch* features, const aae_batch* items,
                      const aae_batch* truth, int32_t exclude_known, float* hidden_dev, int64_t hidden_ld, float* scratch_dev,
                      int64_t scratch_ld, int32_t* ranks_out_dev, void* stream);
#define AAE_LOWRANK_DIMS_MAX 4096
int aae_spmm_f32(const aae_batch* rows, const float* dense_dev, int64_t ld, int32_t n_cols, int32_t width, float* out_dev,
                 int64_t ld_out, void* stream);
int aae_encode(aae_handle h, const aae_batch* batch, float* z_out_dev, void* stream);
int aae_decode(aae_handle h, const float* zc_dev, int64_t zc_ld, int32_t n_rows,
               float* out_dev, int64_t out_ld, void* stream);

int aae_apply_updates(aae_handle h, int which, void* stream);
int aae_w1_export(aae_handle h, int32_t* hdr_dev, float* vals_dev, int32_t cap, void* stream);
int aae_w1_packet_floats(aae_handle h, int32_t cap, int64_t* hdr_words, int64_t* total_floats);
int aae_w1_import(aae_handle h, const int32_t* hdr_dev, const float* vals_dev, int32_t cap, int32_t n_peers,
                  int64_t peer_stride_bytes, int which, void* stream);
int aae_apply_updates_except(aae_handle h, int which, int skip_tensor_id, void* stream);
int aae_apply_shard(aae_handle h, int tensor_id, int64_t row_begin, int64_t row_end,
                    const float* grad_shard_dev, int which, void* stream);
typedef struct aae_collectives {
    void* ctx;
    int (*all_gather)(void* ctx, const float* send_dev, float* recv_dev, int64_t count, void* stream);
    int (*reduce_scatter)(void* ctx, const float* send_dev, float* recv_dev, int64_t count, void* stream);
    int (*all_reduce)(void* ctx, float* buf_dev, int64_t count, void* stream);
    int32_t world, rank;
} aae_collectives;
int aae_rccl_unique_id(char id_out[128]);
int aae_rccl_init(const char id[128], int32_t world, int32_t rank, aae_collectives* out);
int aae_rccl_destroy(aae_collectives* c);
int aae_dp_reserve(aae_handle replica, int32_t n_rows, int32_t world);
int aae_dp_step(aae_handle replica, aae_handle slice, const aae_collectives* coll, const aae_batch* local,
                const aae_batch* global_slice, const aae_batch* next_global_slice, const float* cond_dev,
                const aae_rng_inject* inject, void* stream);
int aae_shard_step(aae_handle h, const aae_collectives* coll, const aae_batch* batch, const aae_batch* next_batch,
                   const float* cond_dev, const aae_rng_inject* inject, float item_share, void* stream);
int aae_ipc_create(int64_t max_floats, char handle_out[64], void** mailbox_out);
int aae_ipc_init(void* mailbox, const char* handles, int32_t world, int32_t rank, int64_t max_floats, aae_collectives* out);
int aae_ipc_destroy(aae_collectives* c, void* mailbox);
int aae_echo_collectives(int32_t world, aae_collectives* out);
int aae_memcpy_sync(void* dst, const void* src, size_t bytes, void* stream);

int aae_set_grad_scale(aae_handle h, float scale);

enum { AAE_K_ENC_GATHER = 0,
       AAE_K_DEC_BCE_FWD,
       AAE_K_DEC_DA2,
       AAE_K_DEC_DV3_ADAM,
       AAE_K_ENC_W1_ADAM,
       AAE_K_DEC_FUSED,
       AAE_K_CHAIN,
       AAE_K_DEC_CRIT,
       AAE_K_DEC_OPT,
       AAE_K_RANK,
       AAE_K_COLLECTIVE,
       AAE_K_N };
int aae_profile_enable(aae_handle h, int on);
int aae_profile_read(aae_handle h, int kernel_id, double* total_ms, int64_t* launches);

int aae_set_input_noise(aae_handle h, const float* noise_dev, int64_t noise_ld);
int aae_set_input_noise_gen(aae_handle h, float scale);
int aae_dae_thin(aae_handle h, const int64_t* indptr_dev, const int32_t* indices_dev, const float* values_dev, int64_t n_rows,
                 float p, float* out_values_dev, void* stream);
int aae_join(aae_handle h, void* stream);
int aae_join_output_layer(aae_handle h, void* stream);
int aae_prefetch_batch(aae_handle h, const aae_batch* next);
int aae_set_split(aae_handle h, int32_t workgroups);

#ifdef __cplusplus
}
#endif
#endif
```

Measured before the change: 449,800 docs/s.

## Inline next-batch unique-item and W1 catch-up work into chain kernel spare workgroups

```diff
diff --git a/aae-recommender_amd/aaerec/_hip.py b/aae-recommender_amd/aaerec/_hip.py
--- a/aae-recommender_amd/aaerec/_hip.py
+++ b/aae-recommender_amd/aaerec/_hip.py
@@ -45,6 +45,7 @@
 T_ADAM_ENC, T_ADAM_GEN, T_ADAM_DEC, T_ADAM_DISC, T_GRAD = 16, 32, 48, 64, 80
 T_ACT_Z, T_ACT_LOSSES, T_ACT_A1, T_ACT_DZC, T_ACT_DH2, T_ACT_DA2 = 96, 97, 98, 99, 100, 101
 T_ACT_GA1 = 102
+T_W1_TSYNC = 103
 CAT_SUM, CAT_MEAN = 0, 1
 CAT_SPARSE_ADAM, CAT_ADAM = 0, 1
 O_ENC, O_DEC, O_GEN, O_DISC = 0, 1, 2, 3
@@ -250,6 +251,7 @@
     "aae_set_split": (C.c_int, [C.c_void_p, C.c_int32]),
 }
 K_ENC_GATHER, K_DEC_BCE_FWD, K_DEC_DA2, K_DEC_DV3_ADAM, K_ENC_W1_ADAM, K_DEC_FUSED, K_CHAIN, K_DEC_CRIT, K_DEC_OPT, K_RANK, K_COLLECTIVE = range(11)
+K_UNIQ_ITEMS, K_W1_CATCHUP = 11, 12
 
 _lib = None
 
diff --git a/aae-recommender_amd/csrc/aae_abi.hip b/aae-recommender_amd/csrc/aae_abi.hip
--- a/aae-recommender_amd/csrc/aae_abi.hip
+++ b/aae-recommender_amd/csrc/aae_abi.hip
@@ -56,7 +56,7 @@
 
 int aae_set_option(const char* name, const char* value) {
     if (!name || !*name) return fail(AAE_EINVAL, "option name is empty");
-    static const char* known[] = {"NO_CHAIN", "CHAIN16", "SPLIT_ANY", "BLOCKED_ANY", "EARLY_ANY", "NO_LATE_JOIN", "NO_ITEM_COUNT", "NO_ITEM_LISTS", "W1_SERIAL",
+    static const char* known[] = {"NO_CHAIN", "CHAIN16", "SPLIT_ANY", "BLOCKED_ANY", "EARLY_ANY", "NO_LATE_JOIN", "NO_ITEM_COUNT", "NO_ITEM_LISTS", "NO_INLINE_PREFETCH", "INLINE_PF_DISC8", "W1_SERIAL",
                                   "NO_RANK_FUSED", "CHAIN_KSLICES", "X16_ROWS", "DW_KSPLIT_ROWS", "DEC_TS", "CHAIN_TS", "DW_TS", "DEC_SKIP", "CHAIN_SKIP", "RANK_SKIP",
                                   "RANK_COLLECT_CAP"};
     bool ok = false;
@@ -216,7 +216,7 @@
             const double t_tile = (2.2 + 0.0096 * m->h) * (m->bf16_one ? 0.98 : 1.0);
             int w = (int)(ntiles * t_tile / (m->bf16_one ? 127.0 : 57.0) / 8.0 + 0.5) * 8;
             w = std::max(w, std::min(ntiles, m->bf16_one ? 40 : 64));
-            const int cap = m->late_enabled ? m->n_cu * 7 / 16 : m->n_cu * 9 / 16;
+            const int cap = !m->late_enabled ? m->n_cu * 9 / 16 : inline_prefetch_handle(m) ? m->n_cu * 13 / 32 : m->n_cu * 7 / 16;
             m->split_wgs = std::max(1, std::min(w, cap));
         }
     }
@@ -386,6 +386,9 @@
     else if (id == AAE_T_ACT_LOSSES) {
         tmp.rows = 1; tmp.cols = 4; tmp.ld = 4; tmp.off = (size_t)((char*)h->losses - h->base); t = &tmp;
     }
+    else if (id == AAE_T_W1_TSYNC && h->lazy) {
+        tmp.rows = 1; tmp.cols = h->N; tmp.ld = h->N; tmp.off = (size_t)((char*)h->tsync - h->base); t = &tmp;
+    }
     if (!t) return fail(AAE_EINVAL, "unknown tensor id");
     out->byte_offset = t->off; out->rows = t->rows; out->cols = t->cols; out->ld = t->ld;
     return AAE_OK;
diff --git a/aae-recommender_amd/csrc/abi_chains.h b/aae-recommender_amd/csrc/abi_chains.h
--- a/aae-recommender_amd/csrc/abi_chains.h
+++ b/aae-recommender_amd/csrc/abi_chains.h
@@ -279,6 +279,7 @@
     if (four && m->x16_ok && cb.P.rows >= (cb.x16_rows > 0 ? cb.x16_rows : m->x16_rows) && !cb.P.bk.enabled && !cb.P.il.enabled && x16_program_ok(cb.P)) {
         ChainProgram X = cb.P;
         if (x16_remap_slots(X)) {
+            cb.P.uq.enabled = cb.P.cu.enabled = 0;
             X.x16_row_lo = 1 << 30;
             for (int i = 0; i < X.nops; ++i) if (X.ops[i].row_lo > 0) X.x16_row_lo = X.ops[i].row_lo;
             for (int cls = 0; cls < 2; ++cls) {
@@ -302,6 +303,9 @@
     int grid = (cb.P.rows + (four ? kR4 : kCR) - 1) / (four ? kR4 : kCR) + (cb.P.bk.enabled ? 1 : 0);
     if (cb.P.il.enabled && !four) cb.P.il.enabled = 0;
     if (cb.P.il.enabled) { grid += cb.P.il.nblocks; m->il_set ^= 1; m->item_lists_valid = true; }
+    if (!four || ts_kernel || cb.vae4) cb.P.uq.enabled = cb.P.cu.enabled = 0;
+    if (cb.P.cu.enabled) { cb.P.uq.enabled = 0; grid += cb.P.cu.nblocks; }
+    else if (cb.P.uq.enabled) grid += cb.P.uq.nblocks;
     hipLaunchKernelGGL(kernel, dim3(grid), dim3(four ? kC4T : kCT), kCSlots * kCR * kCL * sizeof(float), s, cb.P);
     LAUNCHCHK("chain_kernel");
     return want_ts ? print_chain_timeline(cb.P, ts_dev, false, four, s) : AAE_OK;
@@ -588,6 +592,69 @@
     j.enabled = 1;
 }
 
+bool inline_prefetch_handle(const aae_model* m) {
+    return !m->opt.no_inline_prefetch && !m->ae_only && !m->vae && m->use_chain4 && m->lazy && m->cfg.grad_mode == AAE_GRAD_FUSED &&
+           m->cfg.optimizer == AAE_OPT_ADAM && !m->early_any && !m->opt.chain_ts;
+}
+bool inline_prefetch_applies(const aae_model* m) {
+    return inline_prefetch_handle(m) && m->whole_step && !m->dense_step && !m->ext_first && m->rows <= 16 * kMB &&
+           m->pf_batch.n_rows <= 16 * kMB && !(m->x16_ok && 2 * m->rows >= m->x16_rows);
+}
+static BatchView view_of(const aae_batch& b) {
+    BatchView bv; bv.indptr = b.indptr_dev; bv.indices = b.indices_dev; bv.values = b.values_dev;
+    bv.rows = b.rows_dev; bv.row_start = b.row_start; bv.n_rows = b.n_rows;
+    return bv;
+}
+static void piggyback_next_list(aae_model* m, ChainBuilder& cb) {
+    if (!m->inl_step || m->inl_uniq_out) return;
+    UniqJob& j = cb.P.uq;
+    j.bv = view_of(m->inl_batch); j.mark = m->mark2; j.stamp = m->stamp2; j.ulist = m->ulist2; j.ucount = m->ucount2;
+    j.nblocks = (m->inl_batch.n_rows + kC4W - 1) / kC4W;
+    j.enabled = 1;
+}
+static int next_list_sent(aae_model* m, const ChainBuilder* cb, hipStream_t s) {
+    if (!m->inl_step || m->inl_uniq_out) return AAE_OK;
+    if (!cb || !cb->P.uq.enabled) {
+        ProfScope ps(m, AAE_K_UNIQ_ITEMS, s);
+        const aae_batch& b = m->inl_batch;
+        const int mr = b.max_row_nnz > 0 ? b.max_row_nnz : 1024;
+        const int gy = std::max(1, std::min(16, std::max(1, std::min(64, (mr + 15) / 16)) / 16 + 1));
+        hipLaunchKernelGGL(uniq_items_kernel, dim3(b.n_rows, gy), dim3(256), 0, s, view_of(b), m->mark2, m->stamp2, m->ulist2, m->ucount2);
+        LAUNCHCHK("uniq_items (next batch)");
+    }
+    m->inl_uniq_out = true;
+    return AAE_OK;
+}
+static void piggyback_next_catchup(aae_model* m, ChainBuilder& cb, int hi8) {
+    if (!m->inl_step || !m->inl_uniq_out || m->inl_cu8 >= hi8) return;
+    CatchupJob& j = cb.P.cu;
+    j.a = W1Catchup{m->ulist2, m->ucount2, m->N, m->tsync, m->P[P_W1T].p, m->M[0][P_W1T].p, m->V[0][P_W1T].p, m->M[1][P_W1T].p,
+                    m->V[1][P_W1T].p, m->ldw1, m->h, m->tab, m->mark, m->stamp};
+    j.upto = (int)m->hstep; j.lo8 = m->inl_cu8; j.hi8 = hi8;
+    const int bound = std::min(m->cfg.max_nnz, std::max(256, m->inl_batch.n_rows * 32));
+    const int share = std::max(1, (bound * (hi8 - m->inl_cu8) / 8 + kC4T / 256 - 1) / (kC4T / 256));
+    const int idle = m->n_cu - (m->opt_pending ? m->split_wgs : 0) - (cb.P.rows + kR4 - 1) / kR4 - 8;
+    j.nblocks = std::max(8, std::min(idle, share));
+    j.enabled = 1;
+}
+static void next_catchup_sent(aae_model* m, const ChainBuilder& cb) {
+    if (cb.P.cu.enabled) m->inl_cu8 = cb.P.cu.hi8;
+}
+static int inline_prefetch_done(aae_model* m, hipStream_t s) {
+    if (!m->inl_step) return AAE_OK;
+    if (m->inl_cu8 < 8) {
+        ProfScope ps(m, AAE_K_W1_CATCHUP, s);
+        const int grid = std::min(m->cfg.max_nnz, std::max(256, m->inl_batch.n_rows * 32));
+        hipLaunchKernelGGL(w1_catchup_kernel, dim3(grid), dim3(256), 0, s, m->ulist2, m->ucount2, m->N, m->tsync,
+                           m->P[P_W1T].p, m->M[0][P_W1T].p, m->V[0][P_W1T].p, m->M[1][P_W1T].p, m->V[1][P_W1T].p,
+                           m->ldw1, m->h, m->tab, m->step_ctr, 0, m->mark, m->stamp, m->hstep);
+        LAUNCHCHK("w1_catchup (next batch)");
+    }
+    m->inl_step = false;
+    m->pf_built = true; m->pf_step = m->hstep + 1; m->pf_built_batch = m->inl_batch;
+    return AAE_OK;
+}
+
 int chain_ae_forward(aae_model* m, bool with_dec, const float* cond_dev, float* z_out, hipStream_t s) {
     const int B = m->rows, h = m->h, c = m->c, cp = m->cp;
     const aae_rng_inject& I = m->inj;
@@ -672,8 +739,9 @@
         x2.d = make_drop(m, 0, true, I.masks_dev[which == O_GEN ? 8 : 0], nullptr, B, h, which == O_GEN ? 8 : 0);
         cop_out(x2, ga1_ptr(m), m->ldh);
     }
-    if (item_lists) piggyback_item_lists(m, cb);
-    return launch_chain(m, cb, s);
+    if (item_lists) { piggyback_item_lists(m, cb); piggyback_next_list(m, cb); }
+    TRY(launch_chain(m, cb, s));
+    return item_lists ? next_list_sent(m, &cb, s) : AAE_OK;
 }
 
 int encoder_first_layer_update(aae_model* m, const float* ga1, int which, hipStream_t s, bool merged = false) {
@@ -701,13 +769,13 @@
 }
 
 int launch_gather(aae_model* m, const float* bias, float* act_out, const DropSpec& d, bool head, bool open_step, const char* what,
-                  hipStream_t s) {
+                  hipStream_t s, bool bump_next = false) {
     ProfScope ps(m, AAE_K_ENC_GATHER, s);
     const size_t shm = (size_t)16 * r4(m->h) * sizeof(float);
     constexpr int g4_rows = 512;
     const bool four = m->rows >= g4_rows;
     const AdvanceJob adv{m->sc, m->step_ctr, m->lazy ? m->tab : nullptr, m->losses, open_step ? 1 : 0,
-                         head ? m->stamp2 : nullptr, head ? m->ucount2 : nullptr};
+                         head || bump_next ? m->stamp2 : nullptr, head || bump_next ? m->ucount2 : nullptr};
     hipExtLaunchKernelGGL(four ? enc_gather_kernel_t<4> : enc_gather_kernel_t<16>, dim3(m->rows), dim3(four ? 256 : 1024),
                           (uint32_t)(four ? shm / 4 : shm), s, nullptr, head ? m->ev_head : nullptr, 0, m->bv,
                           (const float*)m->P[P_W1T].p, m->ldw1, bias, m->h, (int)m->cfg.normalize_inputs,
@@ -718,9 +786,9 @@
 }
 
 int gather_first_layer(aae_model* m, bool train, const uint8_t* mk1, uint32_t sid1, hipStream_t s, bool head = false,
-                       bool open_step = false) {
+                       bool open_step = false, bool bump_next = false) {
     const DropSpec d1 = make_drop(m, 0, train, mk1, nullptr, m->rows, m->h, sid1);
-    TRY(launch_gather(m, m->P[P_B1].p, m->eh1.p, d1, head, open_step, "enc_gather", s));
+    TRY(launch_gather(m, m->P[P_B1].p, m->eh1.p, d1, head, open_step, "enc_gather", s, bump_next));
     m->pf_bumped = head;
     return AAE_OK;
 }
@@ -747,8 +815,12 @@
     else if (wait_head) HIPCHK(hipStreamWaitEvent(q, m->ev_head, 0));
     if (early || !(wait_head && m->pf_bumped)) hipLaunchKernelGGL(bump_stamp_kernel, dim3(1), dim3(1), 0, q, m->stamp2, m->ucount2);
     m->pf_bumped = false;
-    hipLaunchKernelGGL(uniq_items_kernel, dim3(b.n_rows, gy), dim3(256), 0, q, bv, m->mark2, m->stamp2, m->ulist2, m->ucount2);
+    {
+        ProfScope ps(m, AAE_K_UNIQ_ITEMS, q);
+        hipLaunchKernelGGL(uniq_items_kernel, dim3(b.n_rows, gy), dim3(256), 0, q, bv, m->mark2, m->stamp2, m->ulist2, m->ucount2);
+    }
     if (m->cfg.optimizer == AAE_OPT_ADAM) {
+        ProfScope ps(m, AAE_K_W1_CATCHUP, q);
         const int grid = std::min(m->cfg.max_nnz, std::max(256, b.n_rows * 32));
         hipLaunchKernelGGL(w1_catchup_kernel, dim3(grid), dim3(256), 0, q, m->ulist2, m->ucount2, m->N, m->tsync,
                            m->P[P_W1T].p, m->M[0][P_W1T].p, m->V[0][P_W1T].p, m->M[1][P_W1T].p, m->V[1][P_W1T].p,
@@ -897,7 +969,9 @@
         cop_out(x3, m->gb0.p, m->ldh);
         ChainOp& x2 = cb.add(cop_dx(m, P_D2, 5, 6, h, h, CEPI_ACTBWD, s)); x2.yslot = 1; x2.d = d1.d;
         cop_out(x2, m->gb1.p, m->ldh);
+        piggyback_next_catchup(m, cb, m->opt.inline_pf_disc8);
         TRY(launch_chain(m, cb, s));
+        next_catchup_sent(m, cb);
     }
     DwBuilder dw;
     dw.add(m, m->ga3.p, 4, m->xh2.p, m->ldh, 2 * B, P_D3, O_DISC);
@@ -940,7 +1014,11 @@
     cop_out(w3, m->gb2.p, m->ldh);
     ChainOp& w2 = cb.add(cop_dx(m, P_W2, 7, 8, h, h, CEPI_ACTBWD, s)); w2.yslot = 1; w2.d = e1.d;
     cop_out(w2, ga1_ptr(m), m->ldh);
+    TRY(next_list_sent(m, nullptr, s));
+    piggyback_next_catchup(m, cb, 8);
     TRY(launch_chain(m, cb, s));
+    next_catchup_sent(m, cb);
+    TRY(inline_prefetch_done(m, s));
     DwBuilder dw;
     dw.add(m, m->ga3.p, m->ldz, m->eh2.p, m->ldh, B, P_W3, O_GEN);
     dw.add(m, m->gb2.p, m->ldh, m->eh1.p, m->ldh, B, P_W2, O_GEN);
diff --git a/aae-recommender_amd/csrc/abi_layers.h b/aae-recommender_amd/csrc/abi_layers.h
--- a/aae-recommender_amd/csrc/abi_layers.h
+++ b/aae-recommender_amd/csrc/abi_layers.h
@@ -47,6 +47,7 @@
     m->bv.indptr = b->indptr_dev; m->bv.indices = b->indices_dev; m->bv.values = b->values_dev;
     m->bv.rows = b->rows_dev; m->bv.row_start = b->row_start; m->bv.n_rows = b->n_rows;
     m->rows = b->n_rows; m->have_batch = true; m->buckets_valid = false; m->item_lists_valid = false; m->w1_merged = false;
+    m->inl_step = false;
     {
         int mr = b->max_row_nnz > 0 ? b->max_row_nnz : 1024;
         m->chunks = std::max(1, std::min(64, (mr + 15) / 16));
@@ -57,10 +58,14 @@
 int lazy_prepare(aae_model* m, int upto_off, bool bump, hipStream_t s) {
     if (bump) hipLaunchKernelGGL(bump_stamp_kernel, dim3(1), dim3(1), 0, s, m->stamp, m->ucount);
     int gy = std::max(1, std::min(16, m->chunks / 16 + 1));
-    hipLaunchKernelGGL(uniq_items_kernel, dim3(m->rows, gy), dim3(256), 0, s, m->bv, m->mark, m->stamp, m->ulist,
-                       m->ucount);
+    {
+        ProfScope ps(m, AAE_K_UNIQ_ITEMS, s);
+        hipLaunchKernelGGL(uniq_items_kernel, dim3(m->rows, gy), dim3(256), 0, s, m->bv, m->mark, m->stamp, m->ulist,
+                           m->ucount);
+    }
     LAUNCHCHK("uniq_items");
     if (m->cfg.optimizer == AAE_OPT_ADAM) {
+        ProfScope ps(m, AAE_K_W1_CATCHUP, s);
         int grid = std::min(m->cfg.max_nnz, std::max(256, m->rows * 32));
         hipLaunchKernelGGL(w1_catchup_kernel, dim3(grid), dim3(256), 0, s, m->ulist, m->ucount, m->N, m->tsync,
                            m->P[P_W1T].p, m->M[0][P_W1T].p, m->V[0][P_W1T].p, m->M[1][P_W1T].p, m->V[1][P_W1T].p,
@@ -72,6 +77,7 @@
 
 int lazy_flush(aae_model* m, hipStream_t s) {
     if (!m->lazy || m->cfg.optimizer != AAE_OPT_ADAM) return AAE_OK;
+    ProfScope ps(m, AAE_K_W1_CATCHUP, s);
     hipLaunchKernelGGL(w1_catchup_kernel, dim3(std::min(m->N, 8192)), dim3(256), 0, s, (const int*)nullptr,
                        (const int*)nullptr, m->N, m->tsync, m->P[P_W1T].p, m->M[0][P_W1T].p, m->V[0][P_W1T].p,
                        m->M[1][P_W1T].p, m->V[1][P_W1T].p, m->ldw1, m->h, m->tab, m->step_ctr, 0);
diff --git a/aae-recommender_amd/csrc/abi_model.h b/aae-recommender_amd/csrc/abi_model.h
--- a/aae-recommender_amd/csrc/abi_model.h
+++ b/aae-recommender_amd/csrc/abi_model.h
@@ -30,6 +30,7 @@
 
 }
 
+constexpr int kInlinePfDisc8 = 0;
 struct aae_options {
     bool no_chain;
     bool chain16;
@@ -38,6 +39,8 @@
     bool early_any;
     bool no_late_join;
     bool no_item_lists;
+    bool no_inline_prefetch;
+    int inline_pf_disc8;
     bool no_item_count;
     bool w1_serial;
     bool no_rank_fused;
@@ -57,6 +60,7 @@
     o.no_chain = on("NO_CHAIN"); o.chain16 = on("CHAIN16"); o.split_any = on("SPLIT_ANY"); o.blocked_any = on("BLOCKED_ANY");
     o.early_any = on("EARLY_ANY"); o.no_late_join = on("NO_LATE_JOIN"); o.no_item_count = on("NO_ITEM_COUNT");
     o.no_item_lists = on("NO_ITEM_LISTS");
+    o.no_inline_prefetch = on("NO_INLINE_PREFETCH"); o.inline_pf_disc8 = std::max(0, std::min(num("INLINE_PF_DISC8", kInlinePfDisc8), 8));
     o.w1_serial = on("W1_SERIAL"); o.no_rank_fused = on("NO_RANK_FUSED"); o.chain_kslices = on("CHAIN_KSLICES");
     o.x16_rows = num("X16_ROWS", 1024); o.dw_ksplit_rows = num("DW_KSPLIT_ROWS", -1);
     o.rank_collect_cap = std::max(0, std::min(num("RANK_COLLECT_CAP", 0), 4096));
@@ -144,6 +148,7 @@
     aae_batch pf_batch, pf_built_batch; bool pf_armed; bool pf_built; long long pf_step; long long hstep;
     bool pf_pending; hipEvent_t ev_head, ev_pf;
     bool pf_bumped = false;
+    bool whole_step = false, inl_step = false, inl_uniq_out = false; int inl_cu8 = 0; aae_batch inl_batch;
     bool pf_after_opt = false;
     hipEvent_t ev_bk = nullptr; bool bk_pending = false;
     bool last_out_split = false;
diff --git a/aae-recommender_amd/csrc/abi_step_open.h b/aae-recommender_amd/csrc/abi_step_open.h
--- a/aae-recommender_amd/csrc/abi_step_open.h
+++ b/aae-recommender_amd/csrc/abi_step_open.h
@@ -108,9 +108,13 @@
     if (m->pf_armed && !pf) m->pf_armed = false;
     if (m->use_chain) {
         const bool early = pf && ahead && end_marked && spec_ok && m->early_enabled && (m->rows > 16 * kMB || m->early_any);
+        const bool inl = pf && !early && inline_prefetch_applies(m);
         if (early) TRY(launch_prefetch(m, true, true));
-        TRY(gather_first_layer(m, true, m->inj.masks_dev[0], 0, s, pf && !early, fold_advance));
-        if (pf && !early) TRY(launch_prefetch(m));
+        TRY(gather_first_layer(m, true, m->inj.masks_dev[0], 0, s, pf && !early && !inl, fold_advance, inl));
+        if (inl) {
+            m->inl_step = true; m->inl_uniq_out = false; m->inl_cu8 = 0; m->inl_batch = m->pf_batch;
+            m->pf_armed = false;
+        } else if (pf && !early) TRY(launch_prefetch(m));
         TRY(chain_ae_forward(m, with_dec, cond_dev, z_out, s));
         m->phase = 1;
         return AAE_OK;
diff --git a/aae-recommender_amd/csrc/abi_step_phases.h b/aae-recommender_amd/csrc/abi_step_phases.h
--- a/aae-recommender_amd/csrc/abi_step_phases.h
+++ b/aae-recommender_amd/csrc/abi_step_phases.h
@@ -312,7 +312,10 @@
     if (m->ext_first) return fail(AAE_ESTATE, "aae_step: the first layer is external (aae_set_first_layer_external): drive the phases");
     if (m->cfg.cond_inc > 0 && !cond_dev) return fail(AAE_EINVAL, "cond_inc > 0 needs cond_dev");
     hipStream_t s = S(stream);
-    TRY(ae_encode_impl(m, batch, inj, nullptr, true, cond_dev, stream));
+    m->whole_step = true;
+    const int rc = ae_encode_impl(m, batch, inj, nullptr, true, cond_dev, stream);
+    m->whole_step = false;
+    TRY(rc);
     TRY(stage_cond(m, cond_dev, s));
     DecodeMode mode; mode.enc_too = true;
     TRY(decode_backward(m, nullptr, 0, nullptr, nullptr, mode, s));
diff --git a/aae-recommender_amd/csrc/chain.h b/aae-recommender_amd/csrc/chain.h
--- a/aae-recommender_amd/csrc/chain.h
+++ b/aae-recommender_amd/csrc/chain.h
@@ -74,6 +74,8 @@
     ChainOp ops[kCMaxOps];
     int kslices;
     ItemListJob il;
+    UniqJob uq;
+    CatchupJob cu;
 };
 
 __device__ __forceinline__ void chain_barrier() { asm volatile("s_waitcnt lgkmcnt(0)\n\ts_barrier" ::: "memory"); }
diff --git a/aae-recommender_amd/csrc/chain4.h b/aae-recommender_amd/csrc/chain4.h
--- a/aae-recommender_amd/csrc/chain4.h
+++ b/aae-recommender_amd/csrc/chain4.h
@@ -167,12 +167,28 @@
 template <bool BF, bool TS = false, bool COLS = false, bool VAE = false>
 __global__ __launch_bounds__(kC4T) void chain4_kernel(ChainProgram P) {
     extern __shared__ __attribute__((aligned(16))) float slots[];
+    const int nx_blocks = (TS || VAE) ? 0 : P.cu.enabled ? P.cu.nblocks : P.uq.enabled ? P.uq.nblocks : 0;
+    const int il_end = (int)gridDim.x - nx_blocks;
+    if constexpr (!TS && !VAE) {
+        if ((int)blockIdx.x >= il_end) {
+            static_assert((kC4T / 256) * kLazyReplay * sizeof(LazyTab) <= kCSlots * kCR * kCL * sizeof(float),
+                          "the catch-up's staged table entries (one set per row in flight) fit a chain workgroup's LDS");
+            const int vb = (int)blockIdx.x - il_end;
+            if (P.cu.enabled) {
+                w1_catchup_body<kC4T>(P.cu.a, P.cu.upto, reinterpret_cast<LazyTab*>(slots), vb, nx_blocks, P.cu.lo8, P.cu.hi8);
+            } else {
+                const int wv = __builtin_amdgcn_readfirstlane((int)threadIdx.x >> 6);
+                uniq_items_body(P.uq.bv, P.uq.mark, P.uq.stamp, P.uq.ulist, P.uq.ucount, vb * kC4W + wv, nx_blocks * kC4W, 0, 1, (int)threadIdx.x & 63, 64);
+            }
+            return;
+        }
+    }
     const int il_blocks = P.il.enabled ? P.il.nblocks : 0;
-    if ((int)blockIdx.x >= (int)gridDim.x - il_blocks) {
-        w1_lists_build_body<kC4T>(P.il, reinterpret_cast<unsigned*>(slots), (int)blockIdx.x - ((int)gridDim.x - il_blocks), il_blocks);
+    if ((int)blockIdx.x >= il_end - il_blocks) {
+        w1_lists_build_body<kC4T>(P.il, reinterpret_cast<unsigned*>(slots), (int)blockIdx.x - (il_end - il_blocks), il_blocks);
         return;
     }
-    if (P.bk.enabled && (int)blockIdx.x == (int)gridDim.x - 1 - il_blocks) {
+    if (P.bk.enabled && (int)blockIdx.x == il_end - 1 - il_blocks) {
         tile_bucket_body<kBucketMaxDocs, kC4T>(P.bk.bv, P.bk.ntiles, P.bk.tstart, P.bk.eb, P.bk.en, P.bk.ev, reinterpret_cast<int*>(slots));
         return;
     }
diff --git a/aae-recommender_amd/csrc/kernels.h b/aae-recommender_amd/csrc/kernels.h
--- a/aae-recommender_amd/csrc/kernels.h
+++ b/aae-recommender_amd/csrc/kernels.h
@@ -550,18 +550,25 @@
 }
 
 
+__device__ __forceinline__ void uniq_items_body(const BatchView& bv, int* __restrict__ mark, const int* __restrict__ stamp_p,
+                                                int* __restrict__ ulist, int* __restrict__ ucount, int bx, int nbx, int by,
+                                                int nby, int tid, int nt) {
+    const int stamp = *stamp_p;
+    for (int b = bx; b < bv.n_rows; b += nbx) {
+        const int dc = bv.doc(b);
+        const int64_t lo = bv.indptr[dc], hi = bv.indptr[dc + 1];
+        for (int64_t e = lo + (int64_t)by * nt + tid; e < hi; e += (int64_t)nby * nt) {
+            const int idx = bv.indices[e];
+            if (atomicExch(&mark[idx], stamp) != stamp) ulist[atomicAdd(ucount, 1)] = idx;
+        }
+    }
+}
 __global__ __launch_bounds__(256) void uniq_items_kernel(BatchView bv, int* __restrict__ mark,
                                                          const int* __restrict__ stamp_p, int* __restrict__ ulist,
                                                          int* __restrict__ ucount) {
-    const int b = blockIdx.x;
-    const int dc = bv.doc(b);
-    const int64_t lo = bv.indptr[dc], hi = bv.indptr[dc + 1];
-    const int stamp = *stamp_p;
-    for (int64_t e = lo + (int64_t)blockIdx.y * 256 + threadIdx.x; e < hi; e += (int64_t)gridDim.y * 256) {
-        const int idx = bv.indices[e];
-        if (atomicExch(&mark[idx], stamp) != stamp) ulist[atomicAdd(ucount, 1)] = idx;
-    }
-}
+    uniq_items_body(bv, mark, stamp_p, ulist, ucount, (int)blockIdx.x, (int)gridDim.x, (int)blockIdx.y, (int)gridDim.y, (int)threadIdx.x, 256);
+}
+struct UniqJob { int enabled, nblocks; BatchView bv; int* mark; const int* stamp; int* ulist; int* ucount; };
 
 __device__ __forceinline__ void lazy_replay(float& p, float& m1, float& v1, float& m3, float& v3, int t0, int upto,
                                             const LazyTab* stab) {
@@ -584,6 +591,44 @@
     }
 }
 
+struct W1Catchup {
+    const int* ulist; const int* ucount; int n_rows_all; int* tsync;
+    float* W; float* M1; float* V1; float* M3; float* V3; int ld, h;
+    const LazyTab* tab; const int* skip_mark; const int* skip_stamp;
+};
+template <int NT>
+__device__ __forceinline__ void w1_catchup_body(const W1Catchup& a, int upto, LazyTab* stab, int vblock, int vgrid, int lo8, int hi8) {
+    static_assert(NT % 256 == 0, "w1_catchup_body: whole 256-thread quarters");
+    constexpr int Q = NT / 256;
+    const int q = __builtin_amdgcn_readfirstlane((int)threadIdx.x >> 8), t = (int)threadIdx.x & 255;
+    LazyTab* st = stab + q * kLazyReplay;
+    const int cnt = a.ulist ? *a.ucount : a.n_rows_all;
+    const int r_lo = (int)(((long long)cnt * lo8) >> 3), r_hi = (int)(((long long)cnt * hi8) >> 3);
+    const int skip = a.skip_mark ? *a.skip_stamp : 0;
+    for (int base = r_lo + vblock * Q; base < r_hi; base += vgrid * Q) {
+        const int r = base + q;
+        int row = 0, t0 = upto;
+        if (r < r_hi) {
+            row = a.ulist ? a.ulist[r] : r;
+            t0 = (a.skip_mark && a.skip_mark[row] == skip) ? upto : a.tsync[row];
+        }
+        if (t0 < upto) {
+            const int nl = min(upto - t0, kLazyReplay);
+            for (int j = t; j < nl; j += 256) st[j] = a.tab[(t0 + 1 + j) & (kLazyTabCap - 1)];
+        }
+        __syncthreads();
+        if (t0 < upto) {
+            for (int c = t; c < a.h; c += 256) {
+                const size_t o = (size_t)row * a.ld + c;
+                float p = a.W[o], m1 = a.M1[o], v1 = a.V1[o], m3 = a.M3[o], v3 = a.V3[o];
+                lazy_replay(p, m1, v1, m3, v3, t0, upto, st);
+                a.W[o] = p; a.M1[o] = m1; a.V1[o] = v1; a.M3[o] = m3; a.V3[o] = v3;
+            }
+        }
+        __syncthreads();
+        if (t == 0 && t0 < upto) a.tsync[row] = upto;
+    }
+}
 __global__ __launch_bounds__(256) void w1_catchup_kernel(const int* __restrict__ ulist, const int* __restrict__ ucount,
                                                          int n_rows_all, int* __restrict__ tsync,
                                                          float* __restrict__ W, float* __restrict__ M1,
@@ -594,26 +639,10 @@
                                                          const int* __restrict__ skip_stamp = nullptr, long long upto_abs = -1) {
     __shared__ LazyTab stab[kLazyReplay];
     const int upto = upto_abs >= 0 ? (int)upto_abs : (int)*step_ctr + upto_off;
-    const int cnt = ulist ? *ucount : n_rows_all;
-    const int skip = skip_mark ? *skip_stamp : 0;
-    for (int r = blockIdx.x; r < cnt; r += gridDim.x) {
-        const int row = ulist ? ulist[r] : r;
-        const int t0 = (skip_mark && skip_mark[row] == skip) ? upto : tsync[row];
-        if (t0 < upto) {
-            const int nl = min(upto - t0, kLazyReplay);
-            for (int j = threadIdx.x; j < nl; j += 256) stab[j] = tab[(t0 + 1 + j) & (kLazyTabCap - 1)];
-            __syncthreads();
-            for (int c = threadIdx.x; c < h; c += 256) {
-                const size_t o = (size_t)row * ld + c;
-                float p = W[o], m1 = M1[o], v1 = V1[o], m3 = M3[o], v3 = V3[o];
-                lazy_replay(p, m1, v1, m3, v3, t0, upto, stab);
-                W[o] = p; M1[o] = m1; V1[o] = v1; M3[o] = m3; V3[o] = v3;
-            }
-        }
-        __syncthreads();
-        if (threadIdx.x == 0 && t0 < upto) tsync[row] = upto;
-    }
-}
+    const W1Catchup a{ulist, ucount, n_rows_all, tsync, W, M1, V1, M3, V3, ld, h, tab, skip_mark, skip_stamp};
+    w1_catchup_body<256>(a, upto, stab, (int)blockIdx.x, (int)gridDim.x, 0, 8);
+}
+struct CatchupJob { int enabled, nblocks; W1Catchup a; int upto, lo8, hi8; };
 
 __global__ __launch_bounds__(256) void w1_sparse_adam_kernel(const int* __restrict__ ulist,
                                                              const int* __restrict__ ucount, float* __restrict__ W,
diff --git a/include/aaerec_hip.h b/include/aaerec_hip.h
--- a/include/aaerec_hip.h
+++ b/include/aaerec_hip.h
@@ -99,6 +99,7 @@
     AAE_T_ACT_DH2 = 100,
     AAE_T_ACT_DA2 = 101,
     AAE_T_ACT_GA1 = 102,
+    AAE_T_W1_TSYNC = 103,
     AAE_T_ACT_DZC = 99
 };
 
@@ -333,6 +334,8 @@
        AAE_K_DEC_OPT,
        AAE_K_RANK,
        AAE_K_COLLECTIVE,
+       AAE_K_UNIQ_ITEMS,
+       AAE_K_W1_CATCHUP,
        AAE_K_N };
 int aae_profile_enable(aae_handle h, int on);
 int aae_profile_read(aae_handle h, int kernel_id, double* total_ms, int64_t* launches);
```

New measurement: 459,100 docs/s, median of 6. 1.02x the previous value.
